# zjykzj/YOLOv4

Hardware: AMD Instinct MI355X
Metric: images/sec fwd+bwd @608x608 bs=64 per GPU (YOLOv4 training step: forward + YOLOLoss + backward) (higher is better)
Workload: dtype f32

## Files before the change

include/yolov4_amd.h:

```cpp
#ifndef YOLOV4_AMD_H
#define YOLOV4_AMD_H

#include <stddef.h>
#include <stdint.h>

#ifdef __cplusplus
extern "C" {
#endif

#define Y4_OK 0
#define Y4_ERR_SHAPE 1
#define Y4_ERR_NULL 2
#define Y4_ERR_LAUNCH 3
#define Y4_ERR_WORKSPACE 4
#define Y4_ERR_NODEVICE 5

#define Y4_ACT_LINEAR 0
#define Y4_ACT_LEAKY 1
#define Y4_ACT_MISH 2
#define Y4_ACT_RELU 3

const char* y4_strerror(int code);
int y4_version(void);
int y4_device_count(void);

int y4_set_conv_mode(int mode);
int y4_get_conv_mode(void);
int y4_set_planes_bf16(int on);
int y4_get_planes_bf16(void);
int y4_conv_planes_fit(int B, int H, int W, int Cin, int Cout, int k, int stride, int dgrad_planes);
size_t y4_conv2d_fwd_workspace(int Cin, int Cout, int k);
int y4_conv2d_fwd_f32(const float* x, int ldx, const float* w, float* y, int ldy,
                      int B, int H, int W, int Cin, int Cout, int k, int stride,
                      const float* scale, const float* shift, int act,
                      const float* residual, int ldr, const unsigned* x_amax ,
                      unsigned* y_amax ,
                      void* workspace, size_t workspace_bytes, void* stream);
size_t y4_conv2d_prepared_bytes(int Cout, int K);
int y4_conv2d_prepare_filter_f32(const float* w, int Cout, int K, void* prepared, size_t prepared_bytes, void* stream);
int y4_conv2d_fwd_prepared_f32(const float* x, int ldx, void* w_prepared, float* y, int ldy,
                               int B, int H, int W, int Cin, int Cout, int k, int stride,
                               const float* scale, const float* shift, int act,
                               const float* residual, int ldr, const unsigned* x_amax, unsigned* y_amax, void* stream);
int y4_amax_f32(const float* x, int ldx, long long M, int C, unsigned* amax_bits, void* stream);
int y4_amax_merge_u32(unsigned* dst, const unsigned* src, void* stream);

int y4_last_conv_kernel(char* buf, int cap);

size_t y4_conv2d_bnstats_workspace(int B, int H, int W, int Cin, int Cout, int k, int stride);
int y4_conv2d_fwd_bnstats_f32(const float* x, int ldx, const float* w, float* y, int ldy,
                              int B, int H, int W, int Cin, int Cout, int k, int stride,
                              float* partials, size_t partial_bytes, long long* nparts_host,
                              const unsigned* x_amax ,
                              void* workspace, size_t workspace_bytes ,
                              void* dgrad_filter ,
                              size_t dgrad_filter_bytes , void* stream);

int y4_planes_split_f32(const float* x, int ldx, long long M, int C, const unsigned* amax, void* planes, void* stream);
int y4_planes_split_into_f32(const float* x, int ldx, long long M, int C, const unsigned* amax, void* planes, int ld_planes, int c_valid,
                             void* stream);
int y4_conv2d_fwd_planes_f32(const void* x_planes, const float* w, float* y, int ldy,
                             int B, int H, int W, int Cin, int Cout, int k, int stride,
                             float* partials, size_t partial_bytes, long long* nparts_host, const unsigned* x_amax,
                             void* workspace, size_t workspace_bytes,
                             void* dgrad_filter ,
                             size_t dgrad_filter_bytes,
                             int y_bf16 ,
                             const float* bias ,
                             void* stream);

int y4_conv2d_dgrad_planes_f32(const void* dy_planes, const float* w , float* dx, int lddx,
                               int B, int H, int W, int Cin, int Cout, int k,
                               int stride ,
                               void* workspace, size_t workspace_bytes, const unsigned* dy_amax,
                               const float* residual, int ldr, void* stream);
size_t y4_conv2d_wgrad_planes_workspace(int B, int H, int W, int Cin, int Cout, int k, int stride);
int y4_conv2d_wgrad_planes_f32(const void* x_planes, const void* dy_planes, float* dw,
                               int B, int H, int W, int Cin, int Cout, int k, int stride,
                               void* workspace, size_t workspace_bytes, const unsigned* x_amax, const unsigned* dy_amax,
                               void* stream);

int y4_conv2d_generic_fwd_f32(const float* x, int ldx, const float* w, float* y, int ldy,
                              int B, int H, int W, int Cin, int Cout, int k, int stride,
                              const float* scale, const float* shift, int act, const float* residual, int ldr, void* stream);
int y4_conv2d_generic_dgrad_f32(const float* dy, int lddy, const float* w, float* dx, int lddx,
                                int B, int H, int W, int Cin, int Cout, int k, int stride,
                                const float* residual, int ldr, void* stream);
int y4_conv2d_generic_wgrad_f32(const float* x, int ldx, const float* dy, int lddy, float* dw,
                                int B, int H, int W, int Cin, int Cout, int k, int stride, void* stream);
int y4_conv2d_stem_dgrad_f32(const float* dy, int lddy, const float* w, float* dx, long long sxb, long long sxc, long long sxh,
                             long long sxw, int B, int H, int W, int Cout, void* stream);

int y4_conv2d_stem_fwd_f32(const float* x, long long sxb, long long sxc, long long sxh, long long sxw,
                           const float* w, float* y, int ldy, int B, int H, int W, int Cout,
                           const float* scale, const float* shift, int act,
                           float* bnstats_partials, void* stream);

size_t y4_conv2d_dgrad_workspace(int Cin, int Cout, int k);
int y4_conv2d_dgrad_f32(const float* dy, int lddy, const float* w , float* dx, int lddx,
                        int B, int H, int W, int Cin, int Cout, int k, int stride,
                        void* workspace, size_t workspace_bytes, const unsigned* dy_amax ,
                        const float* residual, int ldr, void* stream);

size_t y4_conv2d_wgrad_workspace(int B, int H, int W, int Cin, int Cout, int k, int stride);
int y4_conv2d_wgrad_f32(const float* x, int ldx, const float* dy, int lddy, float* dw,
                        int B, int H, int W, int Cin, int Cout, int k, int stride,
                        void* workspace, size_t workspace_bytes,
                        const unsigned* x_amax, const unsigned* dy_amax , void* stream);
size_t y4_conv2d_stem_wgrad_workspace(int B, int H, int W, int Cout);
int y4_conv2d_stem_wgrad_f32(const float* x, long long sxb, long long sxc, long long sxh, long long sxw,
                             const float* dy, int lddy, float* dw, int B, int H, int W, int Cout,
                             void* workspace, size_t workspace_bytes, void* stream);

size_t y4_bn_workspace(long long M, int C);
size_t y4_bn_finalize_workspace(int C);
int y4_bn_stats_f32(const float* y, int ldy, long long M, int C, float* mean, float* invstd,
                    float* running_mean, float* running_var, long long* num_batches_tracked,
                    float momentum, float eps, void* workspace, size_t workspace_bytes, void* stream);
int y4_bn_finalize_partials_f32(const float* partials, long long nparts, long long M, int C,
                                float* mean, float* invstd, float* running_mean, float* running_var,
                                long long* num_batches_tracked, float momentum, float eps,
                                void* workspace, size_t workspace_bytes, void* stream);
int y4_bn_planes_bound_f32(const float* gamma, const float* beta, int C, long long M, const unsigned* floor_word, unsigned* out,
                           void* stream);
int y4_bn_act_fwd_f32(const float* y, int ldy, const float* mean, const float* invstd,
                      const float* gamma, const float* beta, int act,
                      const float* residual, int ldr, float* z, int ldz,
                      long long M, int C, unsigned* out_amax, int z_planes, const unsigned* res_amax, float* planes_twin,
                      void* stream);
int y4_bn_act_bwd_f32(const float* dz, int lddz, const float* y, int ldy,
                      const float* mean, const float* invstd, const float* gamma, const float* beta,
                      int act, float* dy, int lddy, float* dgamma, float* dbeta,
                      long long M, int C, void* workspace, size_t workspace_bytes,
                      unsigned* out_amax ,
                      unsigned* f16_planes ,
                      float* planes_twin ,
                      int frozen_stats ,
                      void* stream);
size_t y4_bias_grad_workspace(long long M, int C);
int y4_bias_grad_f32(const float* dy, int lddy, long long M, int C, float* dbias,
                     void* workspace, size_t workspace_bytes, void* stream);
int y4_bn_fold_f32(const float* gamma, const float* beta, const float* running_mean,
                   const float* running_var, float eps, float* scale, float* shift, int C, void* stream);

int y4_copy_channels_f32(const float* src, int lds, float* dst, int ldd, long long M, int C, void* stream);
int y4_add_f32(const float* a, int lda, const float* b, int ldb, float* out, int ldo,
               long long M, int C, void* stream);
int y4_maxpool_s1_fwd_f32(const float* x, int ldx, float* y, int ldy, signed char* idx,
                          int B, int H, int W, int C, int ksize, void* stream);
int y4_maxpool_s1_bwd_f32(const float* dy, int lddy, const signed char* idx, float* dx, int lddx,
                          int accumulate, int B, int H, int W, int C, int ksize, void* stream);
int y4_upsample2x_fwd_f32(const float* x, int ldx, float* y, int ldy, int B, int H, int W, int C, void* stream);
int y4_upsample2x_bwd_f32(const float* dy, int lddy, float* dx, int lddx, int B, int H, int W, int C, void* stream);

int y4_yolo_decode_train_f32(const float* logits, int ldl, float* output, float* pred,
                             int B, int F, int A, int n_classes, const float* anchors_wh_host, void* stream);
int y4_yolo_decode_eval_f32(const float* logits, int ldl, float* out, long long n_total, long long box_off,
                            int B, int F, int A, int n_classes, const float* anchors_wh_host,
                            float stride, void* stream);
int y4_yolo_decode_bwd_f32(const float* logits, int ldl, const float* g_output, const float* g_pred,
                           float* g_logits, int B, int F, int A, int n_classes,
                           const float* anchors_wh_host, void* stream);

size_t y4_yolo_loss_workspace(int B, int F, int A, int K, int n_classes);
int y4_yolo_loss_fwd_f32(const float* output, const float* pred, const float* labels, int K,
                         int B, int F, int A, int n_classes, float stride, float ignore_thresh,
                         const float* all_anchors_host, int n_all_anchors, const int* anch_mask_host,
                         float* obj_mask, double* loss_parts,
                         void* workspace, size_t workspace_bytes, void* stream);
int y4_yolo_loss_bwd_f32(const float* output, int output_is_masked, const float* obj_mask,
                         const float* gscale, float* g_output,
                         int B, int F, int A, int K, int n_classes,
                         const void* workspace, size_t workspace_bytes, void* stream);
int y4_yolo_loss_mask_output_f32(float* output, const float* obj_mask, int B, int F, int A, int K,
                                 int n_classes, const void* workspace, size_t workspace_bytes, void* stream);
int y4_yolo_loss_dense_targets_f32(float* target, float* tgt_mask, float* tgt_scale,
                                   int B, int F, int A, int K, int n_classes,
                                   const void* workspace, size_t workspace_bytes, void* stream);

int y4_post_scan_i32(const int* counts, int n_segments, long long cap, int* seg_offsets, int* info, void* stream);
int y4_post_compact_f32(const float* det_rows, const int* seg_offsets, const int* kept, int B, int n_classes,
                        float* out_rows, int* out_offsets, int* img_offsets, void* stream);
int y4_post_count_f32(float* prediction, int B, long long N, int n_classes, float conf_thre,
                      int convert_xyxy, int* counts, void* stream);
size_t y4_post_nms_workspace(long long total_candidates, int n_segments);
int y4_post_nms_f32(const float* prediction, int B, long long N, int n_classes, float conf_thre,
                    float nms_thre, const int* seg_offsets , long long total_candidates,
                    float* det_rows , int* kept ,
                    void* workspace, size_t workspace_bytes, void* stream);
size_t y4_nms_workspace(long long R);
int y4_nms_f32(const float* boxes, const float* scores , long long R, float thresh,
               int limit, int* keep_idx , int* n_keep ,
               void* workspace, size_t workspace_bytes, void* stream);

int y4_bboxes_iou_f32(const float* boxes_a, long long Na, const float* boxes_b, long long Nb, int xyxy, float* iou,
                      void* stream);
int y4_act_fwd_f32(const float* x, float* y, long long n, int act, void* stream);
int y4_act_bwd_f32(const float* x, const float* dy, float* dx, long long n, int act, void* stream);
int y4_upsample_nearest_fwd_f32(const float* x, int ldx, float* y, int ldy, int B, int H, int W, int Ho, int Wo, int C,
                                int integer_factor, void* stream);
int y4_upsample_nearest_bwd_f32(const float* dy, int lddy, float* dx, int lddx, int B, int H, int W, int Ho, int Wo, int C,
                                int integer_factor, void* stream);

int y4_adam_step_f32(float* param, const float* grad, float* exp_avg, float* exp_avg_sq, long long n,
                     float lr, float beta1, float beta2, float eps, float weight_decay, int step,
                     float grad_scale, void* stream);
int y4_adam_hyper_f32(float lr, float beta1, float beta2, float weight_decay, int step, float* out4_host);
int y4_adam_multi_step_f32(const void* chunks_dev, int nchunks, const float* hyper_host, int nhyper,
                           float beta1, float beta2, float eps, float grad_scale, void* stream);
int y4_sgd_multi_step_f32(const void* chunks_dev, int nchunks, const float* hyper_host, int nhyper,
                          float grad_scale, void* stream);

int y4_preprocess_u8_f32(const void* src, int src_h, int src_w, long long src_pitch_bytes, int swap_rb,
                         float* dst, long long dst_sc, long long dst_sh, long long dst_sw, int S, void* stream);

#ifdef __cplusplus
}
#endif
#endif
```

yolov4_amd/_lib.py:

```python
import ctypes
import os
from ctypes import c_char_p, c_double, c_float, c_int, c_longlong, c_size_t, c_void_p

_HERE = os.path.dirname(os.path.abspath(__file__))
LIB_PATH = os.environ.get('Y4_LIB_PATH') or os.path.join(_HERE, 'lib', 'libyolov4_amd.so')

ACT_IDS = {'linear': 0, 'leaky_relu': 1, 'mish': 2, 'relu': 3}


class Y4Error(RuntimeError):
    pass


P = c_void_p
I, L, F, Z = c_int, c_longlong, c_float, c_size_t

PROTOTYPES = {
    'y4_strerror': (c_char_p, [I]),
    'y4_version': (I, []),
    'y4_device_count': (I, []),
    'y4_set_conv_mode': (I, [I]),
    'y4_get_conv_mode': (I, []),
    'y4_set_planes_bf16': (I, [I]),
    'y4_get_planes_bf16': (I, []),
    'y4_conv_planes_fit': (I, [I, I, I, I, I, I, I, I]),
    'y4_conv2d_fwd_workspace': (Z, [I, I, I]),
    'y4_conv2d_fwd_f32': (I, [P, I, P, P, I, I, I, I, I, I, I, I, P, P, I, P, I, P, P, P, Z, P]),
    'y4_amax_f32': (I, [P, I, L, I, P, P]),
    'y4_conv2d_prepared_bytes': (Z, [I, I]),
    'y4_conv2d_prepare_filter_f32': (I, [P, I, I, P, Z, P]),
    'y4_conv2d_fwd_prepared_f32': (I, [P, I, P, P, I, I, I, I, I, I, I, I, P, P, I, P, I, P, P, P]),
    'y4_amax_merge_u32': (I, [P, P, P]),
    'y4_last_conv_kernel': (I, [ctypes.c_char_p, I]),
    'y4_conv2d_bnstats_workspace': (Z, [I, I, I, I, I, I, I]),
    'y4_conv2d_fwd_bnstats_f32': (I, [P, I, P, P, I, I, I, I, I, I, I, I, P, Z, P, P, P, Z, P, Z, P]),
    'y4_planes_split_f32': (I, [P, I, L, I, P, P, P]),
    'y4_planes_split_into_f32': (I, [P, I, L, I, P, P, I, I, P]),
    'y4_conv2d_fwd_planes_f32': (I, [P, P, P, I, I, I, I, I, I, I, I, P, Z, P, P, P, Z, P, Z, I, P, P]),
    'y4_conv2d_dgrad_planes_f32': (I, [P, P, P, I, I, I, I, I, I, I, I, P, Z, P, P, I, P]),
    'y4_conv2d_wgrad_planes_workspace': (Z, [I, I, I, I, I, I, I]),
    'y4_conv2d_wgrad_planes_f32': (I, [P, P, P, I, I, I, I, I, I, I, P, Z, P, P, P]),
    'y4_conv2d_generic_fwd_f32': (I, [P, I, P, P, I, I, I, I, I, I, I, I, P, P, I, P, I, P]),
    'y4_conv2d_generic_dgrad_f32': (I, [P, I, P, P, I, I, I, I, I, I, I, I, P, I, P]),
    'y4_conv2d_generic_wgrad_f32': (I, [P, I, P, I, P, I, I, I, I, I, I, I, P]),
    'y4_conv2d_stem_dgrad_f32': (I, [P, I, P, P, L, L, L, L, I, I, I, I, P]),
    'y4_conv2d_stem_fwd_f32': (I, [P, L, L, L, L, P, P, I, I, I, I, I, P, P, I, P, P]),
    'y4_conv2d_dgrad_workspace': (Z, [I, I, I]),
    'y4_conv2d_dgrad_f32': (I, [P, I, P, P, I, I, I, I, I, I, I, I, P, Z, P, P, I, P]),
    'y4_conv2d_wgrad_workspace': (Z, [I, I, I, I, I, I, I]),
    'y4_conv2d_wgrad_f32': (I, [P, I, P, I, P, I, I, I, I, I, I, I, P, Z, P, P, P]),
    'y4_conv2d_stem_wgrad_workspace': (Z, [I, I, I, I]),
    'y4_conv2d_stem_wgrad_f32': (I, [P, L, L, L, L, P, I, P, I, I, I, I, P, Z, P]),
    'y4_bn_workspace': (Z, [L, I]),
    'y4_bn_finalize_workspace': (Z, [I]),
    'y4_bn_finalize_partials_f32': (I, [P, L, L, I, P, P, P, P, P, F, F, P, Z, P]),
    'y4_bn_stats_f32': (I, [P, I, L, I, P, P, P, P, P, F, F, P, Z, P]),
    'y4_bn_act_fwd_f32': (I, [P, I, P, P, P, P, I, P, I, P, I, L, I, P, I, P, P, P]),
    'y4_bn_planes_bound_f32': (I, [P, P, I, L, P, P, P]),
    'y4_bn_act_bwd_f32': (I, [P, I, P, I, P, P, P, P, I, P, I, P, P, L, I, P, Z, P, P, P, I, P]),
    'y4_bias_grad_workspace': (Z, [L, I]),
    'y4_bias_grad_f32': (I, [P, I, L, I, P, P, Z, P]),
    'y4_bn_fold_f32': (I, [P, P, P, P, F, P, P, I, P]),
    'y4_copy_channels_f32': (I, [P, I, P, I, L, I, P]),
    'y4_add_f32': (I, [P, I, P, I, P, I, L, I, P]),
    'y4_maxpool_s1_fwd_f32': (I, [P, I, P, I, P, I, I, I, I, I, P]),
    'y4_maxpool_s1_bwd_f32': (I, [P, I, P, P, I, I, I, I, I, I, I, P]),
    'y4_upsample2x_fwd_f32': (I, [P, I, P, I, I, I, I, I, P]),
    'y4_upsample2x_bwd_f32': (I, [P, I, P, I, I, I, I, I, P]),
    'y4_yolo_decode_train_f32': (I, [P, I, P, P, I, I, I, I, P, P]),
    'y4_yolo_decode_eval_f32': (I, [P, I, P, L, L, I, I, I, I, P, F, P]),
    'y4_yolo_decode_bwd_f32': (I, [P, I, P, P, P, I, I, I, I, P, P]),
    'y4_yolo_loss_workspace': (Z, [I, I, I, I, I]),
    'y4_yolo_loss_fwd_f32': (I, [P, P, P, I, I, I, I, I, F, F, P, I, P, P, P, P, Z, P]),
    'y4_yolo_loss_bwd_f32': (I, [P, I, P, P, P, I, I, I, I, I, P, Z, P]),
    'y4_yolo_loss_mask_output_f32': (I, [P, P, I, I, I, I, I, P, Z, P]),
    'y4_yolo_loss_dense_targets_f32': (I, [P, P, P, I, I, I, I, I, P, Z, P]),
    'y4_post_count_f32': (I, [P, I, L, I, F, I, P, P]),
    'y4_post_scan_i32': (I, [P, I, L, P, P, P]),
    'y4_post_compact_f32': (I, [P, P, P, I, I, P, P, P, P]),
    'y4_post_nms_workspace': (Z, [L, I]),
    'y4_post_nms_f32': (I, [P, I, L, I, F, F, P, L, P, P, P, Z, P]),
    'y4_nms_workspace': (Z, [L]),
    'y4_nms_f32': (I, [P, P, L, F, I, P, P, P, Z, P]),
    'y4_bboxes_iou_f32': (I, [P, L, P, L, I, P, P]),
    'y4_act_fwd_f32': (I, [P, P, L, I, P]),
    'y4_act_bwd_f32': (I, [P, P, P, L, I, P]),
    'y4_upsample_nearest_fwd_f32': (I, [P, I, P, I, I, I, I, I, I, I, I, P]),
    'y4_upsample_nearest_bwd_f32': (I, [P, I, P, I, I, I, I, I, I, I, I, P]),
    'y4_adam_step_f32': (I, [P, P, P, P, L, F, F, F, F, F, I, F, P]),
    'y4_adam_hyper_f32': (I, [F, F, F, F, I, P]),
    'y4_adam_multi_step_f32': (I, [P, I, P, I, F, F, F, F, P]),
    'y4_sgd_multi_step_f32': (I, [P, I, P, I, F, P]),
    'y4_preprocess_u8_f32': (I, [P, I, I, L, I, P, L, L, L, I, P]),
}

_lib = None


def lib():
    global _lib
    if _lib is None:
        if not os.path.isfile(LIB_PATH):
            raise Y4Error(f'{LIB_PATH} is missing: build it with `make -C yolov4_amd/csrc` '
                          '(hipcc --offload-arch=gfx950); there is no fallback path')
        handle = ctypes.CDLL(LIB_PATH)
        for name, (res, args) in PROTOTYPES.items():
            fn = getattr(handle, name)
            fn.restype = res
            fn.argtypes = args
        _lib = handle
        if os.environ.get('Y4_CONV_MODE'):
            handle.y4_set_conv_mode(int(os.environ['Y4_CONV_MODE']))
    return _lib


def check(code, what=''):
    if code != 0:
        msg = lib().y4_strerror(code).decode()
        raise Y4Error(f'{what}: {msg} (code {code})')


def float_array(values):
    arr = (c_float * len(values))(*[float(v) for v in values])
    return arr


def int_array(values):
    return (c_int * len(values))(*[int(v) for v in values])
```

yolov4_amd/csrc/common.h:

```cpp
#pragma once
#include <hip/hip_runtime.h>
#include <stdint.h>
#include "../../include/yolov4_amd.h"

typedef float f32x4 __attribute__((ext_vector_type(4)));
typedef float f32x16 __attribute__((ext_vector_type(16)));
typedef unsigned int u32x4 __attribute__((ext_vector_type(4)));

#define Y4_CHECK_LAUNCH()                                   \
    do {                                                    \
        if (hipGetLastError() != hipSuccess) return Y4_ERR_LAUNCH; \
    } while (0)

static inline hipStream_t y4_stream(void* s) { return reinterpret_cast<hipStream_t>(s); }

#include <atomic>
struct Y4DynLds {
    std::atomic<unsigned long long> done{0ull};
    bool ensure(const void* kernel, size_t bytes) {
        int d = 0;
        if (hipGetDevice(&d) != hipSuccess) return false;
        if (d >= 0 && d < 64 && ((done.load(std::memory_order_acquire) >> d) & 1ull)) return true;
        if (hipFuncSetAttribute(kernel, hipFuncAttributeMaxDynamicSharedMemorySize, (int)bytes) != hipSuccess) return false;
        if (d >= 0 && d < 64) done.fetch_or(1ull << d, std::memory_order_release);
        return true;
    }
};

__device__ __forceinline__ float y4_mish(float x) {
    const float n = __expf(fminf(x, 20.0f));
    const float w = n * (n + 2.0f);
    return x * (w * __frcp_rn(w + 2.0f));
}
__device__ __forceinline__ float y4_mish_grad(float x) {
    const float n = __expf(fminf(x, 20.0f));
    const float w = n * (n + 2.0f);
    const float rd = __frcp_rn(w + 2.0f);
    const float q = fmaf(n, n, n);
    return fmaf(4.0f * (x * q), rd, w) * rd;
}
__device__ __forceinline__ float y4_act(float x, int act) {
    switch (act) {
        case Y4_ACT_LEAKY: return x > 0.0f ? x : 0.1f * x;
        case Y4_ACT_MISH: return y4_mish(x);
        case Y4_ACT_RELU: return fmaxf(x, 0.0f);
        default: return x;
    }
}
__device__ __forceinline__ float y4_act_grad(float x, int act) {
    switch (act) {
        case Y4_ACT_LEAKY: return x > 0.0f ? 1.0f : 0.1f;
        case Y4_ACT_MISH: return y4_mish_grad(x);
        case Y4_ACT_RELU: return x > 0.0f ? 1.0f : 0.0f;
        default: return 1.0f;
    }
}

template <int ACT> __device__ __forceinline__ float y4_act_t(float x) {
    if constexpr (ACT == Y4_ACT_LEAKY) return x > 0.0f ? x : 0.1f * x;
    else if constexpr (ACT == Y4_ACT_MISH) return y4_mish(x);
    else if constexpr (ACT == Y4_ACT_RELU) return fmaxf(x, 0.0f);
    else return x;
}
template <int ACT> __device__ __forceinline__ float y4_act_grad_t(float x) {
    if constexpr (ACT == Y4_ACT_LEAKY) return x > 0.0f ? 1.0f : 0.1f;
    else if constexpr (ACT == Y4_ACT_MISH) return y4_mish_grad(x);
    else if constexpr (ACT == Y4_ACT_RELU) return x > 0.0f ? 1.0f : 0.0f;
    else return 1.0f;
}

__device__ __forceinline__ int y4_xcd_remap(int bid, int nwg) {
    const int q = nwg >> 3, r = nwg & 7, xcd = bid & 7;
    const int base = (xcd < r) ? xcd * (q + 1) : r * (q + 1) + (xcd - r) * q;
    return base + (bid >> 3);
}

__device__ __forceinline__ __amdgpu_buffer_rsrc_t y4_make_rsrc(const void* base, unsigned num_bytes) {
    return __builtin_amdgcn_make_buffer_rsrc(const_cast<void*>(base), (short)0, (int)num_bytes, 0x00020000);
}
__device__ __forceinline__ f32x4 y4_buf_load4(__amdgpu_buffer_rsrc_t r, unsigned voff_bytes, unsigned soff_bytes) {
    const u32x4 v = __builtin_amdgcn_raw_buffer_load_b128(r, (int)voff_bytes, (int)soff_bytes, 0);
    return __builtin_bit_cast(f32x4, v);
}
```

yolov4_amd/csrc/conv_geom.h:

```cpp
#pragma once
#include "common.h"

namespace y4 {

struct ConvGeom {
    const float* src; const float* wt; float* dst;
    const float* scale; const float* shift; const float* res;
    float* stats;
    long long lds_, ldd, ldr;
    int B, Hs, Ws, Cs;
    int Cs_valid;
    int Hd, Wd, N;
    int k, stride, pad;
    int M;
    int K;
    int act;
    int mtiles, ntiles;
    int cls_tile0[5];
    int cls_h[2], cls_w[2];
    int cls_slot0[5];
    unsigned long long src_total_bytes;
    unsigned wt_bytes;
    const unsigned short* wt_planes;
    const unsigned* src_amax; const unsigned* wt_amax;
    unsigned* dst_amax;
};

struct WgradGeom {
    const float* x; const float* dy; float* out;
    long long ldx, lddy;
    int B, H, W, Cin, Ho, Wo, Cout;
    int k, stride, pad;
    int M;
    int J;
    int ntn, ntj, splits, chunks_per_split;
    int tn, tj;
    const unsigned* x_amax; const unsigned* dy_amax;
    unsigned long long x_total_bytes, dy_total_bytes;
};

int f16x2_gather(const ConvGeom& g, bool transposed, hipStream_t st, int* nparts);
int f16x2_wgrad(const WgradGeom& g, hipStream_t st);
int f16x2_refresh_prepared(const float* w, void* prepared, int Cout, int K, hipStream_t st);
int f16x2_filter_planes(const float* w, unsigned short* planes, int Cout, int K, unsigned* amax_out, unsigned* part, hipStream_t st);
int f16x2_filter_planes_dual(const float* w, unsigned short* planes, unsigned* amax_out, unsigned* part, unsigned short* planes_t,
                             unsigned* amax_out_t, int Cout, int Cin, int kk, int Cout_pad, bool mirror, hipStream_t st);
int f16x2_filter_planes_transposed(const float* w, unsigned short* planes, int Cout, int Cin, int kk, int Cout_pad,
                                   unsigned* amax_out, unsigned* part, hipStream_t st, bool mirror = false);
int slab_reduce(const float* slabs, float* dw, long long n, int splits, hipStream_t st);
int amax_launch(const float* x, long long ld, long long M, int C, unsigned* amax_bits, hipStream_t st,
                bool prezeroed = false);
int amax_merge(unsigned* dst, const unsigned* src, hipStream_t st);


bool tile_conv_ok(int Cs, int Cs_valid, int N, int k, int stride, int H, int W);
int f16x2_tile(const ConvGeom& g, hipStream_t st, int* nparts);
bool tile_dgrad_s2_ok(int Cs, int Cs_valid, int N, int k, int stride, int Hs, int Ws);
int f16x2_tile_dgrad_s2(const ConvGeom& g, hipStream_t st);

bool tile_wgrad_ok(int Cin, int Cout, int k, int stride, int H, int W, long long ldx, long long lddy);
int tile_wgrad_slabs(int Cin, int Cout);
int f16x2_wgrad_tile(const WgradGeom& g, hipStream_t st);

bool planes_conv_ok(int Cin, int Cout, int k, int stride);
int planes_conv(const void* src, const unsigned* src_amax, const void* wt_planes, const unsigned* wt_amax, float* dst, long long ldd,
                const float* res, long long ldr, float* stats, int* nparts, int B, int Hs, int Ws, int Cs, int N, int k, int stride,
                hipStream_t st, bool bf = false, bool dst_bf16 = false);
int planes_dgrad_s2(const void* dy, const unsigned* dy_amax, const void* wt_planes, const unsigned* wt_amax, float* dx, long long lddx,
                    int B, int H, int W, int Cin, int Cout, hipStream_t st, bool bf = false);
int planes_split(const float* x, long long ld, long long M, int C, const unsigned* amax, void* planes, hipStream_t st, bool bf = false,
                 long long pitch_ch = 0, int c_valid = 0);
void planes_wgrad_plan(int B, int H, int W, int Cin, int Cout, int k, int* ntn, int* ntj, int* splits, int* sps, int tn = 128, bool bf = false);
int planes_wgrad_tn(int Cout, bool bf);
int planes_wgrad(const void* x, const unsigned* x_amax, const void* dy, const unsigned* dy_amax, float* dw, void* workspace,
                 size_t workspace_bytes, int B, int H, int W, int Cin, int Cout, int k, hipStream_t st, bool bf = false,
                 int stride = 1);

void note_kernel(const char* fmt, ...);
}
```

yolov4_amd/csrc/conv_igemm.hip:

```cpp
#include <stdlib.h>
#include "common.h"
#include <cstdarg>
#include <cstdio>
#include "conv_geom.h"

namespace {

constexpr int BK = 32;


using y4::ConvGeom;
using y4::WgradGeom;

template <int BM, int BN, int WM, int WN, bool TRANSPOSED, int BKT = 32>
__global__ __launch_bounds__(256, (BKT == 16 ? 3 : 2)) void conv_gather_mfma_f32(const ConvGeom g) {
    constexpr int LPR = BKT / 4;
    constexpr int RPP = 256 / LPR;
    constexpr int PA = BM / RPP, PB = BN / RPP;
    constexpr int LDS_PITCH = BKT + 4;
    constexpr int BK = BKT;
    constexpr int WTM = BM / WM, WTN = BN / WN;
    constexpr int TM = WTM / 32, TN = WTN / 32;
    static_assert(WM * WN == 4, "4 waves");
    extern __shared__ __attribute__((aligned(16))) float smem[];
// ... 1073 lines not shown
    f32x4 ra[4], rb[4];
    int ld_chunk = 0;
    auto load_chunk = [&]() {
        const int pbase = (chunk0 + ld_chunk) * 32 + pg * 4;
#pragma unroll
        for (int i = 0; i < 4; ++i) {
            const bool ok = an_ok && pbase + i < g.M;
            ra[i] = y4_buf_load4(dy_rsrc, ok ? a_off0 + (unsigned)i * dy_pix_bytes : OOB, (unsigned)ld_chunk * chunk_bytes);
        }
#pragma unroll
        for (int i = 0; i < 4; ++i) {
            const int hi = pb_h[i] * g.stride - g.pad + jr, wi = pb_w[i] * g.stride - g.pad + jq;
            const bool ok = bj_ok && pbase + i < g.M && (unsigned)hi < (unsigned)g.H && (unsigned)wi < (unsigned)g.W;
            const unsigned off = (unsigned)((pb_b[i] * g.H + hi) * g.W + wi) * x_pix_bytes + (unsigned)jc * 4u;
            rb[i] = y4_buf_load4(x_rsrc, ok ? off : OOB, 0u);
            pb_w[i] += 32;
            while (pb_w[i] >= g.Wo) { pb_w[i] -= g.Wo; if (++pb_h[i] == g.Ho) { pb_h[i] = 0; ++pb_b[i]; } }
        }
        ++ld_chunk;
    };
    auto split_store = [&](const f32x4 (&v)[4], unsigned char* base, int rows) {
        if constexpr (NP == 1) {
#pragma unroll
            for (int e = 0; e < 4; ++e) {
                u32x2 p;
                p[0] = pack_hi16(rn_bf16_bits(v[1][e]), rn_bf16_bits(v[0][e]));
                p[1] = pack_hi16(rn_bf16_bits(v[3][e]), rn_bf16_bits(v[2][e]));
                *reinterpret_cast<u32x2*>(base + (cg * 4 + e) * PITCH_B + pg * 8) = p;
            }
            return;
        }
        unsigned h1[4][4], h2[4][4], h3[4][4];
#pragma unroll
        for (int i = 0; i < 4; ++i)
#pragma unroll
            for (int e = 0; e < 4; ++e) {
                h1[i][e] = __float_as_uint(v[i][e]);
                const float r1 = v[i][e] - __uint_as_float(h1[i][e] & 0xffff0000u);
                h2[i][e] = __float_as_uint(r1);
                const float r2 = r1 - __uint_as_float(h2[i][e] & 0xffff0000u);
                h3[i][e] = __float_as_uint(r2);
            }
#pragma unroll
        for (int e = 0; e < 4; ++e) {
            unsigned char* d = base + (cg * 4 + e) * PITCH_B + pg * 8;
            u32x2 p;
            p[0] = pack_hi16(h1[1][e], h1[0][e]); p[1] = pack_hi16(h1[3][e], h1[2][e]);
            *reinterpret_cast<u32x2*>(d) = p;
            p[0] = pack_hi16(h2[1][e], h2[0][e]); p[1] = pack_hi16(h2[3][e], h2[2][e]);
            *reinterpret_cast<u32x2*>(d + rows * PITCH_B) = p;
            p[0] = pack_hi16(h3[1][e], h3[0][e]); p[1] = pack_hi16(h3[3][e], h3[2][e]);
            *reinterpret_cast<u32x2*>(d + 2 * rows * PITCH_B) = p;
        }
    };
    auto store_chunk = [&]() {
        if (a_act) split_store(ra, As, TN_);
        if (b_act) split_store(rb, Bs, TJ_);
    };

    f32x16 acc[MI][MJ];
#pragma unroll
    for (int i = 0; i < MI; ++i)
#pragma unroll
        for (int jj = 0; jj < MJ; ++jj)
#pragma unroll
            for (int e = 0; e < 16; ++e) acc[i][jj][e] = 0.f;

    const int fr = lane & 31, fh = lane >> 5;
    const unsigned char* a_frag = As + (wm * (TN_ / 2) + fr) * PITCH_B + fh * 16;
    const unsigned char* b_frag = Bs + (wn * (TJ_ / 2) + fr) * PITCH_B + fh * 16;
    if (nchunks > 0) {
        load_chunk();
        store_chunk();
        __syncthreads();
        for (int ch = 0; ch < nchunks; ++ch) {
            if (ch + 1 < nchunks) load_chunk();
#pragma unroll
            for (int ks = 0; ks < 2; ++ks) {
                bf16x8 fa[MI][NP], fb[MJ][NP];
#pragma unroll
                for (int i = 0; i < MI; ++i)
#pragma unroll
                    for (int pl = 0; pl < NP; ++pl)
                        fa[i][pl] = *reinterpret_cast<const bf16x8*>(a_frag + pl * TN_ * PITCH_B + i * 32 * PITCH_B + ks * 32);
#pragma unroll
                for (int jj = 0; jj < MJ; ++jj)
#pragma unroll
                    for (int pl = 0; pl < NP; ++pl)
                        fb[jj][pl] = *reinterpret_cast<const bf16x8*>(b_frag + pl * TJ_ * PITCH_B + jj * 32 * PITCH_B + ks * 32);
#pragma unroll
                for (int i = 0; i < MI; ++i)
#pragma unroll
                    for (int jj = 0; jj < MJ; ++jj) {
                        f32x16 c = acc[i][jj];
                        if constexpr (NP == 3) {
                            c = __builtin_amdgcn_mfma_f32_32x32x16_bf16(fa[i][2], fb[jj][0], c, 0, 0, 0);
                            c = __builtin_amdgcn_mfma_f32_32x32x16_bf16(fa[i][1], fb[jj][1], c, 0, 0, 0);
                            c = __builtin_amdgcn_mfma_f32_32x32x16_bf16(fa[i][0], fb[jj][2], c, 0, 0, 0);
                            c = __builtin_amdgcn_mfma_f32_32x32x16_bf16(fa[i][1], fb[jj][0], c, 0, 0, 0);
                            c = __builtin_amdgcn_mfma_f32_32x32x16_bf16(fa[i][0], fb[jj][1], c, 0, 0, 0);
                        }
                        c = __builtin_amdgcn_mfma_f32_32x32x16_bf16(fa[i][0], fb[jj][0], c, 0, 0, 0);
                        acc[i][jj] = c;
                    }
            }
            __syncthreads();
            if (ch + 1 < nchunks) store_chunk();
            __syncthreads();
        }
    }
    float* out = g.out + (long long)split * g.Cout * g.J;
#pragma unroll
    for (int jj = 0; jj < MJ; ++jj) {
        const int jcol = j0 + wn * (TJ_ / 2) + jj * 32 + fr;
#pragma unroll
        for (int i = 0; i < MI; ++i) {
            const int nb = n0 + wm * (TN_ / 2) + i * 32 + 4 * fh;
#pragma unroll
            for (int e = 0; e < 16; ++e) {
                const int n = nb + (e & 3) + 8 * (e >> 2);
                if (n < g.Cout && jcol < g.J) out[(long long)n * g.J + jcol] = acc[i][jj][e];
            }
        }
    }
}

template <int VEC>
__global__ __launch_bounds__(256) void slab_reduce_vec_kernel(const f32x4* __restrict__ slabs, f32x4* __restrict__ out,
                                                              long long nvec, int splits) {
    constexpr int SG = 256 / VEC;
    __shared__ f32x4 red[SG][VEC];
    const int v = threadIdx.x % VEC, sg = threadIdx.x / VEC;
    const long long i = (long long)blockIdx.x * VEC + v;
    f32x4 s0 = {0.f, 0.f, 0.f, 0.f}, s1 = s0, s2 = s0, s3 = s0;
    if (i < nvec) {
        int k = sg;
        for (; k + 3 * SG < splits; k += 4 * SG) {
            const f32x4 a = slabs[(long long)k * nvec + i], b = slabs[(long long)(k + SG) * nvec + i];
            const f32x4 c = slabs[(long long)(k + 2 * SG) * nvec + i], d = slabs[(long long)(k + 3 * SG) * nvec + i];
            s0 += a; s1 += b; s2 += c; s3 += d;
        }
        for (; k < splits; k += SG) s0 += slabs[(long long)k * nvec + i];
    }
    red[sg][v] = (s0 + s1) + (s2 + s3);
    __syncthreads();
    if (sg == 0 && i < nvec) {
        f32x4 t = red[0][v];
#pragma unroll
        for (int g = 1; g < SG; ++g) t += red[g][v];
        out[i] = t;
    }
}

__global__ void slab_reduce_kernel(const float* __restrict__ slabs, float* __restrict__ out,
                                   long long n, int splits) {
    for (long long i = blockIdx.x * (long long)blockDim.x + threadIdx.x; i < n;
         i += (long long)gridDim.x * blockDim.x) {
        float s = 0.f;
        for (int k = 0; k < splits; ++k) s += slabs[(long long)k * n + i];
        out[i] = s;
    }
}

void wgrad_plan(int B, int H, int W, int Cin, int Cout, int k, int stride, WgradGeom& g) {
    const int pad = (k - 1) / 2;
    g.B = B; g.H = H; g.W = W; g.Cin = Cin; g.Cout = Cout; g.k = k; g.stride = stride; g.pad = pad;
    g.Ho = (H + 2 * pad - k) / stride + 1;
    g.Wo = (W + 2 * pad - k) / stride + 1;
    g.M = B * g.Ho * g.Wo;
    g.J = k * k * Cin;
    g.tn = Cout <= 64 ? 64 : 128;
    g.tj = g.J <= 64 ? 64 : 128;
    g.ntn = (Cout + g.tn - 1) / g.tn;
    g.ntj = (g.J + g.tj - 1) / g.tj;
    const int tiles = g.ntn * g.ntj;
    const int chunks = (g.M + 31) / 32;
    int per_cu = (160 * 1024) / (2 * 32 * (g.tn + g.tj) * 4);
    if (per_cu > 4) per_cu = 4;
    if (g.tn + g.tj == 256 && per_cu > 2) per_cu = 2;
    const int slots = 256 * per_cu;
    int max_s = chunks / 16;
    if (max_s < 1) max_s = 1;
    if (max_s > 4096) max_s = 4096;
    int best_s = 1;
    double best_eff = -1.0;
    for (int sp = 1; sp <= max_s; ++sp) {
        const long long blocks = (long long)tiles * sp;
        const long long rounds = (blocks + slots - 1) / slots;
        double eff = (double)blocks / (double)(rounds * slots);
        if (rounds > 6) eff = 1.0;
        if (eff > best_eff + 0.02) { best_eff = eff; best_s = sp; }
        if (blocks >= 2ll * slots && eff >= 0.93) break;
        if (blocks >= 6ll * slots) break;
    }
    { static const char* fs = getenv("Y4_WGRAD_SPLITS"); if (fs) { best_s = atoi(fs); if (best_s > max_s) best_s = max_s; if (best_s < 1) best_s = 1; } }
    g.chunks_per_split = (chunks + best_s - 1) / best_s;
    const unsigned long long per_px = 8ull * (unsigned long long)((Cout + 3) / 4 * 4 > Cin * stride * stride ? (Cout + 3) / 4 * 4 : Cin * stride * stride);
    const unsigned long long slack = 2ull * g.Ho * g.Wo;
    const unsigned long long max_px = 0xf0000000ull / per_px;
    if (max_px > slack + 32 && (unsigned long long)g.chunks_per_split * 32ull + slack > max_px)
        g.chunks_per_split = (int)((max_px - slack) / 32ull);
    g.splits = (chunks + g.chunks_per_split - 1) / g.chunks_per_split;
}

template <int TN_, int TJ_, int NP = 0>
int launch_wgrad(const WgradGeom& g, hipStream_t st) {
    constexpr bool SPLIT = NP > 0;
    const size_t smem = SPLIT ? (size_t)NP * (TN_ + TJ_) * 80 : 2ull * 32 * (TN_ + TJ_) * sizeof(float);
    void (*kern)(const WgradGeom);
    if constexpr (SPLIT) kern = conv_wgrad_bf16x3<TN_, TJ_, (NP > 0 ? NP : 3)>;
    else kern = conv_wgrad_mfma_f32<TN_, TJ_>;
    static Y4DynLds lds_attr;
    if (!lds_attr.ensure(reinterpret_cast<const void*>(kern), smem)) return Y4_ERR_LAUNCH;
    hipLaunchKernelGGL(kern, dim3(g.ntn * g.ntj * g.splits), dim3(256), smem, st, g);
    Y4_CHECK_LAUNCH();
    return Y4_OK;
}

struct StemGeom {
    const float* x; const float* w; float* y; const float* scale; const float* shift;
    float* stats;
    long long sxb, sxc, sxh, sxw, ldy;
    int B, H, W, Cout, act;
    long long M;
};

__global__ __launch_bounds__(256) void conv_stem_fwd_kernel(const StemGeom g) {
    __shared__ float tile[4][64][33];
    __shared__ __attribute__((aligned(16))) float wl[27 * 32];
    const int tid = threadIdx.x, lane = tid & 63, wave = tid >> 6;
    for (int i = tid; i < 27 * 32; i += 256) {
        const int n = i & 31, kk = i >> 5;
        wl[i] = n < g.Cout ? g.w[n * 27 + kk] : 0.f;
    }
    __syncthreads();
    const long long pix0 = (long long)blockIdx.x * 256 + wave * 64;
    const long long pix = pix0 + lane;
    float acc[32];
#pragma unroll
    for (int n = 0; n < 32; ++n) acc[n] = 0.f;
    if (pix < g.M) {
        const int b = (int)(pix / ((long long)g.H * g.W));
        const int rem = (int)(pix - (long long)b * g.H * g.W);
        const int h = rem / g.W, w = rem - h * g.W;
        const float* xb = g.x + b * g.sxb;
        float xv[27];
#pragma unroll
        for (int r = 0; r < 3; ++r)
#pragma unroll
            for (int q = 0; q < 3; ++q) {
                const int hi = h + r - 1, wi = w + q - 1;
                const bool ok = (unsigned)hi < (unsigned)g.H && (unsigned)wi < (unsigned)g.W;
#pragma unroll
                for (int c = 0; c < 3; ++c) xv[(r * 3 + q) * 3 + c] = ok ? xb[c * g.sxc + hi * g.sxh + wi * g.sxw] : 0.f;
            }
#pragma unroll
        for (int kk = 0; kk < 27; ++kk) {
            const f32x4* wp = reinterpret_cast<const f32x4*>(wl + kk * 32);
            const float v = xv[kk];
#pragma unroll
            for (int n4 = 0; n4 < 8; ++n4) {
                const f32x4 wv = wp[n4];
#pragma unroll
                for (int e = 0; e < 4; ++e) acc[n4 * 4 + e] = fmaf(v, wv[e], acc[n4 * 4 + e]);
            }
            __builtin_amdgcn_sched_barrier(0);
        }
    }
#pragma unroll
    for (int n = 0; n < 32; ++n) {
        float v = acc[n];
        if (n < g.Cout) {
            v = v * (g.scale ? g.scale[n] : 1.f) + (g.shift ? g.shift[n] : 0.f);
            v = y4_act(v, g.act);
        }
        tile[wave][lane][n] = v;
    }
    __syncthreads();
    const int ch = lane & 31;
    if (ch < g.Cout) {
#pragma unroll 4
        for (int it = 0; it < 32; ++it) {
            const int pl = it * 2 + (lane >> 5);
            const long long p = pix0 + pl;
            if (p < g.M) g.y[p * g.ldy + ch] = tile[wave][pl][ch];
        }
    }
    if (g.stats) {
        __shared__ float sred[8][32][2];
        const int grp = tid >> 5;
        float cs = 0.f, css = 0.f;
        for (int i = 0; i < 32; ++i) { const float v = tile[grp >> 1][(grp & 1) * 32 + i][ch]; cs += v; css += v * v; }
        sred[grp][ch][0] = cs; sred[grp][ch][1] = css;
        __syncthreads();
        if (tid < 64) {
            const int c = tid & 31, which = tid >> 5;
            float t = 0.f;
            for (int k = 0; k < 8; ++k) t += sred[k][c][which];
            if (c < g.Cout) g.stats[((long long)blockIdx.x * 2 + which) * g.Cout + c] = t;
        }
    }
}

__global__ __launch_bounds__(256) void conv_stem_fwd_bf16x3_kernel(const StemGeom g, const int ngroups, const float inv_hw,
                                                                   const float inv_w) {
    __shared__ float sred[4][32][2];
    const int tid = threadIdx.x, lane = tid & 63, wave = tid >> 6;
    const int fr = lane & 31, fh = lane >> 5;
    const int HW = g.H * g.W;
    bf16x8 fb[2][3];
    int koff[16];
    int ktap[16];
#pragma unroll
    for (int i = 0; i < 16; ++i) {
        const int k = (i >> 3) * 16 + fh * 8 + (i & 7);
        const int r = k / 9, c = (k - r * 9) / 3, q = k - r * 9 - c * 3;
        const bool kv = k < 27;
        koff[i] = kv ? (int)(c * g.sxc + (r - 1) * g.sxh + (q - 1) * g.sxw) * 4 : 0;
        ktap[i] = kv ? r * 3 + q : 9;
    }
#pragma unroll
    for (int ks = 0; ks < 2; ++ks) {
        f32x4 w0, w1;
#pragma unroll
        for (int i = 0; i < 8; ++i) {
            const int k = ks * 16 + fh * 8 + i;
            const int r = k / 9, c = (k - r * 9) / 3, q = k - r * 9 - c * 3;
            const float v = (k < 27 && fr < g.Cout) ? g.w[fr * 27 + (r * 3 + q) * 3 + c] : 0.f;
            if (i < 4) w0[i] = v; else w1[i - 4] = v;
        }
        u32x2 a1, a2, a3, b1, b2, b3;
        split3x4(w0, a1, a2, a3);
        split3x4(w1, b1, b2, b3);
        const u32x4 q1 = {a1[0], a1[1], b1[0], b1[1]}, q2 = {a2[0], a2[1], b2[0], b2[1]}, q3 = {a3[0], a3[1], b3[0], b3[1]};
        fb[ks][0] = __builtin_bit_cast(bf16x8, q1); fb[ks][1] = __builtin_bit_cast(bf16x8, q2); fb[ks][2] = __builtin_bit_cast(bf16x8, q3);
    }
    const float sc = (g.scale && fr < g.Cout) ? g.scale[fr] : 1.f;
    const float sh = (g.shift && fr < g.Cout) ? g.shift[fr] : 0.f;
    const __amdgpu_buffer_rsrc_t rsrc = y4_make_rsrc(g.x, 0xfffffff0u);
    float xv0[16], xv1[16];
    auto load = [&](float (&xv)[16], long long tile) {
        const long long p = tile * 32 + fr;
        unsigned base = 0xffffffffu;
        unsigned m9 = 0;
        if (p < g.M) {
            int b = (int)((float)p * inv_hw);
            int rem = (int)(p - (long long)b * HW);
            if (rem < 0) { --b; rem += HW; } else if (rem >= HW) { ++b; rem -= HW; }
            int h = (int)((float)rem * inv_w);
            int w = rem - h * g.W;
            if (w < 0) { --h; w += g.W; } else if (w >= g.W) { ++h; w -= g.W; }
            base = (unsigned)(b * g.sxb + h * g.sxh + w * g.sxw) * 4u;
            const unsigned hm = (h > 0 ? 1u : 0u) | 2u | (h + 1 < g.H ? 4u : 0u);
            const unsigned wm = (w > 0 ? 1u : 0u) | 2u | (w + 1 < g.W ? 4u : 0u);
            m9 = ((hm & 1u) ? wm : 0u) | ((hm & 2u) ? wm << 3 : 0u) | ((hm & 4u) ? wm << 6 : 0u);
        }
#pragma unroll
        for (int i = 0; i < 16; ++i) {
            const bool ok = (m9 >> ktap[i]) & 1u;
            xv[i] = __builtin_bit_cast(float, __builtin_amdgcn_raw_buffer_load_b32(rsrc, ok ? (int)(base + (unsigned)koff[i]) : -1, 0, 0));
        }
    };
    float cs = 0.f, css = 0.f;
    auto compute = [&](float (&xv)[16], long long tile) {
        f32x16 acc;
#pragma unroll
        for (int e = 0; e < 16; ++e) acc[e] = 0.f;
#pragma unroll
        for (int ks = 0; ks < 2; ++ks) {
            const f32x4 v0 = {xv[ks * 8 + 0], xv[ks * 8 + 1], xv[ks * 8 + 2], xv[ks * 8 + 3]};
            const f32x4 v1 = {xv[ks * 8 + 4], xv[ks * 8 + 5], xv[ks * 8 + 6], xv[ks * 8 + 7]};
            u32x2 a1, a2, a3, b1, b2, b3;
            split3x4(v0, a1, a2, a3);
            split3x4(v1, b1, b2, b3);
            const u32x4 q1 = {a1[0], a1[1], b1[0], b1[1]}, q2 = {a2[0], a2[1], b2[0], b2[1]}, q3 = {a3[0], a3[1], b3[0], b3[1]};
            const bf16x8 f1 = __builtin_bit_cast(bf16x8, q1), f2 = __builtin_bit_cast(bf16x8, q2), f3 = __builtin_bit_cast(bf16x8, q3);
            acc = __builtin_amdgcn_mfma_f32_32x32x16_bf16(f3, fb[ks][0], acc, 0, 0, 0);
            acc = __builtin_amdgcn_mfma_f32_32x32x16_bf16(f2, fb[ks][1], acc, 0, 0, 0);
            acc = __builtin_amdgcn_mfma_f32_32x32x16_bf16(f1, fb[ks][2], acc, 0, 0, 0);
            acc = __builtin_amdgcn_mfma_f32_32x32x16_bf16(f2, fb[ks][0], acc, 0, 0, 0);
            acc = __builtin_amdgcn_mfma_f32_32x32x16_bf16(f1, fb[ks][1], acc, 0, 0, 0);
            acc = __builtin_amdgcn_mfma_f32_32x32x16_bf16(f1, fb[ks][0], acc, 0, 0, 0);
        }
        const long long mbase = tile * 32 + 4 * fh;
#pragma unroll
        for (int e = 0; e < 16; ++e) {
            const float raw = acc[e];
            cs += raw; css += raw * raw;
            const long long m = mbase + (e & 3) + 8 * (e >> 2);
            if (fr < g.Cout && m < g.M) g.y[m * g.ldy + fr] = y4_act(raw * sc + sh, g.act);
        }
    };
    for (int grp = blockIdx.x; grp < ngroups; grp += gridDim.x) {
        const long long t0 = (long long)grp * 8 + wave * 2;
        load(xv0, t0);
        load(xv1, t0 + 1);
        cs = 0.f; css = 0.f;
        compute(xv0, t0);
        compute(xv1, t0 + 1);
        if (g.stats) {
            cs += __shfl_xor(cs, 32, 64);
            css += __shfl_xor(css, 32, 64);
            if (fh == 0) { sred[wave][fr][0] = cs; sred[wave][fr][1] = css; }
            __syncthreads();
            if (tid < 64) {
                const int c = tid & 31, which = tid >> 5;
                const float t = (sred[0][c][which] + sred[1][c][which]) + (sred[2][c][which] + sred[3][c][which]);
                if (c < g.Cout) g.stats[((long long)grp * 2 + which) * g.Cout + c] = t;
            }
            __syncthreads();
        }
    }
}

struct StemWgradGeom {
    const float* x; const float* dy; float* slabs;
    long long sxb, sxc, sxh, sxw, lddy;
    int B, H, W, Cout;
    long long M, pix_per_wave;
};

__global__ __launch_bounds__(256) void conv_stem_wgrad_kernel(const StemWgradGeom g) {
    const int tid = threadIdx.x, lane = tid & 63;
    const long long wave_id = (long long)blockIdx.x * 4 + (tid >> 6);
    const long long p_begin = wave_id * g.pix_per_wave;
    long long p_end = p_begin + g.pix_per_wave;
    if (p_end > g.M) p_end = g.M;
    const int fr = lane & 31, fh = lane >> 5;
    const bool jok = fr < 27;
    const int tap = jok ? fr / 3 : 0, c = jok ? fr - tap * 3 : 0;
    const int r = tap / 3 - 1, q = tap - (tap / 3) * 3 - 1;
    const bool nok = fr < g.Cout;
    f32x16 acc;
#pragma unroll
    for (int e = 0; e < 16; ++e) acc[e] = 0.f;
    long long p = p_begin + fh;
    int b = 0, h = 0, w = 0;
    if (p < g.M) {
        b = (int)(p / ((long long)g.H * g.W));
        const int rem = (int)(p - (long long)b * g.H * g.W);
        h = rem / g.W; w = rem - h * g.W;
    }
    const long long dy_first = p_begin < g.M ? p_begin : 0;
    const __amdgpu_buffer_rsrc_t dy_rsrc = y4_make_rsrc(g.dy + dy_first * g.lddy, (unsigned)(g.pix_per_wave * g.lddy * 4));
    const __amdgpu_buffer_rsrc_t x_rsrc = y4_make_rsrc(g.x, 0xfffffff0u);
    const unsigned dy_step = (unsigned)g.lddy * 8u;
    unsigned dy_off = ((unsigned)fh * (unsigned)g.lddy + (unsigned)fr) * 4u;
    const long long coff = c * g.sxc;
    for (long long pc = p_begin; pc < p_end; pc += 16) {
        float a[8], bv[8];
#pragma unroll
        for (int u = 0; u < 8; ++u) {
            const bool pok = p < p_end;
            const int hi = h + r, wi = w + q;
            const bool xok = pok && jok && (unsigned)hi < (unsigned)g.H && (unsigned)wi < (unsigned)g.W;
            const unsigned xo = (unsigned)(b * g.sxb + coff + hi * g.sxh + wi * g.sxw) * 4u;
            a[u] = __builtin_bit_cast(float, __builtin_amdgcn_raw_buffer_load_b32(dy_rsrc, (pok && nok) ? (int)dy_off : -1, 0, 0));
            bv[u] = __builtin_bit_cast(float, __builtin_amdgcn_raw_buffer_load_b32(x_rsrc, xok ? (int)xo : -1, 0, 0));
            dy_off += dy_step;
            p += 2;
            w += 2;
            if (w >= g.W) { w -= g.W; if (++h == g.H) { h = 0; ++b; } }
        }
#pragma unroll
        for (int u = 0; u < 8; ++u) acc = __builtin_amdgcn_mfma_f32_32x32x2f32(a[u], bv[u], acc, 0, 0, 0);
    }
    float* out = g.slabs + wave_id * 1024;
#pragma unroll
    for (int e = 0; e < 16; ++e) {
        const int n = (e & 3) + 8 * (e >> 2) + 4 * fh;
        out[n * 32 + fr] = acc[e];
    }
}

__global__ __launch_bounds__(256) void stem_wgrad_reduce1_kernel(const float* __restrict__ slabs, double* __restrict__ part,
                                                                 int nslabs) {
    const int per = (nslabs + gridDim.x - 1) / gridDim.x;
    const int k0 = blockIdx.x * per;
    const int k1 = min(nslabs, k0 + per);
    double s[4] = {0, 0, 0, 0};
    for (int k = k0; k < k1; ++k) {
        const f32x4 v = *reinterpret_cast<const f32x4*>(slabs + (long long)k * 1024 + threadIdx.x * 4);
#pragma unroll
        for (int e = 0; e < 4; ++e) s[e] += (double)v[e];
    }
#pragma unroll
    for (int e = 0; e < 4; ++e) part[(long long)blockIdx.x * 1024 + threadIdx.x * 4 + e] = s[e];
}
__global__ __launch_bounds__(256) void stem_wgrad_reduce2_kernel(const double* __restrict__ part, float* __restrict__ dw,
                                                                 int nparts, int Cout) {
    for (int i = threadIdx.x; i < Cout * 27; i += 256) {
        const int n = i / 27, j = i - n * 27;
        double s = 0.0;
        for (int k = 0; k < nparts; ++k) s += part[(long long)k * 1024 + n * 32 + j];
        dw[i] = (float)s;
    }
}

constexpr int STEM_WAVES = 4096;

}

namespace y4 {
int slab_reduce(const float* slabs, float* dw, long long n, int splits, hipStream_t st) {
    if ((n & 3) == 0 && !(reinterpret_cast<uintptr_t>(dw) & 15) && !(reinterpret_cast<uintptr_t>(slabs) & 15)) {
        const long long nvec = n / 4;
        if (nvec >= 64 * 1024)
            hipLaunchKernelGGL(slab_reduce_vec_kernel<64>, dim3((unsigned)((nvec + 63) / 64)), dim3(256), 0, st,
                               reinterpret_cast<const f32x4*>(slabs), reinterpret_cast<f32x4*>(dw), nvec, splits);
        else
            hipLaunchKernelGGL(slab_reduce_vec_kernel<16>, dim3((unsigned)((nvec + 15) / 16)), dim3(256), 0, st,
                               reinterpret_cast<const f32x4*>(slabs), reinterpret_cast<f32x4*>(dw), nvec, splits);
    } else {
        const int blocks = (int)((n + 255) / 256 > 2048 ? 2048 : (n + 255) / 256);
        hipLaunchKernelGGL(slab_reduce_kernel, dim3(blocks), dim3(256), 0, st, slabs, dw, n, splits);
    }
    Y4_CHECK_LAUNCH();
    return Y4_OK;
}
}

extern "C" {

int y4_set_conv_mode(int mode) {
    if (mode < 0 || mode > 3) return Y4_ERR_SHAPE;
    g_conv_mode = mode;
    return Y4_OK;
}
int y4_get_conv_mode(void) { return g_conv_mode; }

constexpr size_t FWD_WS_HDR = 64 + 4096;

size_t y4_conv2d_fwd_workspace(int Cin, int Cout, int k) {
    if (Cin <= 0 || Cout <= 0 || k <= 0) return 0;
    return FWD_WS_HDR + (size_t)Cout * k * k * Cin * 6;
}

static int conv_fwd_impl(const float* x, int ldx, const float* w, float* y, int ldy,
                         int B, int H, int W, int Cin, int Cout, int k, int stride,
                         const float* scale, const float* shift, int act,
                         const float* residual, int ldr, float* stats, int* nparts, const unsigned* x_amax,
                         unsigned* y_amax, void* workspace, size_t workspace_bytes, void* stream,
                         void* w_prepared = nullptr, void* dgrad_filter = nullptr, size_t dgrad_filter_bytes = 0) {
    if (!x || (!w && !w_prepared) || !y) return Y4_ERR_NULL;
    if (B <= 0 || H <= 0 || W <= 0 || Cout <= 0 || (k != 1 && k != 3) || (stride != 1 && stride != 2))
        return Y4_ERR_SHAPE;
    if (Cin <= 0 || Cin % BK != 0 || ldx < Cin || ldy < Cout || (ldx & 3) || (residual && ldr < Cout))
        return Y4_ERR_SHAPE;
    if ((reinterpret_cast<uintptr_t>(x) & 15) || (reinterpret_cast<uintptr_t>(w) & 15)) return Y4_ERR_SHAPE;
    const int pad = (k - 1) / 2;
    ConvGeom g{};
    g.src = x; g.wt = w; g.dst = y; g.scale = scale; g.shift = shift; g.res = residual; g.stats = stats;
    g.lds_ = ldx; g.ldd = ldy; g.ldr = ldr;
    g.B = B; g.Hs = H; g.Ws = W; g.Cs = Cin; g.Cs_valid = Cin;
    g.Hd = (H + 2 * pad - k) / stride + 1;
    g.Wd = (W + 2 * pad - k) / stride + 1;
    g.N = Cout; g.k = k; g.stride = stride; g.pad = pad;
    const long long M = (long long)B * g.Hd * g.Wd;
    if (M >= (1ll << 31)) return Y4_ERR_SHAPE;
    g.M = (int)M; g.K = k * k * Cin; g.act = act;
    if (w_prepared) {
        if (g_conv_mode != 3) return Y4_ERR_SHAPE;
        if (reinterpret_cast<uintptr_t>(w_prepared) & 15) return Y4_ERR_SHAPE;
        unsigned* hdr = static_cast<unsigned*>(w_prepared);
        g.wt_planes = reinterpret_cast<unsigned short*>(static_cast<char*>(w_prepared) + 64 + 4096);
        if (!x_amax) {
            const int rc = y4::amax_launch(x, ldx, (long long)B * H * W, Cin, hdr + 1, y4_stream(stream));
            if (rc != Y4_OK) return rc;
            x_amax = hdr + 1;
        }
        g.src_amax = x_amax; g.wt_amax = hdr; g.dst_amax = y_amax;
        return y4::f16x2_gather(g, false, y4_stream(stream), nparts);
    }
    if (g_conv_mode != 0) {
        const long long nw = (long long)Cout * g.K;
        if (!workspace) return Y4_ERR_NULL;
        if (workspace_bytes < y4_conv2d_fwd_workspace(Cin, Cout, k)) return Y4_ERR_WORKSPACE;
        if (reinterpret_cast<uintptr_t>(workspace) & 15) return Y4_ERR_SHAPE;
        unsigned* hdr = static_cast<unsigned*>(workspace);
        unsigned short* planes = reinterpret_cast<unsigned short*>(static_cast<char*>(workspace) + FWD_WS_HDR);
        g.wt_planes = planes;
        if (g_conv_mode == 3) {
            int rc;
            if (dgrad_filter) {
                if (dgrad_filter_bytes < y4_conv2d_dgrad_workspace(Cin, Cout, k)) return Y4_ERR_WORKSPACE;
                if (reinterpret_cast<uintptr_t>(dgrad_filter) & 15) return Y4_ERR_SHAPE;
                const int cp = (Cout + 31) / 32 * 32;
                unsigned* hdr_t = reinterpret_cast<unsigned*>(static_cast<char*>(dgrad_filter) + (size_t)Cin * k * k * cp * 6);
                rc = y4::f16x2_filter_planes_dual(w, planes, hdr, hdr + 16, static_cast<unsigned short*>(dgrad_filter), hdr_t, Cout, Cin,
                                                  k * k, cp, y4::tile_conv_ok(cp, Cout, Cin, k, stride, H, W), y4_stream(stream));
            } else {
                rc = y4::f16x2_filter_planes(w, planes, Cout, g.K, hdr, hdr + 16, y4_stream(stream));
            }
            if (rc != Y4_OK) return rc;
            if (!x_amax) {
                rc = y4::amax_launch(x, ldx, (long long)B * H * W, Cin, hdr + 1, y4_stream(stream));
                if (rc != Y4_OK) return rc;
                x_amax = hdr + 1;
            }
            g.src_amax = x_amax; g.wt_amax = hdr; g.dst_amax = y_amax;
            return y4::f16x2_gather(g, false, y4_stream(stream), nparts);
        }
        const int blocks = (int)((nw + 255) / 256 > 4096 ? 4096 : (nw + 255) / 256);
        hipLaunchKernelGGL(split_filter_kernel, dim3(blocks), dim3(256), 0, y4_stream(stream), w, planes, nw,
                           g_conv_mode == 2 ? 1 : 3);
        Y4_CHECK_LAUNCH();
    }
    return dispatch_gather<false>(g, y4_stream(stream), nparts);
}

int y4_conv2d_fwd_f32(const float* x, int ldx, const float* w, float* y, int ldy,
                      int B, int H, int W, int Cin, int Cout, int k, int stride,
                      const float* scale, const float* shift, int act,
                      const float* residual, int ldr, const unsigned* x_amax, unsigned* y_amax,
                      void* workspace, size_t workspace_bytes, void* stream) {
    return conv_fwd_impl(x, ldx, w, y, ldy, B, H, W, Cin, Cout, k, stride, scale, shift, act, residual, ldr, nullptr,
                         nullptr, x_amax, y_amax, workspace, workspace_bytes, stream);
}

int y4_amax_f32(const float* x, int ldx, long long M, int C, unsigned* amax_bits, void* stream) {
    if (!x || !amax_bits) return Y4_ERR_NULL;
    if (M < 0 || C <= 0 || ldx < C) return Y4_ERR_SHAPE;
    return y4::amax_launch(x, ldx, M, C, amax_bits, y4_stream(stream));
}

int y4_amax_merge_u32(unsigned* dst, const unsigned* src, void* stream) {
    if (!dst || !src) return Y4_ERR_NULL;
    return y4::amax_merge(dst, src, y4_stream(stream));
}

size_t y4_conv2d_bnstats_workspace(int B, int H, int W, int Cin, int Cout, int k, int stride) {
    if (B <= 0 || H <= 0 || W <= 0 || Cout <= 0 || (k != 1 && k != 3) || (stride != 1 && stride != 2)) return 0;
    const int pad = (k - 1) / 2;
    const long long M = (long long)B * ((H + 2 * pad - k) / stride + 1) * ((W + 2 * pad - k) / stride + 1);
    long long rows = Cin == 3 ? (M + 255) / 256 : (M + 63) / 64;
    const long long per_img = (long long)B * ((M / B + 127) / 128);
    if (per_img > rows) rows = per_img;
    return (size_t)rows * 2 * Cout * sizeof(float);
}

int y4_conv2d_fwd_bnstats_f32(const float* x, int ldx, const float* w, float* y, int ldy,
                              int B, int H, int W, int Cin, int Cout, int k, int stride,
                              float* partials, size_t partial_bytes, long long* nparts_host, const unsigned* x_amax,
                              void* workspace, size_t workspace_bytes, void* dgrad_filter, size_t dgrad_filter_bytes,
                              void* stream) {
    if (!partials || !nparts_host) return Y4_ERR_NULL;
    if (dgrad_filter && g_conv_mode != 3) return Y4_ERR_SHAPE;
    if (partial_bytes < y4_conv2d_bnstats_workspace(B, H, W, Cin, Cout, k, stride)) return Y4_ERR_WORKSPACE;
    int np = 0;
    const int rc = conv_fwd_impl(x, ldx, w, y, ldy, B, H, W, Cin, Cout, k, stride, nullptr, nullptr, Y4_ACT_LINEAR,
                                 nullptr, 0, partials, &np, x_amax, nullptr, workspace, workspace_bytes, stream, nullptr,
                                 dgrad_filter, dgrad_filter_bytes);
    if (rc != Y4_OK) return rc;
    *nparts_host = np;
    return Y4_OK;
}

size_t y4_conv2d_dgrad_workspace(int Cin, int Cout, int k) {
    const size_t cp = (size_t)((Cout + 31) / 32) * 32;
    return (size_t)Cin * k * k * cp * 6 + 64 + 4096;
}

static int conv_dgrad_impl(const float* dy, int lddy, const float* w, float* dx, int lddx,
                           int B, int H, int W, int Cin, int Cout, int k, int stride,
                           void* workspace, size_t workspace_bytes, const unsigned* dy_amax,
                           const float* residual, int ldr, void* stream) {
    if (!dy || !dx || !workspace) return Y4_ERR_NULL;
    if (!w && g_conv_mode != 3) return Y4_ERR_NULL;
    if (B <= 0 || H <= 0 || W <= 0 || Cin <= 0 || Cout <= 0 || (k != 1 && k != 3) || (stride != 1 && stride != 2))
        return Y4_ERR_SHAPE;
    const int Cout_pad = (Cout + 31) / 32 * 32;
    if (lddy < Cout_pad || (lddy & 3) || lddx < Cin) return Y4_ERR_SHAPE;
    if (workspace_bytes < y4_conv2d_dgrad_workspace(Cin, Cout, k)) return Y4_ERR_WORKSPACE;
    if ((reinterpret_cast<uintptr_t>(dy) & 15) || (reinterpret_cast<uintptr_t>(workspace) & 15)) return Y4_ERR_SHAPE;
    hipStream_t st = y4_stream(stream);
    float* wt = static_cast<float*>(workspace);
    const long long total = (long long)Cin * k * k * Cout_pad;
    const int blocks = (int)((total + 255) / 256 > 4096 ? 4096 : (total + 255) / 256);
    unsigned* hdr = reinterpret_cast<unsigned*>(static_cast<char*>(workspace) + (size_t)total * 6);
    unsigned* wamax = hdr;
    if (g_conv_mode == 3) {
        if (w) {
            const int rc = y4::f16x2_filter_planes_transposed(w, static_cast<unsigned short*>(workspace), Cout, Cin, k * k, Cout_pad,
                                                              wamax, hdr + 16, st, y4::tile_conv_ok(Cout_pad, Cout, Cin, k, stride, H, W));
            if (rc != Y4_OK) return rc;
        }
    } else if (g_conv_mode != 0)
        hipLaunchKernelGGL(transpose_split_filter_kernel, dim3(blocks), dim3(256), 0, st, w,
                           static_cast<unsigned short*>(workspace), Cout, Cin, k * k, Cout_pad, g_conv_mode == 2 ? 1 : 3);
    else
        hipLaunchKernelGGL(transpose_filter_kernel, dim3(blocks), dim3(256), 0, st, w, wt, Cout, Cin, k * k, Cout_pad);
    Y4_CHECK_LAUNCH();
    const int pad = (k - 1) / 2;
    ConvGeom g{};
    if (residual && ldr < Cin) return Y4_ERR_SHAPE;
    g.src = dy; g.wt = wt; g.dst = dx; g.scale = nullptr; g.shift = nullptr; g.res = residual;
    g.wt_planes = static_cast<const unsigned short*>(workspace);
    g.lds_ = lddy; g.ldd = lddx; g.ldr = ldr;
    g.B = B;
    g.Hs = (H + 2 * pad - k) / stride + 1;
    g.Ws = (W + 2 * pad - k) / stride + 1;
    g.Cs = Cout_pad; g.Cs_valid = Cout;
    g.Hd = H; g.Wd = W; g.N = Cin; g.k = k; g.stride = stride; g.pad = pad;
    const long long M = (long long)B * H * W;
    if (M >= (1ll << 31)) return Y4_ERR_SHAPE;
    g.M = (int)M; g.K = k * k * Cout_pad; g.act = Y4_ACT_LINEAR;
    if (g_conv_mode == 3) {
        if (!dy_amax) {
            const int rc = y4::amax_launch(dy, lddy, (long long)B * g.Hs * g.Ws, Cout, hdr + 1, st);
            if (rc != Y4_OK) return rc;
            dy_amax = hdr + 1;
        }
        g.src_amax = dy_amax; g.wt_amax = wamax;
        if (y4::tile_conv_ok(Cout_pad, Cout, Cin, k, stride, H, W)) return y4::f16x2_tile(g, st, nullptr);
        if (y4::tile_dgrad_s2_ok(Cout_pad, Cout, Cin, k, stride, g.Hs, g.Ws)) return y4::f16x2_tile_dgrad_s2(g, st);
        return y4::f16x2_gather(g, true, st, nullptr);
    }
    return dispatch_gather<true>(g, st);
}

int y4_conv2d_dgrad_f32(const float* dy, int lddy, const float* w, float* dx, int lddx,
                        int B, int H, int W, int Cin, int Cout, int k, int stride,
                        void* workspace, size_t workspace_bytes, const unsigned* dy_amax,
                        const float* residual, int ldr, void* stream) {
    return conv_dgrad_impl(dy, lddy, w, dx, lddx, B, H, W, Cin, Cout, k, stride, workspace, workspace_bytes, dy_amax,
                           residual, ldr, stream);
}

int y4_last_conv_kernel(char* buf, int cap) {
    if (!buf || cap <= 0) return Y4_ERR_NULL;
    snprintf(buf, (size_t)cap, "%s", g_last_kernel);
    g_last_kernel[0] = 0;
    return Y4_OK;
}

size_t y4_conv2d_prepared_bytes(int Cout, int K) {
    if (Cout <= 0 || K <= 0) return 0;
    return 64 + 4096 + (size_t)Cout * (size_t)K * 4;
}

int y4_conv2d_prepare_filter_f32(const float* w, int Cout, int K, void* prepared, size_t prepared_bytes, void* stream) {
    if (!w || !prepared) return Y4_ERR_NULL;
    if (Cout <= 0 || K <= 0 || (K & 31)) return Y4_ERR_SHAPE;
    if (prepared_bytes < y4_conv2d_prepared_bytes(Cout, K)) return Y4_ERR_WORKSPACE;
    if ((reinterpret_cast<uintptr_t>(prepared) & 15) || (reinterpret_cast<uintptr_t>(w) & 15)) return Y4_ERR_SHAPE;
    return y4::f16x2_refresh_prepared(w, prepared, Cout, K, y4_stream(stream));
}

int y4_conv2d_fwd_prepared_f32(const float* x, int ldx, void* w_prepared, float* y, int ldy,
                               int B, int H, int W, int Cin, int Cout, int k, int stride,
                               const float* scale, const float* shift, int act,
                               const float* residual, int ldr, const unsigned* x_amax, unsigned* y_amax, void* stream) {
    if (!w_prepared) return Y4_ERR_NULL;
    return conv_fwd_impl(x, ldx, nullptr, y, ldy, B, H, W, Cin, Cout, k, stride, scale, shift, act, residual, ldr, nullptr,
                         nullptr, x_amax, y_amax, nullptr, 0, stream, w_prepared);
}

size_t y4_conv2d_wgrad_workspace(int B, int H, int W, int Cin, int Cout, int k, int stride) {
    WgradGeom g{};
    wgrad_plan(B, H, W, Cin, Cout, k, stride, g);
    int splits = g.splits;
    if (y4::tile_wgrad_ok(Cin, Cout, k, stride, H, W, 0, 0) && y4::tile_wgrad_slabs(Cin, Cout) > splits) splits = y4::tile_wgrad_slabs(Cin, Cout);
    return (splits > 1 ? (size_t)splits * Cout * g.J * sizeof(float) : 0) + 64;
}

int y4_conv2d_wgrad_f32(const float* x, int ldx, const float* dy, int lddy, float* dw,
                        int B, int H, int W, int Cin, int Cout, int k, int stride,
                        void* workspace, size_t workspace_bytes, const unsigned* x_amax, const unsigned* dy_amax,
                        void* stream) {
    if (!x || !dy || !dw) return Y4_ERR_NULL;
    if (B <= 0 || H <= 0 || W <= 0 || Cout <= 0 || (k != 1 && k != 3) || (stride != 1 && stride != 2))
        return Y4_ERR_SHAPE;
    if (Cin <= 0 || (Cin & 3) || ldx < Cin || (ldx & 3) || (lddy & 3) || lddy < ((Cout + 3) & ~3)) return Y4_ERR_SHAPE;
    if ((reinterpret_cast<uintptr_t>(x) & 15) || (reinterpret_cast<uintptr_t>(dy) & 15)) return Y4_ERR_SHAPE;
    WgradGeom g{};
    wgrad_plan(B, H, W, Cin, Cout, k, stride, g);
    if ((long long)B * g.Ho * g.Wo >= (1ll << 31)) return Y4_ERR_SHAPE;
    g.x = x; g.dy = dy; g.ldx = ldx; g.lddy = lddy;
    {
        g.x_total_bytes = (unsigned long long)B * H * W * (unsigned long long)ldx * 4ull;
        g.dy_total_bytes = (unsigned long long)B * g.Ho * g.Wo * (unsigned long long)lddy * 4ull;
        const unsigned long long range_px = (unsigned long long)g.chunks_per_split * 32ull + 2ull * g.Ho * g.Wo;
        const unsigned long long per_px = 4ull * (unsigned long long)(lddy > ldx * stride * stride ? lddy : ldx * stride * stride);
        if (range_px * per_px >= 0xfffffff0ull) return Y4_ERR_SHAPE;
    }
    hipStream_t st = y4_stream(stream);
    const bool tile = g_conv_mode == 3 && y4::tile_wgrad_ok(Cin, Cout, k, stride, H, W, ldx, lddy);
    if (tile) g.splits = y4::tile_wgrad_slabs(Cin, Cout);
    const size_t slab_bytes = g.splits > 1 ? (size_t)g.splits * Cout * g.J * sizeof(float) : 0;
    if (g.splits > 1) {
        if (!workspace) return Y4_ERR_NULL;
        if (workspace_bytes < slab_bytes) return Y4_ERR_WORKSPACE;
        g.out = static_cast<float*>(workspace);
    } else {
        g.out = dw;
    }
    int rc;
    if (g_conv_mode == 3) {
        if (!x_amax || !dy_amax) {
            if (!workspace || workspace_bytes < slab_bytes + 64) return Y4_ERR_WORKSPACE;
            unsigned* hdr = reinterpret_cast<unsigned*>(static_cast<char*>(workspace) + slab_bytes);
            if (!x_amax) {
                rc = y4::amax_launch(x, ldx, (long long)B * H * W, Cin, hdr, st);
                if (rc != Y4_OK) return rc;
                x_amax = hdr;
            }
            if (!dy_amax) {
                rc = y4::amax_launch(dy, lddy, (long long)B * g.Ho * g.Wo, Cout, hdr + 1, st);
                if (rc != Y4_OK) return rc;
                dy_amax = hdr + 1;
            }
        }
        g.x_amax = x_amax; g.dy_amax = dy_amax;
        rc = tile ? y4::f16x2_wgrad_tile(g, st) : y4::f16x2_wgrad(g, st);
    } else if (g_conv_mode == 1) {
        if (g.tn == 128 && g.tj == 128) rc = launch_wgrad<128, 128, 3>(g, st);
        else if (g.tn == 128) rc = launch_wgrad<128, 64, 3>(g, st);
        else if (g.tj == 128) rc = launch_wgrad<64, 128, 3>(g, st);
        else rc = launch_wgrad<64, 64, 3>(g, st);
    } else if (g_conv_mode == 2) {
        if (g.tn == 128 && g.tj == 128) rc = launch_wgrad<128, 128, 1>(g, st);
        else if (g.tn == 128) rc = launch_wgrad<128, 64, 1>(g, st);
        else if (g.tj == 128) rc = launch_wgrad<64, 128, 1>(g, st);
        else rc = launch_wgrad<64, 64, 1>(g, st);
    } else if (g.tn == 128 && g.tj == 128) rc = launch_wgrad<128, 128>(g, st);
    else if (g.tn == 128) rc = launch_wgrad<128, 64>(g, st);
    else if (g.tj == 128) rc = launch_wgrad<64, 128>(g, st);
    else rc = launch_wgrad<64, 64>(g, st);
    if (rc != Y4_OK) return rc;
    if (g.splits > 1) {
        const int rc2 = y4::slab_reduce(static_cast<const float*>(workspace), dw, (long long)Cout * g.J, g.splits, st);
        if (rc2 != Y4_OK) return rc2;
    }
    return Y4_OK;
}

int y4_conv2d_stem_fwd_f32(const float* x, long long sxb, long long sxc, long long sxh, long long sxw,
                           const float* w, float* y, int ldy, int B, int H, int W, int Cout,
                           const float* scale, const float* shift, int act,
                           float* bnstats_partials, void* stream) {
    if (!x || !w || !y) return Y4_ERR_NULL;
    if (B <= 0 || H <= 0 || W <= 0 || Cout <= 0 || Cout > 32 || ldy < Cout) return Y4_ERR_SHAPE;
    StemGeom g{};
    g.x = x; g.w = w; g.y = y; g.scale = scale; g.shift = shift; g.stats = bnstats_partials;
    g.sxb = sxb; g.sxc = sxc; g.sxh = sxh; g.sxw = sxw; g.ldy = ldy;
    g.B = B; g.H = H; g.W = W; g.Cout = Cout; g.act = act;
    g.M = (long long)B * H * W;
    const long long blocks = (g.M + 255) / 256;
    if (blocks >= (1ll << 31)) return Y4_ERR_SHAPE;
    const bool mfma_ok = (g_conv_mode >= 1 && g_conv_mode <= 3) && sxb >= 0 && sxc >= 0 && sxh >= 0 && sxw >= 0 &&
                         ((long long)(B - 1) * sxb + 2 * sxc + (long long)(H - 1) * sxh + (long long)(W - 1) * sxw + 1) * 4 < 0xfffffff0ll &&
                         (long long)H * W < (1 << 24);
    if (mfma_ok) {
        const int grid = (int)(blocks < 2048 ? blocks : 2048);
        hipLaunchKernelGGL(conv_stem_fwd_bf16x3_kernel, dim3(grid), dim3(256), 0, y4_stream(stream), g, (int)blocks,
                           1.0f / (float)((long long)H * W), 1.0f / (float)W);
        Y4_CHECK_LAUNCH();
        return Y4_OK;
    }
    hipLaunchKernelGGL(conv_stem_fwd_kernel, dim3((unsigned)blocks), dim3(256), 0, y4_stream(stream), g);
    Y4_CHECK_LAUNCH();
    return Y4_OK;
}

size_t y4_conv2d_stem_wgrad_workspace(int, int, int, int) {
    return (size_t)STEM_WAVES * 1024 * sizeof(float) + 64 * 1024 * sizeof(double);
}

int y4_conv2d_stem_wgrad_f32(const float* x, long long sxb, long long sxc, long long sxh, long long sxw,
                             const float* dy, int lddy, float* dw, int B, int H, int W, int Cout,
                             void* workspace, size_t workspace_bytes, void* stream) {
    if (!x || !dy || !dw || !workspace) return Y4_ERR_NULL;
    if (B <= 0 || H <= 0 || W < 2 || Cout <= 0 || Cout > 32 || lddy < Cout) return Y4_ERR_SHAPE;
    if (workspace_bytes < y4_conv2d_stem_wgrad_workspace(B, H, W, Cout)) return Y4_ERR_WORKSPACE;
    StemWgradGeom g{};
    g.x = x; g.dy = dy; g.slabs = static_cast<float*>(workspace);
    g.sxb = sxb; g.sxc = sxc; g.sxh = sxh; g.sxw = sxw; g.lddy = lddy;
    g.B = B; g.H = H; g.W = W; g.Cout = Cout;
    g.M = (long long)B * H * W;
    long long ppw = (g.M + STEM_WAVES - 1) / STEM_WAVES;
    ppw = (ppw + 15) & ~15ll;
    if ((long long)ppw * lddy * 4 >= 0xfffffff0ll || sxb < 0 || sxc < 0 || sxh < 0 || sxw < 0 ||
        ((long long)(B - 1) * sxb + 2 * sxc + (long long)(H - 1) * sxh + (long long)(W - 1) * sxw + 1) * 4 >= 0xfffffff0ll)
        return Y4_ERR_SHAPE;
    g.pix_per_wave = ppw;
    hipStream_t st = y4_stream(stream);
    hipLaunchKernelGGL(conv_stem_wgrad_kernel, dim3(STEM_WAVES / 4), dim3(256), 0, st, g);
    Y4_CHECK_LAUNCH();
    double* part = reinterpret_cast<double*>(static_cast<char*>(workspace) + (size_t)STEM_WAVES * 1024 * sizeof(float));
    hipLaunchKernelGGL(stem_wgrad_reduce1_kernel, dim3(64), dim3(256), 0, st, static_cast<const float*>(workspace), part,
                       STEM_WAVES);
    Y4_CHECK_LAUNCH();
    hipLaunchKernelGGL(stem_wgrad_reduce2_kernel, dim3(1), dim3(256), 0, st, part, dw, 64, Cout);
    Y4_CHECK_LAUNCH();
    return Y4_OK;
}

}
```

yolov4_amd/csrc/pointwise.hip:

```cpp
#include "common.h"

namespace {

constexpr int PW_THREADS = 256;
constexpr int PW_UNROLL = 4;
#define Y4_ACT_SWITCH(ACTV, CALL)                                              \
    switch (ACTV) {                                                            \
        case Y4_ACT_MISH: { constexpr int A_ = Y4_ACT_MISH; CALL; } break;     \
        case Y4_ACT_LEAKY: { constexpr int A_ = Y4_ACT_LEAKY; CALL; } break;   \
        case Y4_ACT_RELU: { constexpr int A_ = Y4_ACT_RELU; CALL; } break;     \
        default: { constexpr int A_ = Y4_ACT_LINEAR; CALL; } break;            \
    }

struct RowMap {
    int tpr;
    int rpb;
};
static inline RowMap row_map(int C) {
    RowMap r;
    int c4 = C / 4;
    r.tpr = c4 < PW_THREADS ? c4 : PW_THREADS;
    int p = 1;
    while (p * 2 <= r.tpr) p *= 2;
    r.tpr = p;
    r.rpb = PW_THREADS / r.tpr;
    return r;
}

__device__ __forceinline__ f32x4 ld4(const float* p) { return *reinterpret_cast<const f32x4*>(p); }
__device__ __forceinline__ void st4(float* p, f32x4 v) { *reinterpret_cast<f32x4*>(p) = v; }
__device__ __forceinline__ f32x4 ld4y(const float* row, int c0, int ybf) {
    if (!ybf) return ld4(row + c0);
    typedef unsigned u2 __attribute__((ext_vector_type(2)));
    const u2 b = *reinterpret_cast<const u2*>(reinterpret_cast<const unsigned char*>(row) + c0 * 2);
    f32x4 v;
    v[0] = __uint_as_float(b[0] << 16); v[1] = __uint_as_float(b[0] & 0xffff0000u);
    v[2] = __uint_as_float(b[1] << 16); v[3] = __uint_as_float(b[1] & 0xffff0000u);
    return v;
}

constexpr int STAT_ROWS_PER_THREAD = 128;
static inline int stat_rows(long long M, int rpb) {
    long long r = M / ((long long)rpb * 4096);
    if (r < 4) r = 4;
    if (r > STAT_ROWS_PER_THREAD) r = STAT_ROWS_PER_THREAD;
    return (int)r;
}

__global__ __launch_bounds__(PW_THREADS) void bn_stats_kernel(const float* __restrict__ y, long long ldy,
                                                              long long M, int C, int tpr, int rpb, int nrows,
                                                              float* __restrict__ part ) {
    __shared__ float red[2][PW_THREADS][4];
    const int tid = threadIdx.x;
    const int cv = tid % tpr, rg = tid / tpr;
    const long long row0 = (long long)blockIdx.x * rpb * nrows;
    for (int cb = 0; cb < C; cb += tpr * 4) {
        const int c0 = cb + cv * 4;
        const bool cok = c0 < C;
        f32x4 s = {0, 0, 0, 0}, ss = {0, 0, 0, 0};
#pragma unroll 8
        for (int i = 0; i < nrows; ++i) {
            const long long m = row0 + (long long)i * rpb + rg;
            if (m < M && cok) {
                const f32x4 v = ld4(y + m * ldy + c0);
                s += v;
                ss += v * v;
            }
        }
#pragma unroll
        for (int e = 0; e < 4; ++e) { red[0][tid][e] = s[e]; red[1][tid][e] = ss[e]; }
        __syncthreads();
        if (rg == 0 && cok) {
            f32x4 ds = {0, 0, 0, 0}, dss = {0, 0, 0, 0};
            for (int g = 0; g < rpb; ++g)
#pragma unroll
                for (int e = 0; e < 4; ++e) {
                    ds[e] += red[0][g * tpr + cv][e];
                    dss[e] += red[1][g * tpr + cv][e];
                }
            float* pp = part + (long long)blockIdx.x * 2 * C;
            st4(pp + c0, ds);
            st4(pp + C + c0, dss);
        }
        __syncthreads();
    }
}

constexpr int FOLD_BLOCKS = 256;
__global__ __launch_bounds__(PW_THREADS) void fold_partials_kernel(const float* __restrict__ part, long long nparts,
                                                                   int C2, int cw, double* __restrict__ bacc) {
    __shared__ double red[PW_THREADS];
    const long long per = (nparts + gridDim.x - 1) / gridDim.x;
    const long long p0 = (long long)blockIdx.x * per;
    long long p1 = p0 + per;
    if (p1 > nparts) p1 = nparts;
    const int rg_n = PW_THREADS / cw;
    const int col = threadIdx.x % cw, rg = threadIdx.x / cw;
    for (int c0 = 0; c0 < C2; c0 += cw) {
        const int c = c0 + col;
        double s[8] = {0, 0, 0, 0, 0, 0, 0, 0};
        if (c < C2) {
            long long p = p0 + rg;
            for (; p + 7ll * rg_n < p1; p += 8ll * rg_n) {
                float v[8];
#pragma unroll
                for (int u = 0; u < 8; ++u) v[u] = part[(p + (long long)u * rg_n) * C2 + c];
#pragma unroll
                for (int u = 0; u < 8; ++u) s[u] += (double)v[u];
            }
            for (; p < p1; p += rg_n) s[0] += (double)part[p * C2 + c];
        }
        red[threadIdx.x] = ((s[0] + s[1]) + (s[2] + s[3])) + ((s[4] + s[5]) + (s[6] + s[7]));
        __syncthreads();
        if (rg == 0 && c < C2) {
            double t = red[col];
            for (int g = 1; g < rg_n; ++g) t += red[g * cw + col];
            bacc[(long long)blockIdx.x * C2 + c] = t;
        }
        __syncthreads();
    }
}

__device__ __forceinline__ void fold_rows32(const double* __restrict__ bacc, int nb, int C, int c0, double (&red)[2][8][32],
                                            double& s, double& ss) {
    const int cl = threadIdx.x & 31, g = threadIdx.x >> 5;
    const int c = c0 + cl;
    double a = 0, b2 = 0;
    if (c < C) {
        int r = g;
        for (; r + 56 < nb; r += 64) {
            double va[8], vb[8];
#pragma unroll
            for (int u = 0; u < 8; ++u) {
                va[u] = bacc[(long long)(r + 8 * u) * 2 * C + c];
                vb[u] = bacc[(long long)(r + 8 * u) * 2 * C + C + c];
            }
#pragma unroll
            for (int u = 0; u < 8; ++u) { a += va[u]; b2 += vb[u]; }
        }
        for (; r < nb; r += 8) { a += bacc[(long long)r * 2 * C + c]; b2 += bacc[(long long)r * 2 * C + C + c]; }
    }
    red[0][g][cl] = a; red[1][g][cl] = b2;
    __syncthreads();
    s = 0; ss = 0;
    if (g == 0) {
#pragma unroll
        for (int k = 0; k < 8; ++k) { s += red[0][k][cl]; ss += red[1][k][cl]; }
    }
}

__global__ __launch_bounds__(256) void bn_finalize_kernel(const double* __restrict__ bacc, int nb, long long M, int C, float eps,
                                                          float momentum, float* __restrict__ mean, float* __restrict__ invstd,
                                                          float* __restrict__ rmean, float* __restrict__ rvar, long long* nbt) {
    __shared__ double red[2][8][32];
    double s, ss;
    fold_rows32(bacc, nb, C, blockIdx.x * 32, red, s, ss);
    if (blockIdx.x == 0 && threadIdx.x == 0 && nbt) *nbt += 1;
    const int c = blockIdx.x * 32 + (threadIdx.x & 31);
    if ((threadIdx.x >> 5) != 0 || c >= C) return;
    const double mu = s / (double)M;
    double var = ss / (double)M - mu * mu;
    if (var < 0) var = 0;
    mean[c] = (float)mu;
    invstd[c] = (float)(1.0 / sqrt(var + (double)eps));
    if (rmean) rmean[c] = (1.0f - momentum) * rmean[c] + momentum * (float)mu;
    if (rvar) {
        const double unb = M > 1 ? var * (double)M / (double)(M - 1) : var;
        rvar[c] = (1.0f - momentum) * rvar[c] + momentum * (float)unb;
    }
}

__device__ __forceinline__ void amax_track(unsigned& m, const f32x4 o) {
#pragma unroll
    for (int e = 0; e < 4; ++e) {
        const unsigned b = __float_as_uint(o[e]) & 0x7fffffffu;
        if (b < 0x7f800000u && b > m) m = b;
    }
}
__device__ __forceinline__ void amax_commit(unsigned m, unsigned* out) {
    __shared__ unsigned wmax[PW_THREADS / 64];
#pragma unroll
    for (int off = 32; off > 0; off >>= 1) {
        const unsigned o = (unsigned)__shfl_xor((int)m, off, 64);
        m = o > m ? o : m;
    }
    if ((threadIdx.x & 63) == 0) wmax[threadIdx.x >> 6] = m;
    __syncthreads();
    if (threadIdx.x == 0) {
        unsigned v = wmax[0];
#pragma unroll
        for (int w = 1; w < PW_THREADS / 64; ++w) v = wmax[w] > v ? wmax[w] : v;
        if (v > __hip_atomic_load(out, __ATOMIC_RELAXED, __HIP_MEMORY_SCOPE_AGENT)) atomicMax(out, v);
    }
}

__global__ __launch_bounds__(256) void bn_planes_bound_kernel(const float* __restrict__ gamma, const float* __restrict__ beta, int C,
                                                              float sqrt_m1, const unsigned* __restrict__ res_amax,
                                                              unsigned* __restrict__ out, const unsigned* __restrict__ floor_word = nullptr) {
    __shared__ float red[256];
    float m = 0.f;
    for (int c = threadIdx.x; c < C; c += 256) m = fmaxf(m, fabsf(gamma[c]) * sqrt_m1 + fabsf(beta[c]));
    red[threadIdx.x] = m;
    __syncthreads();
    for (int s = 128; s > 0; s >>= 1) {
        if (threadIdx.x < s) red[threadIdx.x] = fmaxf(red[threadIdx.x], red[threadIdx.x + s]);
        __syncthreads();
    }
    if (threadIdx.x == 0) {
        float b = red[0] * 1.0001f;
        if (res_amax) b += __uint_as_float(*res_amax) * 1.0001f;
        unsigned w = __float_as_uint(b);
        if (floor_word && *floor_word > w) w = *floor_word;
        *out = w;
    }
}


__device__ __forceinline__ unsigned st_off(unsigned voff, unsigned soff) { return voff + soff; }
constexpr int POL_NT = 2;
typedef unsigned u2v __attribute__((ext_vector_type(2)));
__device__ __forceinline__ unsigned pair_swap(unsigned v) {
    return (unsigned)__builtin_amdgcn_update_dpp(0, (int)v, 0xB1, 0xf, 0xf, true);
}
__device__ __forceinline__ unsigned planes_col_off(int c0, bool paired) {
    const unsigned tile = (unsigned)(c0 >> 5) * 128u;
    return paired ? tile + ((c0 & 4) ? 64u : 0u) + (unsigned)((c0 & 24) >> 3) * 16u : tile + (unsigned)(c0 & 31) * 2u;
}
__device__ __forceinline__ void store_planes4(__amdgpu_buffer_rsrc_t rs, unsigned voff, unsigned soff, int c0, const f32x4 o, float ps,
                                              bool paired) {
    typedef _Float16 h2 __attribute__((ext_vector_type(2)));
    h2 h01, h23, l01, l23;
    const float t0 = o[0] * ps, t1 = o[1] * ps, t2 = o[2] * ps, t3 = o[3] * ps;
    h01[0] = (_Float16)t0; h01[1] = (_Float16)t1; h23[0] = (_Float16)t2; h23[1] = (_Float16)t3;
    l01[0] = (_Float16)((t0 - (float)h01[0]) * 2048.f); l01[1] = (_Float16)((t1 - (float)h01[1]) * 2048.f);
    l23[0] = (_Float16)((t2 - (float)h23[0]) * 2048.f); l23[1] = (_Float16)((t3 - (float)h23[1]) * 2048.f);
    const unsigned hv0 = __builtin_bit_cast(unsigned, h01), hv1 = __builtin_bit_cast(unsigned, h23);
    const unsigned lv0 = __builtin_bit_cast(unsigned, l01), lv1 = __builtin_bit_cast(unsigned, l23);
    if (paired) {
        const bool odd = (c0 & 4) != 0;
        const unsigned r0 = pair_swap(odd ? hv0 : lv0), r1 = pair_swap(odd ? hv1 : lv1);
        u32x4 v;
        if (odd) { v[0] = r0; v[1] = r1; v[2] = lv0; v[3] = lv1; }
        else { v[0] = hv0; v[1] = hv1; v[2] = r0; v[3] = r1; }
        __builtin_amdgcn_raw_buffer_store_b128(v, rs, (int)st_off(voff, soff), 0, 0);
    } else {
        u2v hv, lv;
        hv[0] = hv0; hv[1] = hv1; lv[0] = lv0; lv[1] = lv1;
        __builtin_amdgcn_raw_buffer_store_b64(hv, rs, (int)st_off(voff, soff), 0, 0);
        __builtin_amdgcn_raw_buffer_store_b64(lv, rs, (int)(st_off(voff, soff) + 64u), 0, 0);
    }
}

__device__ __forceinline__ void store_bf16x4(__amdgpu_buffer_rsrc_t rs, unsigned voff, unsigned soff, const f32x4 o) {
    u2v v;
    v[0] = (unsigned)__builtin_bit_cast(unsigned short, (__bf16)o[0]) | ((unsigned)__builtin_bit_cast(unsigned short, (__bf16)o[1]) << 16);
    v[1] = (unsigned)__builtin_bit_cast(unsigned short, (__bf16)o[2]) | ((unsigned)__builtin_bit_cast(unsigned short, (__bf16)o[3]) << 16);
    __builtin_amdgcn_raw_buffer_store_b64(v, rs, (int)st_off(voff, soff), 0, 0);
}

template <bool YBF> struct YRaw { u32x4 r; };
template <> struct YRaw<true> { u2v r; };
template <bool YBF, int POL>
__device__ __forceinline__ void y_load(YRaw<YBF>& d, __amdgpu_buffer_rsrc_t rs, unsigned voff, unsigned soff) {
    if constexpr (YBF) d.r = __builtin_amdgcn_raw_buffer_load_b64(rs, (int)voff, (int)soff, POL);
    else d.r = __builtin_amdgcn_raw_buffer_load_b128(rs, (int)voff, (int)soff, POL);
}
template <bool YBF> __device__ __forceinline__ f32x4 y_get(const YRaw<YBF>& d) {
    if constexpr (YBF) {
        f32x4 v;
        v[0] = __uint_as_float(d.r[0] << 16); v[1] = __uint_as_float(d.r[0] & 0xffff0000u);
        v[2] = __uint_as_float(d.r[1] << 16); v[3] = __uint_as_float(d.r[1] & 0xffff0000u);
        return v;
    } else {
        return __builtin_bit_cast(f32x4, d.r);
    }
}
template <int POL>
__device__ __forceinline__ f32x4 bn_load4(__amdgpu_buffer_rsrc_t rs, unsigned voff, unsigned soff) {
    return __builtin_bit_cast(f32x4, __builtin_amdgcn_raw_buffer_load_b128(rs, (int)voff, (int)soff, POL));
}
__device__ __forceinline__ void buf_store4(__amdgpu_buffer_rsrc_t rs, unsigned voff, unsigned soff, f32x4 v) {
    __builtin_amdgcn_raw_buffer_store_b128(__builtin_bit_cast(u32x4, v), rs, (int)st_off(voff, soff), 0, 0);
}
__device__ __forceinline__ __amdgpu_buffer_rsrc_t trip_rsrc(const float* t, long long ld, long long tb, long long M) {
    const unsigned long long left = (unsigned long long)(M - tb) * (unsigned long long)ld * 4ull;
    return y4_make_rsrc(t ? t + tb * ld : t, t ? (unsigned)(left < 0xfffffff0ull ? left : 0xfffffff0ull) : 0u);
}

template <int ACT, bool RES, bool YBF, bool NT>
__global__ __launch_bounds__(PW_THREADS) void bn_act_fwd_kernel(
    const float* __restrict__ y, long long ldy, const float* __restrict__ mean, const float* __restrict__ invstd,
    const float* __restrict__ gamma, const float* __restrict__ beta,
    const float* __restrict__ res, long long ldr, float* __restrict__ z, long long ldz,
    long long M, int C, int tpr, int rpb, unsigned* __restrict__ out_amax, int planes, float* __restrict__ twin) {
    const int tid = threadIdx.x;
    const int cv = tid % tpr, rg = tid / tpr;
    unsigned amax = 0u;
    float ps = 1.f;
    const bool paired = (C & 7) == 0 && tpr >= 2;
    if (planes == 1) {
        const unsigned e8 = (*out_amax >> 23) & 0xffu;
        int se = 268 - (int)e8;
        if (e8 == 0u || e8 == 255u) se = 127;
        se = se < 2 ? 2 : (se > 252 ? 252 : se);
        ps = __uint_as_float((unsigned)se << 23);
    }
    const long long trip_rows = (long long)PW_UNROLL * rpb;
    const long long step = (long long)gridDim.x * trip_rows;
    float* const pdst = twin ? twin : z;
    const long long ldp = twin ? (long long)C : ldz;
    const unsigned sy = (unsigned)(rpb * ldy * 4), sr = (unsigned)(rpb * ldr * 4), sz = (unsigned)(rpb * ldz * 4),
                   sp = (unsigned)(rpb * ldp * 4);
    for (int c0 = cv * 4; c0 < C; c0 += tpr * 4) {
        f32x4 a, b;
#pragma unroll
// ... 550 lines not shown
}

int y4_bn_stats_f32(const float* y, int ldy, long long M, int C, float* mean, float* invstd,
                    float* running_mean, float* running_var, long long* num_batches_tracked,
                    float momentum, float eps, void* workspace, size_t workspace_bytes, void* stream) {
    if (!y || !mean || !invstd || !workspace) return Y4_ERR_NULL;
    if (!vec_ok(y, ldy, C) || M <= 0) return Y4_ERR_SHAPE;
    if (workspace_bytes < y4_bn_workspace(M, C)) return Y4_ERR_WORKSPACE;
    hipStream_t st = y4_stream(stream);
    double* acc = static_cast<double*>(workspace);
    double* bacc = acc + 2 * C;
    float* part = reinterpret_cast<float*>(acc + (size_t)(1 + FOLD_BLOCKS) * 2 * C);
    const RowMap rm = row_map(C);
    const int nrows = stat_rows(M, rm.rpb);
    const long long blocks = bn_blocks(M, C);
    hipLaunchKernelGGL(bn_stats_kernel, dim3((unsigned)blocks), dim3(PW_THREADS), 0, st, y, (long long)ldy, M, C,
                       rm.tpr, rm.rpb, nrows, part);
    Y4_CHECK_LAUNCH();
    int nb = 0;
    { const int rc = fold_partials(part, blocks, C, bacc, &nb, st); if (rc != Y4_OK) return rc; }
    hipLaunchKernelGGL(bn_finalize_kernel, dim3((C + 31) / 32), dim3(256), 0, st, bacc, nb, M, C, eps, momentum, mean,
                       invstd, running_mean, running_var, num_batches_tracked);
    Y4_CHECK_LAUNCH();
    return Y4_OK;
}

int y4_bn_finalize_partials_f32(const float* partials, long long nparts, long long M, int C,
                                float* mean, float* invstd, float* running_mean, float* running_var,
                                long long* num_batches_tracked, float momentum, float eps,
                                void* workspace, size_t workspace_bytes, void* stream) {
    if (!partials || !mean || !invstd || !workspace) return Y4_ERR_NULL;
    if (nparts <= 0 || M <= 0 || C <= 0) return Y4_ERR_SHAPE;
    if (workspace_bytes < y4_bn_finalize_workspace(C)) return Y4_ERR_WORKSPACE;
    hipStream_t st = y4_stream(stream);
    double* bacc = static_cast<double*>(workspace) + 2 * C;
    int nb = 0;
    { const int rc = fold_partials(partials, nparts, C, bacc, &nb, st); if (rc != Y4_OK) return rc; }
    hipLaunchKernelGGL(bn_finalize_kernel, dim3((C + 31) / 32), dim3(256), 0, st, bacc, nb, M, C, eps, momentum, mean,
                       invstd, running_mean, running_var, num_batches_tracked);
    Y4_CHECK_LAUNCH();
    return Y4_OK;
}

int y4_bn_planes_bound_f32(const float* gamma, const float* beta, int C, long long M, const unsigned* floor_word, unsigned* out,
                           void* stream) {
    if (!gamma || !beta || !out) return Y4_ERR_NULL;
    if (C <= 0 || M <= 0) return Y4_ERR_SHAPE;
    hipLaunchKernelGGL(bn_planes_bound_kernel, dim3(1), dim3(256), 0, y4_stream(stream), gamma, beta, C,
                       sqrtf((float)(M > 1 ? M - 1 : 1)), nullptr, out, floor_word);
    Y4_CHECK_LAUNCH();
    return Y4_OK;
}

int y4_bn_act_fwd_f32(const float* y, int ldy, const float* mean, const float* invstd,
                      const float* gamma, const float* beta, int act,
                      const float* residual, int ldr, float* z, int ldz,
                      long long M, int C, unsigned* out_amax, int z_planes, const unsigned* res_amax, float* planes_twin,
                      void* stream) {
    if (!y || !mean || !invstd || !gamma || !beta) return Y4_ERR_NULL;
    const int ybf = (z_planes >> 4) & 1;
    z_planes &= 15;
    if (!z && (!out_amax || z_planes)) return Y4_ERR_NULL;
    if (z_planes < 0 || z_planes > 3) return Y4_ERR_SHAPE;
    if (planes_twin && (!z_planes || (reinterpret_cast<uintptr_t>(planes_twin) & 15))) return Y4_ERR_SHAPE;
    if (z_planes && ((!out_amax && z_planes != 3) || (C & 31))) return Y4_ERR_SHAPE;
    if (z_planes && !planes_twin && ldz != C && (ldz < C || (ldz & 31) || (reinterpret_cast<uintptr_t>(z) & 127))) return Y4_ERR_SHAPE;
    if (z_planes == 2) {
        if (residual && !res_amax) return Y4_ERR_NULL;
        hipLaunchKernelGGL(bn_planes_bound_kernel, dim3(1), dim3(256), 0, y4_stream(stream), gamma, beta, C,
                           sqrtf((float)(M > 1 ? M - 1 : 1)), residual ? res_amax : nullptr, out_amax);
        Y4_CHECK_LAUNCH();
    }
    if (!vec_ok(y, ldy, C) || (z && !vec_ok(z, ldz, C)) || (residual && !vec_ok(residual, ldr, C)) || M <= 0)
        return Y4_ERR_SHAPE;
    const RowMap rm = row_map(C);
    long long blocks = (M + rm.rpb * PW_UNROLL - 1) / (rm.rpb * PW_UNROLL);
    if (blocks > 256 * 16) blocks = 256 * 16;
    const bool nt = bn_loads_nt(M, C);
#define Y4_BN_FWD(RES_, YBF_)                                                                                                    \
    if (nt) Y4_BN_FWD_(RES_, YBF_, true); else Y4_BN_FWD_(RES_, YBF_, false)
#define Y4_BN_FWD_(RES_, YBF_, NT_)                                                                                              \
    hipLaunchKernelGGL((bn_act_fwd_kernel<A_, RES_, YBF_, NT_>), dim3((unsigned)blocks), dim3(PW_THREADS), 0, y4_stream(stream), y, \
                       (long long)ldy, mean, invstd, gamma, beta, residual, (long long)ldr, z, (long long)ldz, M, C, rm.tpr,      \
                       rm.rpb, z_planes == 3 ? nullptr : out_amax, z_planes == 3 ? 2 : (z_planes ? 1 : 0), planes_twin)
    if (residual) {
        if (ybf) { Y4_ACT_SWITCH(act, Y4_BN_FWD(true, true)); }
        else { Y4_ACT_SWITCH(act, Y4_BN_FWD(true, false)); }
    } else {
        if (ybf) { Y4_ACT_SWITCH(act, Y4_BN_FWD(false, true)); }
        else { Y4_ACT_SWITCH(act, Y4_BN_FWD(false, false)); }
    }
#undef Y4_BN_FWD
#undef Y4_BN_FWD_
    Y4_CHECK_LAUNCH();
    return Y4_OK;
}

static int bn_act_bwd_impl(const float* dz, int lddz, const float* y, int ldy,
                           const float* mean, const float* invstd, const float* gamma, const float* beta,
                           int act, float* dy, int lddy, float* dgamma, float* dbeta,
                           long long M, int C, void* workspace, size_t workspace_bytes, unsigned* out_amax,
                           unsigned* f16_planes, float* planes_twin, int flags, void* stream) {
    if (!dz || !y || !mean || !invstd || !gamma || !beta || !dy || !dgamma || !dbeta || !workspace) return Y4_ERR_NULL;
    const int frozen = flags & 1, bf = (flags >> 1) & 1, ybf = (flags >> 2) & 1;
    if (frozen && f16_planes) return Y4_ERR_SHAPE;
    if (bf && (f16_planes || (!planes_twin && lddy != C) || (C & 31))) return Y4_ERR_SHAPE;
    if (planes_twin && ((!f16_planes && !bf) || (reinterpret_cast<uintptr_t>(planes_twin) & 15))) return Y4_ERR_SHAPE;
    if (!vec_ok(dz, lddz, C) || !vec_ok(y, ldy, C) || !vec_ok(dy, lddy, C) || M <= 0) return Y4_ERR_SHAPE;
    if (workspace_bytes < y4_bn_workspace(M, C)) return Y4_ERR_WORKSPACE;
    hipStream_t st = y4_stream(stream);
    double* acc = static_cast<double*>(workspace);
    double* bacc = acc + 2 * C;
    float* part = reinterpret_cast<float*>(acc + (size_t)(1 + FOLD_BLOCKS) * 2 * C);
    const RowMap rm = row_map(C);
    const int nrows = stat_rows(M, rm.rpb);
    const long long rblocks = bn_blocks(M, C);
    int nb = 0;
    const bool nt = bn_loads_nt(M, C);
    {
#define Y4_BN_RED(BND_, YBF_)                                                                                                    \
        if (nt) Y4_BN_RED_(BND_, YBF_, true); else Y4_BN_RED_(BND_, YBF_, false)
#define Y4_BN_RED_(BND_, YBF_, NT_)                                                                                              \
        hipLaunchKernelGGL((bn_act_bwd_reduce_kernel<A_, BND_, YBF_, NT_>), dim3((unsigned)rblocks), dim3(PW_THREADS), 0, st, dz,  \
                           (long long)lddz, y, (long long)ldy, mean, invstd, gamma, beta, M, C, rm.tpr, rm.rpb, nrows, part,       \
                           f16_planes)
        if (f16_planes && ybf) return Y4_ERR_SHAPE;
        if (f16_planes) { Y4_ACT_SWITCH(act, Y4_BN_RED(true, false)); }
        else if (ybf) { Y4_ACT_SWITCH(act, Y4_BN_RED(false, true)); }
        else { Y4_ACT_SWITCH(act, Y4_BN_RED(false, false)); }
#undef Y4_BN_RED
#undef Y4_BN_RED_
        Y4_CHECK_LAUNCH();
        const int rc = fold_partials(part, rblocks, C, bacc, &nb, st);
        if (rc != Y4_OK) return rc;
    }
    if (f16_planes && ((!planes_twin && lddy != C) || (C & 31))) return Y4_ERR_SHAPE;
    hipLaunchKernelGGL(bn_bwd_finalize_kernel, dim3((C + 31) / 32), dim3(256), 0, st, bacc, nb, C, acc, dgamma, dbeta, gamma,
                       invstd, 1.0 / (double)M, f16_planes);
    Y4_CHECK_LAUNCH();
    long long blocks = (M + rm.rpb * PW_UNROLL - 1) / (rm.rpb * PW_UNROLL);
    if (blocks > 256 * 16) blocks = 256 * 16;
#define Y4_BN_APP(YBF_)                                                                                                          \
    if (nt) Y4_BN_APP_(YBF_, true); else Y4_BN_APP_(YBF_, false)
#define Y4_BN_APP_(YBF_, NT_)                                                                                                    \
    hipLaunchKernelGGL((bn_act_bwd_apply_kernel<A_, YBF_, NT_>), dim3((unsigned)blocks), dim3(PW_THREADS), 0, st, dz,              \
                       (long long)lddz,                                                                                          \
                       y, (long long)ldy, mean, invstd, gamma, beta, acc, dy, (long long)lddy, M, C, rm.tpr, rm.rpb, out_amax,    \
                       f16_planes, frozen ? 1 : 0, bf, planes_twin)
    if (ybf) { Y4_ACT_SWITCH(act, Y4_BN_APP(true)); }
    else { Y4_ACT_SWITCH(act, Y4_BN_APP(false)); }
#undef Y4_BN_APP
#undef Y4_BN_APP_
    Y4_CHECK_LAUNCH();
    return Y4_OK;
}

int y4_bn_act_bwd_f32(const float* dz, int lddz, const float* y, int ldy,
                      const float* mean, const float* invstd, const float* gamma, const float* beta,
                      int act, float* dy, int lddy, float* dgamma, float* dbeta,
                      long long M, int C, void* workspace, size_t workspace_bytes, unsigned* out_amax,
                      unsigned* f16_planes, float* planes_twin, int frozen_stats, void* stream) {
    return bn_act_bwd_impl(dz, lddz, y, ldy, mean, invstd, gamma, beta, act, dy, lddy, dgamma, dbeta, M, C, workspace,
                           workspace_bytes, out_amax, f16_planes, planes_twin, frozen_stats, stream);
}

static int colsum_rows(long long M) { return (int)(M < 1024 ? M : 1024); }

size_t y4_bias_grad_workspace(long long M, int C) {
    if (M <= 0 || C <= 0) return 0;
    return (size_t)colsum_rows(M) * (size_t)C * sizeof(float);
}

int y4_bias_grad_f32(const float* dy, int lddy, long long M, int C, float* dbias,
                     void* workspace, size_t workspace_bytes, void* stream) {
    if (!dy || !dbias || !workspace) return Y4_ERR_NULL;
    if (M <= 0 || C <= 0 || lddy < C) return Y4_ERR_SHAPE;
    if (workspace_bytes < y4_bias_grad_workspace(M, C)) return Y4_ERR_WORKSPACE;
    hipStream_t st = y4_stream(stream);
    float* part = static_cast<float*>(workspace);
    const int R = colsum_rows(M);
    hipLaunchKernelGGL(colsum_kernel, dim3((unsigned)R, (C + 255) / 256), dim3(256), 0, st, dy, (long long)lddy, M, C, part);
    Y4_CHECK_LAUNCH();
    hipLaunchKernelGGL(colsum_finalize_kernel, dim3((C + 7) / 8), dim3(256), 0, st, part, R, C, dbias);
    Y4_CHECK_LAUNCH();
    return Y4_OK;
}

int y4_bn_fold_f32(const float* gamma, const float* beta, const float* running_mean,
                   const float* running_var, float eps, float* scale, float* shift, int C, void* stream) {
    if (!gamma || !beta || !running_mean || !running_var || !scale || !shift) return Y4_ERR_NULL;
    if (C <= 0) return Y4_ERR_SHAPE;
    hipLaunchKernelGGL(bn_fold_kernel, dim3((C + 255) / 256), dim3(256), 0, y4_stream(stream), gamma, beta,
                       running_mean, running_var, eps, scale, shift, C);
    Y4_CHECK_LAUNCH();
    return Y4_OK;
}

int y4_copy_channels_f32(const float* src, int lds, float* dst, int ldd, long long M, int C, void* stream) {
    if (!vec_ok(src, lds, C) || !vec_ok(dst, ldd, C) || M <= 0) return Y4_ERR_SHAPE;
    hipLaunchKernelGGL(copy_rows_kernel, dim3(grid_for(M * (C / 4))), dim3(PW_THREADS), 0, y4_stream(stream),
                       src, (long long)lds, dst, (long long)ldd, M, C / 4);
    Y4_CHECK_LAUNCH();
    return Y4_OK;
}

int y4_add_f32(const float* a, int lda, const float* b, int ldb, float* out, int ldo,
               long long M, int C, void* stream) {
    if (!vec_ok(a, lda, C) || !vec_ok(b, ldb, C) || !vec_ok(out, ldo, C) || M <= 0) return Y4_ERR_SHAPE;
    hipLaunchKernelGGL(add_rows_kernel, dim3(grid_for(M * (C / 4))), dim3(PW_THREADS), 0, y4_stream(stream),
                       a, (long long)lda, b, (long long)ldb, out, (long long)ldo, M, C / 4);
    Y4_CHECK_LAUNCH();
    return Y4_OK;
}

int y4_maxpool_s1_fwd_f32(const float* x, int ldx, float* y, int ldy, signed char* idx,
                          int B, int H, int W, int C, int ksize, void* stream) {
    if (!vec_ok(x, ldx, C) || !vec_ok(y, ldy, C) || B <= 0 || H <= 0 || W <= 0) return Y4_ERR_SHAPE;
    if (ksize < 1 || (ksize & 1) == 0 || ksize > 11) return Y4_ERR_SHAPE;
    hipLaunchKernelGGL(maxpool_fwd_kernel, dim3(grid_for((long long)B * H * W * (C / 4))), dim3(PW_THREADS), 0,
                       y4_stream(stream), x, (long long)ldx, y, (long long)ldy, idx, B, H, W, C / 4, ksize);
    Y4_CHECK_LAUNCH();
    return Y4_OK;
}

int y4_maxpool_s1_bwd_f32(const float* dy, int lddy, const signed char* idx, float* dx, int lddx,
                          int accumulate, int B, int H, int W, int C, int ksize, void* stream) {
    if (!idx) return Y4_ERR_NULL;
    if (!vec_ok(dy, lddy, C) || !vec_ok(dx, lddx, C) || B <= 0 || H <= 0 || W <= 0) return Y4_ERR_SHAPE;
    if (ksize < 1 || (ksize & 1) == 0 || ksize > 11) return Y4_ERR_SHAPE;
    const int grid = grid_for((long long)B * H * W * (C / 4));
    if (accumulate)
        hipLaunchKernelGGL(maxpool_bwd_kernel<true>, dim3(grid), dim3(PW_THREADS), 0, y4_stream(stream), dy,
                           (long long)lddy, idx, dx, (long long)lddx, B, H, W, C / 4, ksize);
    else
        hipLaunchKernelGGL(maxpool_bwd_kernel<false>, dim3(grid), dim3(PW_THREADS), 0, y4_stream(stream), dy,
                           (long long)lddy, idx, dx, (long long)lddx, B, H, W, C / 4, ksize);
    Y4_CHECK_LAUNCH();
    return Y4_OK;
}

int y4_upsample2x_fwd_f32(const float* x, int ldx, float* y, int ldy, int B, int H, int W, int C, void* stream) {
    if (!vec_ok(x, ldx, C) || !vec_ok(y, ldy, C) || B <= 0 || H <= 0 || W <= 0) return Y4_ERR_SHAPE;
    hipLaunchKernelGGL(upsample2x_fwd_kernel, dim3(grid_for((long long)B * 4 * H * W * (C / 4))), dim3(PW_THREADS), 0,
                       y4_stream(stream), x, (long long)ldx, y, (long long)ldy, B, H, W, C / 4);
    Y4_CHECK_LAUNCH();
    return Y4_OK;
}

int y4_upsample2x_bwd_f32(const float* dy, int lddy, float* dx, int lddx, int B, int H, int W, int C, void* stream) {
    if (!vec_ok(dy, lddy, C) || !vec_ok(dx, lddx, C) || B <= 0 || H <= 0 || W <= 0) return Y4_ERR_SHAPE;
    hipLaunchKernelGGL(upsample2x_bwd_kernel, dim3(grid_for((long long)B * H * W * (C / 4))), dim3(PW_THREADS), 0,
                       y4_stream(stream), dy, (long long)lddy, dx, (long long)lddx, B, H, W, C / 4);
    Y4_CHECK_LAUNCH();
    return Y4_OK;
}

int y4_upsample_nearest_fwd_f32(const float* x, int ldx, float* y, int ldy, int B, int H, int W, int Ho, int Wo, int C,
                                int integer_factor, void* stream) {
    if (!vec_ok(x, ldx, C) || !vec_ok(y, ldy, C) || B <= 0 || H <= 0 || W <= 0 || Ho <= 0 || Wo <= 0) return Y4_ERR_SHAPE;
    int fh = 0, fw = 0;
    if (integer_factor) {
        if (Ho % H || Wo % W) return Y4_ERR_SHAPE;
        fh = Ho / H; fw = Wo / W;
    }
    hipLaunchKernelGGL(upsample_nearest_fwd_kernel, dim3(grid_for((long long)B * Ho * Wo * (C / 4))), dim3(PW_THREADS), 0,
                       y4_stream(stream), x, (long long)ldx, y, (long long)ldy, B, H, W, Ho, Wo, C / 4, fh, fw,
                       (float)H / (float)Ho, (float)W / (float)Wo);
    Y4_CHECK_LAUNCH();
    return Y4_OK;
}

int y4_upsample_nearest_bwd_f32(const float* dy, int lddy, float* dx, int lddx, int B, int H, int W, int Ho, int Wo, int C,
                                int integer_factor, void* stream) {
    if (!vec_ok(dy, lddy, C) || !vec_ok(dx, lddx, C) || B <= 0 || H <= 0 || W <= 0 || Ho <= 0 || Wo <= 0) return Y4_ERR_SHAPE;
    int fh = 0, fw = 0;
    if (integer_factor) {
        if (Ho % H || Wo % W) return Y4_ERR_SHAPE;
        fh = Ho / H; fw = Wo / W;
    }
    hipLaunchKernelGGL(upsample_nearest_bwd_kernel, dim3(grid_for((long long)B * H * W * (C / 4))), dim3(PW_THREADS), 0,
                       y4_stream(stream), dy, (long long)lddy, dx, (long long)lddx, B, H, W, Ho, Wo, C / 4, fh, fw,
                       (float)H / (float)Ho, (float)W / (float)Wo);
    Y4_CHECK_LAUNCH();
    return Y4_OK;
}

int y4_act_fwd_f32(const float* x, float* y, long long n, int act, void* stream) {
    if (!x || !y) return Y4_ERR_NULL;
    if (n <= 0 || act < 0 || act > 3) return Y4_ERR_SHAPE;
    hipLaunchKernelGGL(act_fwd_flat_kernel, dim3(grid_for((n + 3) / 4)), dim3(PW_THREADS), 0, y4_stream(stream), x, y, n, act);
    Y4_CHECK_LAUNCH();
    return Y4_OK;
}

int y4_act_bwd_f32(const float* x, const float* dy, float* dx, long long n, int act, void* stream) {
    if (!x || !dy || !dx) return Y4_ERR_NULL;
    if (n <= 0 || act < 0 || act > 3) return Y4_ERR_SHAPE;
    hipLaunchKernelGGL(act_bwd_flat_kernel, dim3(grid_for((n + 3) / 4)), dim3(PW_THREADS), 0, y4_stream(stream), x, dy, dx, n, act);
    Y4_CHECK_LAUNCH();
    return Y4_OK;
}

}
```

yolov4_amd/ops.py:

```python
import ctypes
import functools
import os

import torch

from ._lib import ACT_IDS, Y4Error, check, float_array, int_array, lib

CL = torch.channels_last


def _stream():
    return ctypes.c_void_p(torch.cuda.current_stream().cuda_stream)


def _ptr(t):
    return ctypes.c_void_p(t.data_ptr()) if t is not None else None


def _require_gpu(t, what):
    if not t.is_cuda:
        raise Y4Error(f'{what}: tensor is on {t.device}; the yolov4_amd hot path runs on an MI355X only '
                      '(no CPU fallback)')
    if t.dtype != torch.float32:
        raise Y4Error(f'{what}: expected float32, got {t.dtype}')
# ... 306 lines not shown
    __str__ = __repr__

    def __format__(self, spec):
        return self.__repr__()

    def detach(self):
        return as_planes(torch.Tensor.detach(self), getattr(self, 'y4_amax', None))


def as_planes(t, cell=None):
    if type(t) is not PlanesTensor:
        t = t.as_subclass(PlanesTensor)
    t.y4_planes = True
    if cell is not None:
        t.y4_amax = cell
    return t


def planes_split_raw(x, amax=None):
    L = lib()
    B, C, H, W = x.shape
    x, ldx = as_nhwc(x)
    if planes_mode() == 'bf16':
        amax = None
    else:
        if amax is None:
            amax = amax_of(x)
        if amax is None:
            amax = amax_raw(x)
    buf = torch.empty((B, H, W, C * 4), dtype=torch.uint8, device=x.device)
    check(L.y4_planes_split_f32(_ptr(x), ldx, B * H * W, C, _ptr(amax), _ptr(buf), _stream()), 'planes_split')
    return Planes(buf, (B, C, H, W), amax)


def conv_fwd_planes_raw(xp, w, k, s, stats=True, dgrad_filter=None, y_bf16=False, bias=None, out=None):
    L = lib()
    B, Cin, H, W = xp.shape
    Cout = w.shape[0]
    Ho, Wo = conv_out_hw(H, W, k, s)
    y = out if _slot_ok(out, (B, Cout, Ho, Wo)) else empty_nhwc(B, Cout, Ho, Wo, xp.buf.device)
    w = krsc(w)
    nbytes = L.y4_conv2d_fwd_workspace(Cin, Cout, k)
    ws = _ws(nbytes, xp.buf.device)
    pbytes = ((B * Ho * Wo + 127) // 128) * 2 * Cout * 4 if stats else 0
    part = _ws(pbytes, xp.buf.device) if stats else None
    n = ctypes.c_longlong(0)
    check(L.y4_conv2d_fwd_planes_f32(_ptr(xp.buf), _ptr(w), _ptr(y), nhwc_pitch(y), B, H, W, Cin, Cout, k, s,
                                     _ptr(part), pbytes, ctypes.byref(n), _ptr(xp.amax), _ptr(ws), nbytes,
                                     _ptr(dgrad_filter), dgrad_filter.numel() if dgrad_filter is not None else 0,
                                     1 if y_bf16 else 0, _ptr(bias), _stream()),
          'conv2d_fwd_planes')
    return (y, part, n.value) if stats else y


def conv_fwd_planes_bnstats_raw(xp, w, k, s, running_mean, running_var, nbt, momentum, eps, dgrad_filter=None, y_bf16=False):
    L = lib()
    y, part, nparts = conv_fwd_planes_raw(xp, w, k, s, dgrad_filter=dgrad_filter, y_bf16=y_bf16)
    Cout = w.shape[0]
    M = y.shape[0] * y.shape[2] * y.shape[3]
    mean = torch.empty(Cout, device=y.device, dtype=torch.float32)
    invstd = torch.empty(Cout, device=y.device, dtype=torch.float32)
    wsb = L.y4_bn_finalize_workspace(Cout)
    ws = _ws(wsb, y.device)
    check(L.y4_bn_finalize_partials_f32(_ptr(part), nparts, M, Cout, _ptr(mean), _ptr(invstd),
                                        _ptr(running_mean), _ptr(running_var), _ptr(nbt), float(momentum), float(eps),
                                        _ptr(ws), wsb, _stream()), 'bn_finalize_partials')
    return y, mean, invstd


def planes_of(t):
    if t is None or not getattr(t, 'y4_planes', False):
        return None
    return Planes(t, t.shape, getattr(t, 'y4_amax', None))


def conv_dgrad_planes_raw(dyp, w, x_shape, k, residual=None, prepared=None, s=1):
    L = lib()
    B, Cin, H, W = x_shape
    Cout = w.shape[0]
    dx = empty_nhwc(B, Cin, H, W, dyp.buf.device)
    nbytes = L.y4_conv2d_dgrad_workspace(Cin, Cout, k)
    ws = prepared if prepared is not None else _ws(nbytes, dyp.buf.device)
    ldr = 0
    if residual is not None:
        residual, ldr = as_nhwc(residual)
    check(L.y4_conv2d_dgrad_planes_f32(_ptr(dyp.buf), None if prepared is not None else _ptr(krsc(w)), _ptr(dx), nhwc_pitch(dx), B, H, W, Cin, Cout, k,
                                       s, _ptr(ws), nbytes, _ptr(dyp.amax), _ptr(residual), ldr, _stream()), 'conv2d_dgrad_planes')
    return dx


def conv_wgrad_planes_raw(xp, dyp, w_shape, k, out=None, s=1):
    L = lib()
    B, Cin, H, W = xp.shape
    Cout = w_shape[0]
    if out is not None and tuple(out.shape) == tuple(w_shape) and _is_krsc_dense(out) and out.data_ptr() % 16 == 0:
        dw = out
        WGRAD_STATS['in_place'] += 1
    else:
        WGRAD_STATS['temporary'] += 1
        dw = krsc(torch.empty(w_shape, device=xp.buf.device, dtype=torch.float32).contiguous(memory_format=CL))
    nbytes = L.y4_conv2d_wgrad_planes_workspace(B, H, W, Cin, Cout, k, s)
    ws = _ws(nbytes, xp.buf.device)
    check(L.y4_conv2d_wgrad_planes_f32(_ptr(xp.buf), _ptr(dyp.buf), _ptr(dw), B, H, W, Cin, Cout, k, s, _ptr(ws), nbytes,
                                       _ptr(xp.amax), _ptr(dyp.amax), _stream()), 'conv2d_wgrad_planes')
    return dw


def conv_stem_dgrad_raw(dy, w, x):
    L = lib()
    B, _, H, W = x.shape
    dy, lddy = as_nhwc(dy, need_vec4=False)
    dx = torch.empty_like(x, memory_format=torch.preserve_format)
    sb, sc, sh, sw = dx.stride()
    check(L.y4_conv2d_stem_dgrad_f32(_ptr(dy), lddy, _ptr(krsc(w)), _ptr(dx), sb, sc, sh, sw, B, H, W, w.shape[0], _stream()),
          'conv2d_stem_dgrad')
    return dx


def last_conv_kernel():
    import ctypes
    buf = ctypes.create_string_buffer(160)
    check(lib().y4_last_conv_kernel(buf, 160), 'last_conv_kernel')
    return buf.value.decode()


def conv_dgrad_raw(dy, w, x_shape, k, s, dy_amax=None, residual=None, prepared=None):
    L = lib()
    B, Cin, H, W = x_shape
    Cout = w.shape[0]
    if k not in (1, 3) or s not in (1, 2):
        dy, lddy = as_nhwc(dy, need_vec4=False)
        dx = empty_nhwc(B, Cin, H, W, dy.device)
        ldr = 0
        if residual is not None:
            residual, ldr = as_nhwc(residual, need_vec4=False)
        check(L.y4_conv2d_generic_dgrad_f32(_ptr(dy), lddy, _ptr(krsc(w)), _ptr(dx), nhwc_pitch(dx), B, H, W, Cin, Cout, k, s,
                                            _ptr(residual), ldr, _stream()), 'conv2d_generic_dgrad')
        return dx
    cpad = (Cout + 31) // 32 * 32
    dy, lddy = as_nhwc(dy, min_pitch=cpad)
    dx = empty_nhwc(B, Cin, H, W, dy.device)
    nbytes = L.y4_conv2d_dgrad_workspace(Cin, Cout, k)
    ws = prepared if prepared is not None else _ws(nbytes, dy.device)
    ldr = 0
    if residual is not None:
        residual, ldr = as_nhwc(residual, need_vec4=False)
    check(L.y4_conv2d_dgrad_f32(_ptr(dy), lddy, None if prepared is not None else _ptr(krsc(w)), _ptr(dx), nhwc_pitch(dx), B, H, W, Cin, Cout, k, s,
                                _ptr(ws), nbytes, _ptr(dy_amax), _ptr(residual), ldr, _stream()),
          'conv2d_dgrad')
    return dx


def _is_krsc_dense(t):
    Co, Ci, kh, kw = t.shape
    exp = (kh * kw * Ci, 1, kw * Ci, Ci)
    st = t.stride()
    return t.dtype == torch.float32 and all(t.shape[i] == 1 or st[i] == exp[i] for i in range(4))


WGRAD_STATS = {'in_place': 0, 'temporary': 0}



def conv_wgrad_raw(x, dy, w_shape, k, s, out=None, x_amax=None, dy_amax=None):
    L = lib()
    B, Cin, H, W = x.shape
    Cout = w_shape[0]
    if out is not None and tuple(out.shape) == tuple(w_shape) and _is_krsc_dense(out) and out.data_ptr() % 16 == 0:
        dw = out
        WGRAD_STATS['in_place'] += 1
    else:
        WGRAD_STATS['temporary'] += 1
        dw = torch.empty(w_shape, device=dy.device, dtype=torch.float32).contiguous(memory_format=CL)
        dw = krsc(dw)
    if k not in (1, 3) or s not in (1, 2) or (Cin % 4 and Cin != 3) or (Cin == 3 and (k != 3 or s != 1 or Cout > 32)):
        xs, ldx = as_nhwc(x, need_vec4=False)
        dys, lddy = as_nhwc(dy, need_vec4=False)
        check(L.y4_conv2d_generic_wgrad_f32(_ptr(xs), ldx, _ptr(dys), lddy, _ptr(dw), B, H, W, Cin, Cout, k, s, _stream()),
              'conv2d_generic_wgrad')
        return dw
    if Cin == 3:
        dy, lddy = as_nhwc(dy, need_vec4=False)
        nbytes = L.y4_conv2d_stem_wgrad_workspace(B, H, W, Cout)
        ws = _ws(nbytes, dy.device)
        sb, sc, sh, sw = x.stride()
        check(L.y4_conv2d_stem_wgrad_f32(_ptr(x), sb, sc, sh, sw, _ptr(dy), lddy, _ptr(dw), B, H, W, Cout,
                                         _ptr(ws), nbytes, _stream()), 'conv2d_stem_wgrad')
        return dw
    x, ldx = as_nhwc(x)
    dy, lddy = as_nhwc(dy, min_pitch=(Cout + 3) // 4 * 4)
    nbytes = L.y4_conv2d_wgrad_workspace(B, H, W, Cin, Cout, k, s)
    ws = _ws(nbytes, dy.device)
    check(L.y4_conv2d_wgrad_f32(_ptr(x), ldx, _ptr(dy), lddy, _ptr(dw), B, H, W, Cin, Cout, k, s,
                                _ptr(ws), nbytes, _ptr(x_amax), _ptr(dy_amax), _stream()), 'conv2d_wgrad')
    return dw


def bn_stats_raw(y, running_mean, running_var, nbt, momentum, eps):
    L = lib()
    B, C, H, W = y.shape
    y, ld = as_nhwc(y)
    mean = torch.empty(C, device=y.device, dtype=torch.float32)
    invstd = torch.empty(C, device=y.device, dtype=torch.float32)
    nbytes = L.y4_bn_workspace(B * H * W, C)
    ws = _ws(nbytes, y.device)
    check(L.y4_bn_stats_f32(_ptr(y), ld, B * H * W, C, _ptr(mean), _ptr(invstd), _ptr(running_mean),
                            _ptr(running_var), _ptr(nbt), float(momentum), float(eps), _ptr(ws), nbytes, _stream()),
          'bn_stats')
    return mean, invstd


def _slot_ok(out, shape):
    if out is None:
        return False
    ld = nhwc_pitch(out)
    return (tuple(out.shape) == tuple(shape) and out.dtype == torch.float32 and ld is not None and ld % 4 == 0
            and out.data_ptr() % 16 == 0)


def bn_act_fwd_raw(y, mean, invstd, gamma, beta, act, residual=None, out=None, out_amax=None, planes=False, y_bf16=False, cell=None):
    L = lib()
    B, C, H, W = y.shape
    y, ldy = as_nhwc(y)
    ldr = 0
    if residual is not None:
        residual, ldr = as_nhwc(residual)
    yb = 16 if y_bf16 else 0
    if planes == 'slot':
        cb = out.y4_cat
        if residual is not None or not _slot_ok(out, (B, C, H, W)):
            raise Y4Error('a pre-split concat slot takes a BatchNorm result of its own shape, without a skip operand')
        bf = planes_mode() == 'bf16'
        zp = out.data_ptr()
        if bf:
            zp = cb.buf.data_ptr() + (zp - cb.buf.data_ptr()) // 2
        check(L.y4_bn_act_fwd_f32(_ptr(y), ldy, _ptr(mean), _ptr(invstd), _ptr(gamma), _ptr(beta), ACT_IDS[act], None, 0,
                                  ctypes.c_void_p(zp), nhwc_pitch(out), B * H * W, C, None if bf else _ptr(cb.cell[0:1]),
                                  (3 if bf else 1) + yb, None, None, _stream()), 'bn_act_fwd(planes slot)')
        return out
    if planes:
        both = planes == 'both'
        zp = empty_nhwc(B, C, H, W, y.device)
        z = (out if _slot_ok(out, (B, C, H, W)) else empty_nhwc(B, C, H, W, y.device)) if both else zp
        args = (_ptr(y), ldy, _ptr(mean), _ptr(invstd), _ptr(gamma), _ptr(beta), ACT_IDS[act], _ptr(residual), ldr)
        if planes_mode() == 'bf16':
            check(L.y4_bn_act_fwd_f32(*args, _ptr(z), nhwc_pitch(z), B * H * W, C, None, 3 + yb, None,
                                      _ptr(zp) if both else None, _stream()), 'bn_act_fwd(bf16)')
            zp = as_planes(zp)
            if both:
                z.y4_twin = zp
                return z
            return zp
        given = cell is not None
        if given and (residual is not None or both):
            raise Y4Error('a given plane scale goes with a plain planes-only result')
        cell = cell if given else planes_cell(y.device)
        res_cell = amax_of(residual) if residual is not None else None
        if given:
            mode = 1
        elif residual is not None and res_cell is None:
            check(L.y4_bn_act_fwd_f32(*args, None, C, B * H * W, C, _ptr(cell), yb, None, None, _stream()), 'bn_act_fwd(measure)')
            mode = 1
        else:
            mode = 2
        check(L.y4_bn_act_fwd_f32(*args, _ptr(z), nhwc_pitch(z), B * H * W, C, _ptr(cell), mode + yb, _ptr(res_cell),
                                  _ptr(zp) if both else None, _stream()), 'bn_act_fwd(planes)')
        zp = as_planes(zp, cell)
        if both:
            z.y4_twin = zp
            return tag_amax(z, cell[0:1])
        return as_planes(zp, cell[0:1])
    z = out if _slot_ok(out, (B, C, H, W)) else empty_nhwc(B, C, H, W, y.device)
    check(L.y4_bn_act_fwd_f32(_ptr(y), ldy, _ptr(mean), _ptr(invstd), _ptr(gamma), _ptr(beta), ACT_IDS[act],
                              _ptr(residual), ldr, _ptr(z), nhwc_pitch(z), B * H * W, C, _ptr(out_amax), yb, None, None, _stream()),
          'bn_act_fwd')
    return z


def bn_act_bwd_raw(dz, y, mean, invstd, gamma, beta, act, dgamma_out=None, dbeta_out=None, out_amax=None, planes=None,
                   frozen=False, bf16=False, twin=False, y_bf16=False):
    L = lib()
    B, C, H, W = y.shape
    dz, lddz = as_nhwc(dz)
    y, ldy = as_nhwc(y)
    dy = empty_nhwc(B, C, H, W, y.device)

    def slot(t):
        ok = t is not None and t.dtype == torch.float32 and tuple(t.shape) == (C,) and t.is_contiguous() and t.is_cuda
        return t if ok else torch.empty(C, device=y.device, dtype=torch.float32)
    dgamma, dbeta = slot(dgamma_out), slot(dbeta_out)
    dyp = empty_nhwc(B, C, H, W, y.device) if twin else None
    nbytes = L.y4_bn_workspace(B * H * W, C)
    ws = _ws(nbytes, y.device)
    check(L.y4_bn_act_bwd_f32(_ptr(dz), lddz, _ptr(y), ldy, _ptr(mean), _ptr(invstd), _ptr(gamma), _ptr(beta),
                              ACT_IDS[act], _ptr(dy), nhwc_pitch(dy), _ptr(dgamma), _ptr(dbeta), B * H * W, C,
                              _ptr(ws), nbytes, _ptr(out_amax), _ptr(planes), _ptr(dyp) if twin else None,
                              (1 if frozen else 0) | (2 if bf16 else 0) | (4 if y_bf16 else 0), _stream()),
          'bn_act_bwd')
    if twin:
        return dy, dgamma, dbeta, dyp
    return dy, dgamma, dbeta


def bias_grad_raw(dy):
    L = lib()
    B, C, H, W = dy.shape
    dy, ld = as_nhwc(dy, need_vec4=False)
    db = torch.empty(C, device=dy.device, dtype=torch.float32)
    nbytes = L.y4_bias_grad_workspace(B * H * W, C)
    ws = _ws(nbytes, dy.device)
    check(L.y4_bias_grad_f32(_ptr(dy), ld, B * H * W, C, _ptr(db), _ptr(ws), nbytes, _stream()), 'bias_grad')
    return db


def bn_fold_raw(gamma, beta, rm, rv, eps):
    L = lib()
    C = gamma.numel()
    scale = torch.empty(C, device=gamma.device, dtype=torch.float32)
    shift = torch.empty(C, device=gamma.device, dtype=torch.float32)
    check(L.y4_bn_fold_f32(_ptr(gamma), _ptr(beta), _ptr(rm), _ptr(rv), float(eps), _ptr(scale), _ptr(shift), C,
                           _stream()), 'bn_fold')
    return scale, shift


def add_raw(a, b):
    L = lib()
    B, C, H, W = a.shape
    a, lda = as_nhwc(a)
    b, ldb = as_nhwc(b)
    out = empty_nhwc(B, C, H, W, a.device)
    check(L.y4_add_f32(_ptr(a), lda, _ptr(b), ldb, _ptr(out), nhwc_pitch(out), B * H * W, C, _stream()), 'add')
    return out


def copy_into_raw(src, dst):
    L = lib()
    B, C, H, W = src.shape
    src, lds = as_nhwc(src)
    ldd = nhwc_pitch(dst)
    if ldd is None:
        raise Y4Error('copy_into: destination is not NHWC')
    check(L.y4_copy_channels_f32(_ptr(src), lds, _ptr(dst), ldd, B * H * W, C, _stream()), 'copy_channels')


_ASYNC = {'on': os.environ.get('Y4_ASYNC_WGRAD', '0') == '1', 'streams': {}, 'join_queued': False}


def set_async_wgrad(on):
    _ASYNC['on'] = bool(on)


def side_stream(device):
    key = device.index if device.index is not None else torch.cuda.current_device()
    st = _ASYNC['streams'].get(key)
    if st is None:
        st = torch.cuda.Stream(device=device)
        _ASYNC['streams'][key] = st
    return st


def join_side_stream(device=None):
    for st in _ASYNC['streams'].values():
        torch.cuda.current_stream(st.device).wait_stream(st)
    _ASYNC['join_queued'] = False


def _wgrad_to_param(x, dy, param, k, s, x_amax=None, dy_amax=None, fn=None):
    main = torch.cuda.current_stream(x.device)
    side = side_stream(x.device)
    ev = main.record_event()
    with torch.cuda.stream(side):
        side.wait_event(ev)
        dw = fn() if fn is not None else conv_wgrad_raw(x, dy, tuple(param.shape), k, s, x_amax=x_amax, dy_amax=dy_amax)
        if param.grad is None:
            dw.record_stream(main)
            param.grad = dw
        else:
            param.grad.record_stream(side)
            param.grad.add_(dw)
        ready = getattr(param, '_y4_grad_ready', None)
        if ready is not None:
            ready()
    x.record_stream(side)
    dy.record_stream(side)
    for cell in (x_amax, dy_amax):
        if cell is not None:
            cell.record_stream(side)
    if not _ASYNC['join_queued']:
        _ASYNC['join_queued'] = True
        torch.autograd.Variable._execution_engine.queue_callback(join_side_stream)


def _pad_out_channels(weight, bias, cop):
    co = weight.shape[0]
    if cop == co:
        return weight, bias
    wp = torch.zeros((cop,) + tuple(weight.shape[1:]), dtype=weight.dtype, device=weight.device).contiguous(memory_format=torch.channels_last)
    wp[:co].copy_(weight)
    bp = None
    if bias is not None:
        bp = torch.zeros(cop, dtype=bias.dtype, device=bias.device)
        bp[:co].copy_(bias)
    return wp, bp


def _split_padded(t, cop, amax=None):
    B, C, H, W = t.shape
    t, ld = as_nhwc(t)
    if ld < cop:
        v = empty_nhwc(B, cop, H, W, t.device)
        v[:, :C].copy_(t)
        t, ld = v, nhwc_pitch(v)
    buf = torch.empty((B, H, W, cop * 4), dtype=torch.uint8, device=t.device)
    check(lib().y4_planes_split_into_f32(_ptr(t), ld, B * H * W, cop, _ptr(amax), _ptr(buf), cop, C, _stream()), 'planes_split(padded)')
    return Planes(buf, (B, cop, H, W), amax)


class ConvBNActFn(torch.autograd.Function):

    @staticmethod
    def forward(ctx, x, weight, bias, gamma, beta, residual, cfg):
        k, s, act, training, bn = cfg['k'], cfg['s'], cfg['act'], cfg['training'], cfg['bn']
        _require_gpu(x, 'ConvBNAct input')
        _require_gpu(weight, 'ConvBNAct weight')
        dest = cfg.pop('out', None)
        ctx.cfg = {key: cfg.get(key) for key in ('k', 's', 'act', 'gamma_param', 'beta_param', 'weight_param',
                                                 'dres_put', 'dres_take', 'dx_put')}
        ctx.x_shape = tuple(x.shape)
        ctx.has_res = residual is not None
        f16 = f16x2_mode() and x.shape[1] != 3
        bfm = planes_mode() == 'bf16'
        xp = planes_of(x)
        if xp is None and cfg.get('x_twin') is not None:
            xp = planes_of(cfg['x_twin'])
        ctx.x_planes = xp is not None
        nobn_planes = xp is not None and not bn and act == 'linear' and residual is None and s == 1 and cfg.get('grad', True)
        if xp is not None and not ((f16 or bfm) and x.shape[1] % 32 == 0 and (nobn_planes or (
                bn and training and weight.shape[0] % 32 == 0 and (s == 1 or planes_stride2_ok(k, s, x.shape[2], x.shape[3]))))):
            raise Y4Error('a pre-split (planes) tensor reached a conv that cannot consume it')
        x_amax = live(cfg.get('x_amax')) if f16 else None
        z_amax = None
        io = cfg.get('io')
        if xp is not None:
            x_amax = xp.amax
        elif f16 and x_amax is None and (ctx.needs_input_grad[0] or ctx.needs_input_grad[1]):
            x_amax = amax_raw(x)
        ctx.x_amax = x_amax
        if bn and training:
            if x.shape[0] * conv_out_hw(x.shape[2], x.shape[3], k, s)[0] * conv_out_hw(x.shape[2], x.shape[3], k, s)[1] <= 1:
                raise ValueError('Expected more than 1 value per channel when training')
            ctx.dgrad_filter = None
            if ((f16 or (bfm and xp is not None)) and ctx.needs_input_grad[0] and x.shape[1] % 32 == 0 and fast_conv_shape(x.shape[1], k, s)
                    and weight.shape[0] % 4 == 0 and (xp is None or weight.shape[0] % 32 == 0)
                    and not (bfm and xp is not None and s == 2
                             and not s2_plane_dgrad(x.shape[0], x.shape[2], x.shape[3], x.shape[1], weight.shape[0]))):
                ctx.dgrad_filter = dgrad_filter_buffer(x.shape[1], weight.shape[0], k, x.device)
            ybf = ctx.y_bf16 = bool(bfm and xp is not None and weight.shape[0] % 32 == 0 and _BF16_Y)
            if xp is not None:
                y, mean, invstd = conv_fwd_planes_bnstats_raw(xp, weight, k, s, cfg['running_mean'], cfg['running_var'],
                                                              cfg['nbt'], cfg['momentum'], cfg['eps'], dgrad_filter=ctx.dgrad_filter,
                                                              y_bf16=ybf)
            else:
                y, mean, invstd = conv_fwd_bnstats_raw(x, weight, k, s, cfg['running_mean'], cfg['running_var'],
                                                       cfg['nbt'], cfg['momentum'], cfg['eps'], x_amax=x_amax,
                                                       dgrad_filter=ctx.dgrad_filter)
            want = cfg.get('out_planes')
            cb = cfg.get('out_cat')
            if cb is not None and cb.planes:
                z = bn_act_fwd_raw(y, mean, invstd, gamma, beta, act, residual, out=dest, planes='slot', y_bf16=ybf)
                if io is not None:
                    io['z_planes'] = True
                z_amax = cb.cell[0:1] if cb.cell is not None else None
            elif want and (f16 or bfm) and y.shape[1] % 32 == 0 and (want == 'both' or dest is None):
                sf = cfg.get('scale_from')
                z = bn_act_fwd_raw(y, mean, invstd, gamma, beta, act, residual, out=dest if want == 'both' else None,
                                   planes='both' if want == 'both' else True, y_bf16=ybf,
                                   cell=sf.cell if (sf is not None and sf.planes and sf.cell is not None and want is True) else None)
                z_amax = getattr(z, 'y4_amax', None)
                if io is not None:
                    io['z_planes'] = want != 'both'
                    io['z_twin'] = getattr(z, 'y4_twin', None)
            else:
                if f16x2_mode():
                    z_amax = live(cfg.get('out_amax')) if (dest is not None and _slot_ok(dest, tuple(y.shape))) else None
                    if z_amax is None:
                        z_amax = new_amax(x.device)
                z = bn_act_fwd_raw(y, mean, invstd, gamma, beta, act, residual, out=dest, out_amax=z_amax, y_bf16=ybf)
            ctx.save_for_backward(xp.buf if xp is not None else x, weight, y, mean, invstd, gamma, beta)
            ctx.mode = 'bn_train'
        elif bn and cfg.get('grad', True) and any(ctx.needs_input_grad[i] for i in (0, 1, 3, 4)):
            y = conv_fwd_raw(x, weight, k, s, x_amax=x_amax, out=empty_nhwc(x.shape[0], weight.shape[0],
                                                                              *conv_out_hw(x.shape[2], x.shape[3], k, s), x.device, pad_to=4))
            invstd, _ = bn_fold_raw(torch.ones_like(gamma), beta, cfg['running_mean'], cfg['running_var'], cfg['eps'])
            mean = cfg['running_mean']
            if f16x2_mode():
                z_amax = live(cfg.get('out_amax')) if (dest is not None and _slot_ok(dest, tuple(y.shape))) else None
                if z_amax is None:
                    z_amax = new_amax(x.device)
            z = bn_act_fwd_raw(y, mean, invstd, gamma, beta, act, residual, out=dest, out_amax=z_amax)
            ctx.save_for_backward(x, weight, y, mean.detach().clone(), invstd, gamma, beta)
            ctx.mode = 'bn_eval_grad'
        elif bn:
            frozen = not cfg.get('grad', True) and os.environ.get('Y4_NO_INFER_CACHE') != '1'
            fast = f16 and fast_conv_shape(x.shape[1], k, s)
            wprep = prepared_filter(cfg['weight_param']) if (frozen and fast and cfg.get('weight_param') is not None) else None
            scale, shift = bn_fold_raw(gamma, beta, cfg['running_mean'], cfg['running_var'], cfg['eps'])
            o = dest
            Ho, Wo = conv_out_hw(x.shape[2], x.shape[3], k, s)
            o = o if _slot_ok(o, (x.shape[0], weight.shape[0], Ho, Wo)) else None
            if fast:
                z_amax = live(cfg.get('out_amax')) if o is not None else None
                if z_amax is None:
                    z_amax = new_amax(x.device)
            z = conv_fwd_raw(x, weight, k, s, scale, shift, act, residual, out=o, x_amax=x_amax, out_amax=z_amax,
                             w_prepared=wprep)
            ctx.mode = 'bn_eval'
        elif nobn_planes:
            co = weight.shape[0]
            q = 64 if bfm else 32
            cop = (co + q - 1) // q * q
            wpad, bpad = _pad_out_channels(weight, bias, cop)
            Ho, Wo = conv_out_hw(x.shape[2], x.shape[3], k, s)
            zf = empty_nhwc(x.shape[0], cop, Ho, Wo, x.device)
            ctx.dgrad_filter = dgrad_filter_buffer(x.shape[1], cop, k, x.device) if ctx.needs_input_grad[0] else None
            conv_fwd_planes_raw(xp, wpad, k, s, stats=False, dgrad_filter=ctx.dgrad_filter, bias=bpad, out=zf)
            z = zf[:, :co]
            ctx.save_for_backward(xp.buf, weight)
            ctx.mode = 'nobn_linear'
        else:
            wprep = prepared_filter(cfg['weight_param']) if (not cfg.get('grad', True) and f16 and fast_conv_shape(x.shape[1], k, s)
                                                              and os.environ.get('Y4_NO_INFER_CACHE') != '1'
                                                              and cfg.get('weight_param') is not None) else None
            z = conv_fwd_raw(x, weight, k, s, None, bias, act, residual, out_pad=32, x_amax=x_amax, w_prepared=wprep)
            if act != 'linear':
                ctx.mode = 'nobn_act'
            else:
                ctx.save_for_backward(x, weight)
                ctx.mode = 'nobn_linear'
        if io is not None:
            io['z_amax'] = z_amax
        return z

    @staticmethod
    def backward(ctx, dz):
        cfg = ctx.cfg
        k, s, act = cfg['k'], cfg['s'], cfg['act']
        f16 = f16x2_mode() and ctx.x_shape[1] != 3
        dy_amax = dy_pl = dyP = wq = None
        x_amax = live(ctx.x_amax)
        x_planes = getattr(ctx, 'x_planes', False)
        if ctx.mode in ('bn_train', 'bn_eval_grad'):
            x, weight, y, mean, invstd, gamma, beta = ctx.saved_tensors
            gp, bp = cfg.get('gamma_param'), cfg.get('beta_param')
            sink = (gp is not None and bp is not None and getattr(gp, '_y4_grad_fresh', False)
                    and getattr(bp, '_y4_grad_fresh', False) and gp.grad is not None and bp.grad is not None
                    and ctx.needs_input_grad[3] and ctx.needs_input_grad[4])
            bfp = x_planes and planes_mode() == 'bf16'
            planes = planes_cell(dz.device, 8) if (x_planes and not bfp) else None
            dy_amax = planes[5:6] if planes is not None else (new_amax(dz.device) if f16 else None)
            twin_dy = x_planes and s == 2 and ctx.needs_input_grad[0] and not s2_plane_dgrad(
                ctx.x_shape[0], ctx.x_shape[2], ctx.x_shape[3], ctx.x_shape[1], dz.shape[1])
            res = bn_act_bwd_raw(dz, y, mean, invstd, gamma, beta, act,
                                 gp.grad if sink else None, bp.grad if sink else None,
                                 out_amax=None if planes is not None else dy_amax, planes=planes,
                                 frozen=ctx.mode == 'bn_eval_grad', bf16=bfp, twin=twin_dy, y_bf16=getattr(ctx, 'y_bf16', False))
            dy, dgamma, dbeta = res[:3]
            dy_pl = res[3] if twin_dy else dy
            if sink and dgamma is gp.grad and dbeta is bp.grad:
                gp._y4_grad_fresh = bp._y4_grad_fresh = False
                gp._y4_grad_ready()
                bp._y4_grad_ready()
                dgamma = dbeta = None
            dbias = None
        elif ctx.mode == 'nobn_linear':
            x, weight = ctx.saved_tensors
            dy = dz
            dgamma = dbeta = None
            dbias = bias_grad_raw(dz) if ctx.needs_input_grad[2] else None
            if x_planes:
                bfp = planes_mode() == 'bf16'
                q = 64 if bfp else 32
                cop = (weight.shape[0] + q - 1) // q * q
                dyP = _split_padded(dz, cop, None if bfp else amax_raw(dz))
                wq = _pad_out_channels(weight, None, cop)[0]
            elif f16:
                dy_amax = amax_raw(dy)
        else:
            raise Y4Error(f'backward through ConvBNAct in mode {ctx.mode} is not implemented')
        dx = None
        take = cfg.get('dres_take')
        skip_grad = take.pop('dres', None) if take is not None else None
        if take is not None and skip_grad is None:
            take['taker_done'] = True
        if ctx.needs_input_grad[0]:
            if ctx.x_shape[1] == 3 and k == 3 and s == 1 and weight.shape[0] <= 32 and skip_grad is None:
                dx = conv_stem_dgrad_raw(dy, weight, x)
            elif x_planes and dyP is not None:
                dx = conv_dgrad_planes_raw(dyP, wq, ctx.x_shape, k, residual=skip_grad, prepared=getattr(ctx, 'dgrad_filter', None))
            elif x_planes and (s == 1 or not twin_dy):
                dx = conv_dgrad_planes_raw(Planes(dy, dy.shape, dy_amax), weight, ctx.x_shape, k, residual=skip_grad,
                                           prepared=getattr(ctx, 'dgrad_filter', None), s=s)
            else:
                dx = conv_dgrad_raw(dy, weight, ctx.x_shape, k, s, dy_amax=dy_amax, residual=skip_grad,
                                    prepared=getattr(ctx, 'dgrad_filter', None) if f16x2_mode() else None)
            ctx.dgrad_filter = None
        elif skip_grad is not None:
            raise Y4Error('a parked skip gradient has no consumer (input of the 1x1 conv does not require grad)')
        fbox = cfg.get('dx_put')
        if fbox is not None and dx is not None and not fbox.get('taker_done'):
            fbox['dres'] = dx
            dx = None
        dw = None
        if ctx.needs_input_grad[1]:
            param = cfg.get('weight_param')

            def wgrad(out=None):
                if x_planes and dyP is not None:
                    return conv_wgrad_planes_raw(Planes(x, ctx.x_shape, ctx.x_amax), dyP, tuple(weight.shape), k, out=out)
                if x_planes:
                    return conv_wgrad_planes_raw(Planes(x, ctx.x_shape, ctx.x_amax), Planes(dy_pl, dy.shape, dy_amax),
                                                 tuple(weight.shape), k, out=out, s=s)
                return conv_wgrad_raw(x, dy, tuple(weight.shape), k, s, out=out, x_amax=x_amax, dy_amax=dy_amax)
            if _ASYNC['on'] and param is not None and param.requires_grad:
                _wgrad_to_param(x, (dyP.buf if dyP is not None else dy_pl) if x_planes else dy, param, k, s,
                                ctx.x_amax if x_planes else x_amax, dyP.amax if dyP is not None else dy_amax,
                                fn=wgrad if x_planes else None)
            elif param is not None and getattr(param, '_y4_grad_fresh', False) and param.grad is not None:
                param._y4_grad_fresh = False
                got = wgrad(out=param.grad)
                if got is not param.grad:
                    param.grad.add_(got)
                param._y4_grad_ready()
            else:
                dw = wgrad()
        dres = dz if ctx.has_res else None
        put = cfg.get('dres_put')
        if dres is not None and put is not None:
            put['dres'] = dres
            dres = None
        return dx, dw, dbias, dgamma, dbeta, dres, None


class Fork2Fn(torch.autograd.Function):

    @staticmethod
    def forward(ctx, x):
        ctx.set_materialize_grads(False)
        return x.view_as(x), x.view_as(x)

    @staticmethod
    def backward(ctx, g1, g2):
        if g1 is None:
            return g2
        if g2 is None:
            return g1
        return add_raw(g1, g2)


def fork(x):
    if not (torch.is_grad_enabled() and x.requires_grad):
        return x, x
    a, b = Fork2Fn.apply(x)
    cell = amax_of(x)
    twin = getattr(x, 'y4_twin', None)
    if twin is not None:
        a.y4_twin = b.y4_twin = twin
    if getattr(x, 'y4_planes', False):
        cell = getattr(x, 'y4_amax', None)
        return as_planes(a, cell), as_planes(b, cell)
    return tag_amax(a, cell), tag_amax(b, cell)


class AddFn(torch.autograd.Function):

    @staticmethod
    def forward(ctx, a, b):
        _require_gpu(a, 'add input')
        _require_gpu(b, 'add input')
        return add_raw(a, b)

    @staticmethod
    def backward(ctx, g):
        return g, g


class CatBuffer:

    def __init__(self, B, sizes, H, W, device, planes_norms=None):
        self.sizes = list(sizes)
        self.buf = empty_nhwc(B, sum(self.sizes), H, W, device)
        self.offsets = [sum(self.sizes[:i]) for i in range(len(self.sizes))]
        self.amax = new_amax(device) if (device.type == 'cuda' and f16x2_mode()) else None
        self.planes = False
        pm = planes_mode()
        q = 64 if pm == 'bf16' else 32
        if planes_norms is not None and pm is not None and device.type == 'cuda' and all(c % q == 0 for c in self.sizes):
            self.planes = True
            self.cell = None
            if pm == 'f16x2':
                self.cell = planes_cell(device)
                for i, n in enumerate(planes_norms):
                    if isinstance(n, torch.Tensor) and not isinstance(n, torch.nn.Module):
                        c = live(amax_of(n))
                        amax_merge(self.cell[0:1], c if c is not None else amax_raw(n))
                        continue
                    n, M = n if isinstance(n, tuple) else (n, B * H * W)
                    check(lib().y4_bn_planes_bound_f32(_ptr(n.weight), _ptr(n.bias), self.sizes[i], M,
                                                       _ptr(self.cell[0:1]) if i else None, _ptr(self.cell[0:1]), _stream()),
                          'bn_planes_bound')
                self.amax = self.cell[0:1]

    def slot(self, i):
        t = tag_amax(self.buf[:, self.offsets[i]:self.offsets[i] + self.sizes[i]], self.amax)
        if self.planes:
            t.y4_cat = self
        return t


def _split_into_slot(t, dst, cb):
    B, C, H, W = t.shape
    t, ldt = as_nhwc(t)
    zp = dst.data_ptr()
    if planes_mode() == 'bf16':
        zp = cb.buf.data_ptr() + (zp - cb.buf.data_ptr()) // 2
    check(lib().y4_planes_split_into_f32(_ptr(t), ldt, B * H * W, C, _ptr(cb.cell[0:1]) if cb.cell is not None else None,
                                         ctypes.c_void_p(zp), nhwc_pitch(dst), 0, _stream()), 'planes_split_into')


class CatFn(torch.autograd.Function):

    @staticmethod
    def forward(ctx, into, *xs):
        B, _, H, W = xs[0].shape
        ctx.sizes = [t.shape[1] for t in xs]
        if into is not None and (into.sizes != ctx.sizes or tuple(into.buf.shape) != (B, sum(ctx.sizes), H, W)):
            into = None
        out = into.buf if into is not None else empty_nhwc(B, sum(ctx.sizes), H, W, xs[0].device)
        o = 0
        for t in xs:
            _require_gpu(t, 'cat input')
            dst = out[:, o:o + t.shape[1]]
            if not (t.data_ptr() == dst.data_ptr() and t.stride() == dst.stride()):
                if into is not None and into.planes:
                    if getattr(t, 'y4_planes', False):
                        raise Y4Error('a pre-split concat buffer takes pre-split inputs only where their producers wrote them in place')
                    _split_into_slot(t, dst, into)
                else:
                    copy_into_raw(t, dst)
            elif into is not None and into.planes != bool(getattr(t, 'y4_planes', False)):
                raise Y4Error('concat buffer and input disagree on the pre-split form')
            o += t.shape[1]
        return out

    @staticmethod
    def backward(ctx, g):
        outs, o = [None], 0
        for c in ctx.sizes:
            outs.append(g[:, o:o + c])
            o += c
        return tuple(outs)


def cat(xs, into=None):
    out = CatFn.apply(into, *xs)
    if into is not None and into.planes and out.data_ptr() == into.buf.data_ptr():
        return as_planes(out, into.cell[0:1] if into.cell is not None else None)
    if into is not None and into.amax is not None and out.data_ptr() == into.buf.data_ptr():
        for t in xs:
            cell = amax_of(t)
            if cell is None:
                cell = amax_raw(t)
            if cell.data_ptr() != into.amax.data_ptr():
                amax_merge(into.amax, cell)
        tag_amax(out, into.amax)
    return out


def cat_buffer(like, sizes, hw=None, planes_norms=None):
    H, W = hw if hw is not None else (like.shape[2], like.shape[3])
    return CatBuffer(like.shape[0], sizes, H, W, like.device, planes_norms=planes_norms)


class SppPoolCatFn(torch.autograd.Function):

    @staticmethod
    def forward(ctx, x, cell=None):
        L = lib()
        _require_gpu(x, 'SPP input')
        B, C, H, W = x.shape
        x, ldx = as_nhwc(x)
        out = empty_nhwc(B, 4 * C, H, W, x.device)
        ldo = nhwc_pitch(out)
        need_idx = ctx.needs_input_grad[0]
        idx5 = torch.empty((B, H, W, C), dtype=torch.int8, device=x.device) if need_idx else None
        idx9 = torch.empty((B, H, W, C), dtype=torch.int8, device=x.device) if need_idx else None
        st = _stream()
        check(L.y4_maxpool_s1_fwd_f32(_ptr(x), ldx, _ptr(out[:, 0:C]), ldo, _ptr(idx5), B, H, W, C, 5, st), 'maxpool5')
        check(L.y4_maxpool_s1_fwd_f32(_ptr(x), ldx, _ptr(out[:, C:2 * C]), ldo, _ptr(idx9), B, H, W, C, 9, st), 'maxpool9')
        copy_into_raw(out[:, 0:C], out[:, 2 * C:3 * C])
        copy_into_raw(x, out[:, 3 * C:4 * C])
        ctx.idx = (idx5, idx9)
        ctx.shape = (B, C, H, W)
        if cell is not None:
            pl = empty_nhwc(B, 4 * C, H, W, x.device)
            check(L.y4_planes_split_f32(_ptr(out), ldo, B * H * W, 4 * C, _ptr(cell.t), _ptr(pl), st), 'planes_split(spp)')
            return pl
        return out

    @staticmethod
    def backward(ctx, g):
        L = lib()
        B, C, H, W = ctx.shape
        idx5, idx9 = ctx.idx
        g, ldg = as_nhwc(g)
        dx = empty_nhwc(B, C, H, W, g.device)
        ldx = nhwc_pitch(dx)
        st = _stream()
        copy_into_raw(g[:, 3 * C:4 * C], dx)
        for sl, idx, ks in ((g[:, 0:C], idx5, 5), (g[:, C:2 * C], idx9, 9), (g[:, 2 * C:3 * C], idx5, 5)):
            check(L.y4_maxpool_s1_bwd_f32(_ptr(sl), ldg, _ptr(idx), _ptr(dx), ldx, 1, B, H, W, C, ks, st), 'maxpool_bwd')
        return dx, None


def spp_pool_cat(x, planes=False):
    pm = planes_mode()
    if planes and pm is not None and x.is_cuda and (4 * x.shape[1]) % (64 if pm == 'bf16' else 32) == 0:
        cell = None
        if pm == 'f16x2':
            cell = planes_cell(x.device)
            src = live(amax_of(x))
            amax_merge(cell[0:1], src if src is not None else amax_raw(x))
        out = SppPoolCatFn.apply(x, Slot(cell[0:1]) if cell is not None else Slot(None))
        return as_planes(out, cell[0:1] if cell is not None else None)
    return tag_amax(SppPoolCatFn.apply(x), amax_of(x))


class MaxPoolS1Fn(torch.autograd.Function):

    @staticmethod
    def forward(ctx, x, ksize):
        L = lib()
        _require_gpu(x, 'maxpool input')
        B, C, H, W = x.shape
        x, ldx = as_nhwc(x)
        out = empty_nhwc(B, C, H, W, x.device)
        idx = torch.empty((B, H, W, C), dtype=torch.int8, device=x.device)
        check(L.y4_maxpool_s1_fwd_f32(_ptr(x), ldx, _ptr(out), nhwc_pitch(out), _ptr(idx), B, H, W, C, ksize,
                                      _stream()), 'maxpool')
        ctx.idx, ctx.ks, ctx.shape = idx, ksize, (B, C, H, W)
        return out

    @staticmethod
    def backward(ctx, g):
# ... 239 lines not shown
```

Before: 453.5.

## Fuse stem conv with BatchNorm and activation in forward and backward passes

Adds dedicated stem kernels that fuse the 3-channel 3x3 conv with BN statistics, normalization, activation and amax. In backward they recompute the conv output from x instead of storing y, and fuse BN backward, dgamma/dbeta and the weight gradient. The aim is to avoid materializing the large pre-BN stem activation (608x608x64 pixels, 32 channels) and the separate BN passes over it. The cost is recomputing the conv, which is cheap for K=27, plus added code complexity. The path is on by default and is gated on the stem shape conditions.

```diff
diff --git a/include/yolov4_amd.h b/include/yolov4_amd.h
--- a/include/yolov4_amd.h
+++ b/include/yolov4_amd.h
@@ -111,6 +111,17 @@
 int y4_conv2d_stem_wgrad_f32(const float* x, long long sxb, long long sxc, long long sxh, long long sxw,
                              const float* dy, int lddy, float* dw, int B, int H, int W, int Cout,
                              void* workspace, size_t workspace_bytes, void* stream);
+
+size_t y4_stem_bn_workspace(long long sxb, long long sxc, long long sxh, long long sxw, int B, int H, int W, int Cout);
+int y4_stem_bn_fwd_f32(const float* x, long long sxb, long long sxc, long long sxh, long long sxw, const float* w,
+                       const float* gamma, const float* beta, int act, float* z, int ldz, int B, int H, int W, int Cout,
+                       float* mean, float* invstd, int stats_given, float* running_mean, float* running_var,
+                       long long* num_batches_tracked, float momentum, float eps, unsigned* out_amax,
+                       void* workspace, size_t workspace_bytes, void* stream);
+int y4_stem_bn_bwd_f32(const float* x, long long sxb, long long sxc, long long sxh, long long sxw, const float* w,
+                       const float* dz, int lddz, int B, int H, int W, int Cout,
+                       const float* mean, const float* invstd, const float* gamma, const float* beta, int act,
+                       float* dgamma, float* dbeta, float* dw, void* workspace, size_t workspace_bytes, void* stream);
 
 size_t y4_bn_workspace(long long M, int C);
 size_t y4_bn_finalize_workspace(int C);
diff --git a/yolov4_amd/_lib.py b/yolov4_amd/_lib.py
--- a/yolov4_amd/_lib.py
+++ b/yolov4_amd/_lib.py
@@ -51,6 +51,9 @@
     'y4_conv2d_wgrad_f32': (I, [P, I, P, I, P, I, I, I, I, I, I, I, P, Z, P, P, P]),
     'y4_conv2d_stem_wgrad_workspace': (Z, [I, I, I, I]),
     'y4_conv2d_stem_wgrad_f32': (I, [P, L, L, L, L, P, I, P, I, I, I, I, P, Z, P]),
+    'y4_stem_bn_workspace': (Z, [L, L, L, L, I, I, I, I]),
+    'y4_stem_bn_fwd_f32': (I, [P, L, L, L, L, P, P, P, I, P, I, I, I, I, I, P, P, I, P, P, P, F, F, P, P, Z, P]),
+    'y4_stem_bn_bwd_f32': (I, [P, L, L, L, L, P, P, I, I, I, I, I, P, P, P, P, I, P, P, P, P, Z, P]),
     'y4_bn_workspace': (Z, [L, I]),
     'y4_bn_finalize_workspace': (Z, [I]),
     'y4_bn_finalize_partials_f32': (I, [P, L, L, I, P, P, P, P, P, F, F, P, Z, P]),
diff --git a/yolov4_amd/csrc/common.h b/yolov4_amd/csrc/common.h
--- a/yolov4_amd/csrc/common.h
+++ b/yolov4_amd/csrc/common.h
@@ -69,6 +69,14 @@
     else return 1.0f;
 }
 
+#define Y4_ACT_SWITCH(ACTV, CALL)                                              \
+    switch (ACTV) {                                                            \
+        case Y4_ACT_MISH: { constexpr int A_ = Y4_ACT_MISH; CALL; } break;     \
+        case Y4_ACT_LEAKY: { constexpr int A_ = Y4_ACT_LEAKY; CALL; } break;   \
+        case Y4_ACT_RELU: { constexpr int A_ = Y4_ACT_RELU; CALL; } break;     \
+        default: { constexpr int A_ = Y4_ACT_LINEAR; CALL; } break;            \
+    }
+
 __device__ __forceinline__ int y4_xcd_remap(int bid, int nwg) {
     const int q = nwg >> 3, r = nwg & 7, xcd = bid & 7;
     const int base = (xcd < r) ? xcd * (q + 1) : r * (q + 1) + (xcd - r) * q;
diff --git a/yolov4_amd/csrc/conv_geom.h b/yolov4_amd/csrc/conv_geom.h
--- a/yolov4_amd/csrc/conv_geom.h
+++ b/yolov4_amd/csrc/conv_geom.h
@@ -76,5 +76,8 @@
                  size_t workspace_bytes, int B, int H, int W, int Cin, int Cout, int k, hipStream_t st, bool bf = false,
                  int stride = 1);
 
+int bn_bwd_finalize_partials(const float* part, long long nparts, long long M, int C, const float* gamma, const float* invstd,
+                             float* dgamma, float* dbeta, void* workspace, hipStream_t st);
+
 void note_kernel(const char* fmt, ...);
 }
diff --git a/yolov4_amd/csrc/conv_igemm.hip b/yolov4_amd/csrc/conv_igemm.hip
--- a/yolov4_amd/csrc/conv_igemm.hip
+++ b/yolov4_amd/csrc/conv_igemm.hip
@@ -1399,114 +1399,268 @@
     }
 }
 
+struct StemFrag {
+    bf16x8 fb[2][3];
+    int koff[16];
+    int ktap[16];
+};
+__device__ __forceinline__ void stem_setup(StemFrag& s, const StemGeom& g, const int fr, const int fh) {
+#pragma unroll
+    for (int i = 0; i < 16; ++i) {
+        const int k = (i >> 3) * 16 + fh * 8 + (i & 7);
+        const int r = k / 9, c = (k - r * 9) / 3, q = k - r * 9 - c * 3;
+        const bool kv = k < 27;
+        s.koff[i] = kv ? (int)(c * g.sxc + (r - 1) * g.sxh + (q - 1) * g.sxw) * 4 : 0;
+        s.ktap[i] = kv ? r * 3 + q : 9;
+    }
+#pragma unroll
+    for (int ks = 0; ks < 2; ++ks) {
+        f32x4 w0, w1;
+#pragma unroll
+        for (int i = 0; i < 8; ++i) {
+            const int k = ks * 16 + fh * 8 + i;
+            const int r = k / 9, c = (k - r * 9) / 3, q = k - r * 9 - c * 3;
+            const float v = (k < 27 && fr < g.Cout) ? g.w[fr * 27 + (r * 3 + q) * 3 + c] : 0.f;
+            if (i < 4) w0[i] = v; else w1[i - 4] = v;
+        }
+        u32x2 a1, a2, a3, b1, b2, b3;
+        split3x4(w0, a1, a2, a3);
+        split3x4(w1, b1, b2, b3);
+        const u32x4 q1 = {a1[0], a1[1], b1[0], b1[1]}, q2 = {a2[0], a2[1], b2[0], b2[1]}, q3 = {a3[0], a3[1], b3[0], b3[1]};
+        s.fb[ks][0] = __builtin_bit_cast(bf16x8, q1); s.fb[ks][1] = __builtin_bit_cast(bf16x8, q2); s.fb[ks][2] = __builtin_bit_cast(bf16x8, q3);
+    }
+}
+__device__ __forceinline__ void stem_pixel(const StemGeom& g, const long long p, const float inv_hw, const float inv_w, int& b, int& h,
+                                           int& w) {
+    const int HW = g.H * g.W;
+    b = (int)((float)p * inv_hw);
+    int rem = (int)(p - (long long)b * HW);
+    if (rem < 0) { --b; rem += HW; } else if (rem >= HW) { ++b; rem -= HW; }
+    h = (int)((float)rem * inv_w);
+    w = rem - h * g.W;
+    if (w < 0) { --h; w += g.W; } else if (w >= g.W) { ++h; w -= g.W; }
+}
+__device__ __forceinline__ void stem_load(const StemFrag& s, const StemGeom& g, const __amdgpu_buffer_rsrc_t rsrc, float (&xv)[16],
+                                          const long long tile, const int fr, const float inv_hw, const float inv_w) {
+    const long long p = tile * 32 + fr;
+    unsigned base = 0xffffffffu;
+    unsigned m9 = 0;
+    if (p < g.M) {
+        int b, h, w;
+        stem_pixel(g, p, inv_hw, inv_w, b, h, w);
+        base = (unsigned)(b * g.sxb + h * g.sxh + w * g.sxw) * 4u;
+        const unsigned hm = (h > 0 ? 1u : 0u) | 2u | (h + 1 < g.H ? 4u : 0u);
+        const unsigned wm = (w > 0 ? 1u : 0u) | 2u | (w + 1 < g.W ? 4u : 0u);
+        m9 = ((hm & 1u) ? wm : 0u) | ((hm & 2u) ? wm << 3 : 0u) | ((hm & 4u) ? wm << 6 : 0u);
+    }
+#pragma unroll
+    for (int i = 0; i < 16; ++i) {
+        const bool ok = (m9 >> s.ktap[i]) & 1u;
+        xv[i] = __builtin_bit_cast(float, __builtin_amdgcn_raw_buffer_load_b32(rsrc, ok ? (int)(base + (unsigned)s.koff[i]) : -1, 0, 0));
+    }
+}
+__device__ __forceinline__ f32x16 stem_mma(const StemFrag& s, const float (&xv)[16]) {
+    f32x16 acc;
+#pragma unroll
+    for (int e = 0; e < 16; ++e) acc[e] = 0.f;
+#pragma unroll
+    for (int ks = 0; ks < 2; ++ks) {
+        const f32x4 v0 = {xv[ks * 8 + 0], xv[ks * 8 + 1], xv[ks * 8 + 2], xv[ks * 8 + 3]};
+        const f32x4 v1 = {xv[ks * 8 + 4], xv[ks * 8 + 5], xv[ks * 8 + 6], xv[ks * 8 + 7]};
+        u32x2 a1, a2, a3, b1, b2, b3;
+        split3x4(v0, a1, a2, a3);
+        split3x4(v1, b1, b2, b3);
+        const u32x4 q1 = {a1[0], a1[1], b1[0], b1[1]}, q2 = {a2[0], a2[1], b2[0], b2[1]}, q3 = {a3[0], a3[1], b3[0], b3[1]};
+        const bf16x8 f1 = __builtin_bit_cast(bf16x8, q1), f2 = __builtin_bit_cast(bf16x8, q2), f3 = __builtin_bit_cast(bf16x8, q3);
+        acc = __builtin_amdgcn_mfma_f32_32x32x16_bf16(f3, s.fb[ks][0], acc, 0, 0, 0);
+        acc = __builtin_amdgcn_mfma_f32_32x32x16_bf16(f2, s.fb[ks][1], acc, 0, 0, 0);
+        acc = __builtin_amdgcn_mfma_f32_32x32x16_bf16(f1, s.fb[ks][2], acc, 0, 0, 0);
+        acc = __builtin_amdgcn_mfma_f32_32x32x16_bf16(f2, s.fb[ks][0], acc, 0, 0, 0);
+        acc = __builtin_amdgcn_mfma_f32_32x32x16_bf16(f1, s.fb[ks][1], acc, 0, 0, 0);
+        acc = __builtin_amdgcn_mfma_f32_32x32x16_bf16(f1, s.fb[ks][0], acc, 0, 0, 0);
+    }
+    return acc;
+}
+__device__ __forceinline__ void stem_stat_add(float& cs, float& css, const float raw) {
+#pragma clang fp contract(off)
+    cs += raw;
+    css += raw * raw;
+}
+__device__ __forceinline__ void stem_group_row(float (&sred)[4][32][2], float cs, float css, float* __restrict__ rows, const int grp,
+                                               const int Cout) {
+    const int tid = threadIdx.x, lane = tid & 63, wave = tid >> 6, fr = lane & 31, fh = lane >> 5;
+    cs += __shfl_xor(cs, 32, 64);
+    css += __shfl_xor(css, 32, 64);
+    if (fh == 0) { sred[wave][fr][0] = cs; sred[wave][fr][1] = css; }
+    __syncthreads();
+    if (tid < 64) {
+        const int c = tid & 31, which = tid >> 5;
+        const float t = (sred[0][c][which] + sred[1][c][which]) + (sred[2][c][which] + sred[3][c][which]);
+        if (c < Cout) rows[((long long)grp * 2 + which) * Cout + c] = t;
+    }
+    __syncthreads();
+}
+
 __global__ __launch_bounds__(256) void conv_stem_fwd_bf16x3_kernel(const StemGeom g, const int ngroups, const float inv_hw,
                                                                    const float inv_w) {
     __shared__ float sred[4][32][2];
     const int tid = threadIdx.x, lane = tid & 63, wave = tid >> 6;
     const int fr = lane & 31, fh = lane >> 5;
-    const int HW = g.H * g.W;
-    bf16x8 fb[2][3];
-    int koff[16];
-    int ktap[16];
-#pragma unroll
-    for (int i = 0; i < 16; ++i) {
-        const int k = (i >> 3) * 16 + fh * 8 + (i & 7);
-        const int r = k / 9, c = (k - r * 9) / 3, q = k - r * 9 - c * 3;
-        const bool kv = k < 27;
-        koff[i] = kv ? (int)(c * g.sxc + (r - 1) * g.sxh + (q - 1) * g.sxw) * 4 : 0;
-        ktap[i] = kv ? r * 3 + q : 9;
-    }
-#pragma unroll
-    for (int ks = 0; ks < 2; ++ks) {
-        f32x4 w0, w1;
-#pragma unroll
-        for (int i = 0; i < 8; ++i) {
-            const int k = ks * 16 + fh * 8 + i;
-            const int r = k / 9, c = (k - r * 9) / 3, q = k - r * 9 - c * 3;
-            const float v = (k < 27 && fr < g.Cout) ? g.w[fr * 27 + (r * 3 + q) * 3 + c] : 0.f;
-            if (i < 4) w0[i] = v; else w1[i - 4] = v;
-        }
-        u32x2 a1, a2, a3, b1, b2, b3;
-        split3x4(w0, a1, a2, a3);
-        split3x4(w1, b1, b2, b3);
-        const u32x4 q1 = {a1[0], a1[1], b1[0], b1[1]}, q2 = {a2[0], a2[1], b2[0], b2[1]}, q3 = {a3[0], a3[1], b3[0], b3[1]};
-        fb[ks][0] = __builtin_bit_cast(bf16x8, q1); fb[ks][1] = __builtin_bit_cast(bf16x8, q2); fb[ks][2] = __builtin_bit_cast(bf16x8, q3);
-    }
+    StemFrag s;
+    stem_setup(s, g, fr, fh);
     const float sc = (g.scale && fr < g.Cout) ? g.scale[fr] : 1.f;
     const float sh = (g.shift && fr < g.Cout) ? g.shift[fr] : 0.f;
     const __amdgpu_buffer_rsrc_t rsrc = y4_make_rsrc(g.x, 0xfffffff0u);
     float xv0[16], xv1[16];
-    auto load = [&](float (&xv)[16], long long tile) {
-        const long long p = tile * 32 + fr;
-        unsigned base = 0xffffffffu;
-        unsigned m9 = 0;
-        if (p < g.M) {
-            int b = (int)((float)p * inv_hw);
-            int rem = (int)(p - (long long)b * HW);
-            if (rem < 0) { --b; rem += HW; } else if (rem >= HW) { ++b; rem -= HW; }
-            int h = (int)((float)rem * inv_w);
-            int w = rem - h * g.W;
-            if (w < 0) { --h; w += g.W; } else if (w >= g.W) { ++h; w -= g.W; }
-            base = (unsigned)(b * g.sxb + h * g.sxh + w * g.sxw) * 4u;
-            const unsigned hm = (h > 0 ? 1u : 0u) | 2u | (h + 1 < g.H ? 4u : 0u);
-            const unsigned wm = (w > 0 ? 1u : 0u) | 2u | (w + 1 < g.W ? 4u : 0u);
-            m9 = ((hm & 1u) ? wm : 0u) | ((hm & 2u) ? wm << 3 : 0u) | ((hm & 4u) ? wm << 6 : 0u);
-        }
-#pragma unroll
-        for (int i = 0; i < 16; ++i) {
-            const bool ok = (m9 >> ktap[i]) & 1u;
-            xv[i] = __builtin_bit_cast(float, __builtin_amdgcn_raw_buffer_load_b32(rsrc, ok ? (int)(base + (unsigned)koff[i]) : -1, 0, 0));
-        }
-    };
     float cs = 0.f, css = 0.f;
     auto compute = [&](float (&xv)[16], long long tile) {
-        f32x16 acc;
-#pragma unroll
-        for (int e = 0; e < 16; ++e) acc[e] = 0.f;
-#pragma unroll
-        for (int ks = 0; ks < 2; ++ks) {
-            const f32x4 v0 = {xv[ks * 8 + 0], xv[ks * 8 + 1], xv[ks * 8 + 2], xv[ks * 8 + 3]};
-            const f32x4 v1 = {xv[ks * 8 + 4], xv[ks * 8 + 5], xv[ks * 8 + 6], xv[ks * 8 + 7]};
-            u32x2 a1, a2, a3, b1, b2, b3;
-            split3x4(v0, a1, a2, a3);
-            split3x4(v1, b1, b2, b3);
-            const u32x4 q1 = {a1[0], a1[1], b1[0], b1[1]}, q2 = {a2[0], a2[1], b2[0], b2[1]}, q3 = {a3[0], a3[1], b3[0], b3[1]};
-            const bf16x8 f1 = __builtin_bit_cast(bf16x8, q1), f2 = __builtin_bit_cast(bf16x8, q2), f3 = __builtin_bit_cast(bf16x8, q3);
-            acc = __builtin_amdgcn_mfma_f32_32x32x16_bf16(f3, fb[ks][0], acc, 0, 0, 0);
-            acc = __builtin_amdgcn_mfma_f32_32x32x16_bf16(f2, fb[ks][1], acc, 0, 0, 0);
-            acc = __builtin_amdgcn_mfma_f32_32x32x16_bf16(f1, fb[ks][2], acc, 0, 0, 0);
-            acc = __builtin_amdgcn_mfma_f32_32x32x16_bf16(f2, fb[ks][0], acc, 0, 0, 0);
-            acc = __builtin_amdgcn_mfma_f32_32x32x16_bf16(f1, fb[ks][1], acc, 0, 0, 0);
-            acc = __builtin_amdgcn_mfma_f32_32x32x16_bf16(f1, fb[ks][0], acc, 0, 0, 0);
-        }
+        const f32x16 acc = stem_mma(s, xv);
         const long long mbase = tile * 32 + 4 * fh;
 #pragma unroll
         for (int e = 0; e < 16; ++e) {
             const float raw = acc[e];
-            cs += raw; css += raw * raw;
+            stem_stat_add(cs, css, raw);
             const long long m = mbase + (e & 3) + 8 * (e >> 2);
             if (fr < g.Cout && m < g.M) g.y[m * g.ldy + fr] = y4_act(raw * sc + sh, g.act);
         }
     };
     for (int grp = blockIdx.x; grp < ngroups; grp += gridDim.x) {
         const long long t0 = (long long)grp * 8 + wave * 2;
-        load(xv0, t0);
-        load(xv1, t0 + 1);
+        stem_load(s, g, rsrc, xv0, t0, fr, inv_hw, inv_w);
+        stem_load(s, g, rsrc, xv1, t0 + 1, fr, inv_hw, inv_w);
         cs = 0.f; css = 0.f;
         compute(xv0, t0);
         compute(xv1, t0 + 1);
-        if (g.stats) {
-            cs += __shfl_xor(cs, 32, 64);
-            css += __shfl_xor(css, 32, 64);
-            if (fh == 0) { sred[wave][fr][0] = cs; sred[wave][fr][1] = css; }
+        if (g.stats) stem_group_row(sred, cs, css, g.stats, grp, g.Cout);
+    }
+}
+
+enum { STEM_STATS = 1, STEM_FWD = 2, STEM_RED = 3, STEM_APPLY = 4 };
+struct StemBn {
+    const float* mean; const float* invstd; const float* gamma; const float* beta;
+    const float* dz; long long lddz;
+    unsigned* out_amax;
+    float* rows;
+    const double* acc;
+    float* slabs;
+    double invM;
+};
+
+template <int MODE, int ACT>
+__global__ __launch_bounds__(256) void stem_bn_kernel(const StemGeom g, const StemBn q, const int ngroups, const float inv_hw,
+                                                      const float inv_w) {
+    constexpr bool ROWS = MODE == STEM_STATS || MODE == STEM_RED;
+    constexpr bool BWD = MODE == STEM_RED || MODE == STEM_APPLY;
+    __shared__ float sred[4][32][2];
+    const int tid = threadIdx.x, lane = tid & 63, wave = tid >> 6;
+    const int fr = lane & 31, fh = lane >> 5;
+    const bool cok = fr < g.Cout;
+    StemFrag s;
+    stem_setup(s, g, fr, fh);
+    float mu = 0.f, is = 0.f, ga = 0.f, be = 0.f, k1 = 0.f, k2 = 0.f;
+    if (MODE != STEM_STATS && cok) { mu = q.mean[fr]; is = q.invstd[fr]; ga = q.gamma[fr]; be = q.beta[fr]; }
+    if (MODE == STEM_APPLY && cok) { k1 = (float)(q.acc[fr] * q.invM); k2 = (float)(q.acc[g.Cout + fr] * q.invM); }
+    const float a = is * ga, b = be - mu * a;
+    const __amdgpu_buffer_rsrc_t rsrc = y4_make_rsrc(g.x, 0xfffffff0u);
+    auto load_dz = [&](float (&d)[16], const long long tile) {
+        long long rows = g.M - tile * 32;
+        rows = rows < 0 ? 0 : (rows > 32 ? 32 : rows);
+        const __amdgpu_buffer_rsrc_t drs = y4_make_rsrc(q.dz + tile * 32 * q.lddz, (unsigned)(rows * q.lddz * 4));
+        const unsigned o0 = ((unsigned)(4 * fh) * (unsigned)q.lddz + (unsigned)fr) * 4u;
+#pragma unroll
+        for (int e = 0; e < 16; ++e) {
+            const unsigned o = o0 + (unsigned)((e & 3) + 8 * (e >> 2)) * (unsigned)q.lddz * 4u;
+            d[e] = __builtin_bit_cast(float, __builtin_amdgcn_raw_buffer_load_b32(drs, cok ? (int)o : -1, 0, 0));
+        }
+    };
+    __shared__ __attribute__((aligned(16))) float xs[MODE == STEM_APPLY ? 4 * 2 * 32 * 36 : 4];
+    const int jtap = fr / 3, jc = fr - jtap * 3;
+    const int jk = fr < 27 ? (jtap / 3) * 9 + jc * 3 + (jtap - (jtap / 3) * 3) : fr;
+    auto put_x = [&](const float (&xv)[16], const int t) {
+        float* row = xs + ((wave * 2 + t) * 32 + fr) * 36 + fh * 8;
+#pragma unroll
+        for (int h = 0; h < 2; ++h) {
+            const f32x4 v0 = {xv[h * 8 + 0], xv[h * 8 + 1], xv[h * 8 + 2], xv[h * 8 + 3]};
+            const f32x4 v1 = {xv[h * 8 + 4], xv[h * 8 + 5], xv[h * 8 + 6], xv[h * 8 + 7]};
+            *reinterpret_cast<f32x4*>(row + h * 16) = v0;
+            *reinterpret_cast<f32x4*>(row + h * 16 + 4) = v1;
+        }
+    };
+    const float* const xcol = xs + (wave * 2 * 32 + 4 * fh) * 36 + jk;
+    float cs = 0.f, css = 0.f;
+    unsigned amax = 0u;
+    f32x16 wacc;
+#pragma unroll
+    for (int e = 0; e < 16; ++e) wacc[e] = 0.f;
+    float xv0[16], xv1[16], d0[BWD ? 16 : 1], d1[BWD ? 16 : 1];
+    auto compute = [&](float (&xv)[16], float (&d)[BWD ? 16 : 1], const int t, const long long tile) {
+        const f32x16 acc = stem_mma(s, xv);
+        const long long mbase = tile * 32 + 4 * fh;
+        const long long mleft = g.M - mbase;
+        const int left = cok ? (int)(mleft < 0 ? 0 : (mleft > 32 ? 32 : mleft)) : 0;
+        float* const zcol = MODE == STEM_FWD ? g.y + mbase * g.ldy + fr : nullptr;
+#pragma unroll
+        for (int e = 0; e < 16; ++e) {
+            const float raw = acc[e];
+            const int re = (e & 3) + 8 * (e >> 2);
+            if constexpr (MODE == STEM_STATS) {
+                stem_stat_add(cs, css, raw);
+            } else if constexpr (MODE == STEM_FWD) {
+                const float o = y4_act_t<ACT>(raw * a + b);
+                if (re < left) {
+                    zcol[(long long)re * g.ldy] = o;
+                    const unsigned ob = __float_as_uint(o) & 0x7fffffffu;
+                    if (ob < 0x7f800000u && ob > amax) amax = ob;
+                }
+            } else {
+                const float xh = (raw - mu) * is;
+                const float gg = d[e] * y4_act_grad_t<ACT>(ga * xh + be);
+                if constexpr (MODE == STEM_RED) {
+                    cs += gg; css += gg * xh;
+                } else {
+                    const float dy = re < left ? (ga * is) * (gg - k1 - xh * k2) : 0.f;
+                    wacc = __builtin_amdgcn_mfma_f32_32x32x2f32(dy, xcol[(t * 32 + re) * 36], wacc, 0, 0, 0);
+                }
+            }
+        }
+    };
+    for (int grp = blockIdx.x; grp < ngroups; grp += gridDim.x) {
+        const long long t0 = (long long)grp * 8 + wave * 2;
+        stem_load(s, g, rsrc, xv0, t0, fr, inv_hw, inv_w);
+        stem_load(s, g, rsrc, xv1, t0 + 1, fr, inv_hw, inv_w);
+        if constexpr (BWD) { load_dz(d0, t0); load_dz(d1, t0 + 1); }
+        if constexpr (MODE == STEM_APPLY) {
+            put_x(xv0, 0); put_x(xv1, 1);
             __syncthreads();
-            if (tid < 64) {
-                const int c = tid & 31, which = tid >> 5;
-                const float t = (sred[0][c][which] + sred[1][c][which]) + (sred[2][c][which] + sred[3][c][which]);
-                if (c < g.Cout) g.stats[((long long)grp * 2 + which) * g.Cout + c] = t;
-            }
+        }
+        cs = 0.f; css = 0.f;
+        compute(xv0, d0, 0, t0);
+        compute(xv1, d1, 1, t0 + 1);
+        if constexpr (ROWS) stem_group_row(sred, cs, css, q.rows, grp, g.Cout);
+        if constexpr (MODE == STEM_APPLY) __syncthreads();
+    }
+    if constexpr (MODE == STEM_FWD) {
+        if (q.out_amax) {
+            unsigned* wmax = reinterpret_cast<unsigned*>(&sred[0][0][0]);
+#pragma unroll
+            for (int off = 32; off > 0; off >>= 1) {
+                const unsigned o = (unsigned)__shfl_xor((int)amax, off, 64);
+                amax = o > amax ? o : amax;
+            }
+            if (lane == 0) wmax[wave] = amax;
             __syncthreads();
-        }
+            if (tid == 0) {
+                unsigned v = wmax[0];
+#pragma unroll
+                for (int w = 1; w < 4; ++w) v = wmax[w] > v ? wmax[w] : v;
+                if (v > __hip_atomic_load(q.out_amax, __ATOMIC_RELAXED, __HIP_MEMORY_SCOPE_AGENT)) atomicMax(q.out_amax, v);
+            }
+        }
+    }
+    if constexpr (MODE == STEM_APPLY) {
+        float* out = q.slabs + ((long long)blockIdx.x * 4 + wave) * 1024;
+#pragma unroll
+        for (int e = 0; e < 16; ++e) out[((e & 3) + 8 * (e >> 2) + 4 * fh) * 32 + fr] = wacc[e];
     }
 }
 
@@ -1589,12 +1743,41 @@
     for (int i = threadIdx.x; i < Cout * 27; i += 256) {
         const int n = i / 27, j = i - n * 27;
         double s = 0.0;
-        for (int k = 0; k < nparts; ++k) s += part[(long long)k * 1024 + n * 32 + j];
+        int k = 0;
+        for (; k + 16 <= nparts; k += 16) {
+            double v[16];
+#pragma unroll
+            for (int u = 0; u < 16; ++u) v[u] = part[(long long)(k + u) * 1024 + n * 32 + j];
+#pragma unroll
+            for (int u = 0; u < 16; ++u) s += v[u];
+        }
+        for (; k < nparts; ++k) s += part[(long long)k * 1024 + n * 32 + j];
         dw[i] = (float)s;
     }
 }
 
 constexpr int STEM_WAVES = 4096;
+
+int stem_bn_grid(long long M, int max_grid) {
+    const long long groups = (M + 255) / 256;
+    return (int)(groups < max_grid ? groups : max_grid);
+}
+template <int MODE, int ACT>
+void launch_stem_bn_act(const StemGeom& g, const StemBn& q, int grid, hipStream_t st) {
+    y4::note_kernel("stem_bn_kernel<%d, %d>", MODE, ACT);
+    hipLaunchKernelGGL((stem_bn_kernel<MODE, ACT>), dim3(grid), dim3(256), 0, st, g, q, (int)((g.M + 255) / 256),
+                       1.0f / (float)((long long)g.H * g.W), 1.0f / (float)g.W);
+}
+template <int MODE>
+int launch_stem_bn(const StemGeom& g, const StemBn& q, int act, int grid, hipStream_t st) {
+    if constexpr (MODE == STEM_STATS) {
+        launch_stem_bn_act<MODE, Y4_ACT_LINEAR>(g, q, grid, st);
+    } else {
+        Y4_ACT_SWITCH(act, (launch_stem_bn_act<MODE, A_>(g, q, grid, st)));
+    }
+    Y4_CHECK_LAUNCH();
+    return Y4_OK;
+}
 
 }
 
@@ -1950,11 +2133,13 @@
                          (long long)H * W < (1 << 24);
     if (mfma_ok) {
         const int grid = (int)(blocks < 2048 ? blocks : 2048);
+        y4::note_kernel("conv_stem_fwd_bf16x3_kernel");
         hipLaunchKernelGGL(conv_stem_fwd_bf16x3_kernel, dim3(grid), dim3(256), 0, y4_stream(stream), g, (int)blocks,
                            1.0f / (float)((long long)H * W), 1.0f / (float)W);
         Y4_CHECK_LAUNCH();
         return Y4_OK;
     }
+    y4::note_kernel("conv_stem_fwd_kernel");
     hipLaunchKernelGGL(conv_stem_fwd_kernel, dim3((unsigned)blocks), dim3(256), 0, y4_stream(stream), g);
     Y4_CHECK_LAUNCH();
     return Y4_OK;
@@ -1982,6 +2167,7 @@
         return Y4_ERR_SHAPE;
     g.pix_per_wave = ppw;
     hipStream_t st = y4_stream(stream);
+    y4::note_kernel("conv_stem_wgrad_kernel");
     hipLaunchKernelGGL(conv_stem_wgrad_kernel, dim3(STEM_WAVES / 4), dim3(256), 0, st, g);
     Y4_CHECK_LAUNCH();
     double* part = reinterpret_cast<double*>(static_cast<char*>(workspace) + (size_t)STEM_WAVES * 1024 * sizeof(float));
@@ -1993,4 +2179,81 @@
     return Y4_OK;
 }
 
-}
+static size_t stem_bn_fin_bytes(int Cout) { return (y4_bn_finalize_workspace(Cout) + 15) & ~(size_t)15; }
+static bool stem_bn_fit(long long sxb, long long sxc, long long sxh, long long sxw, int B, int H, int W, int Cout) {
+    if (B <= 0 || H <= 0 || W <= 0 || Cout <= 0 || Cout > 32) return false;
+    return (g_conv_mode >= 1 && g_conv_mode <= 3) && sxb >= 0 && sxc >= 0 && sxh >= 0 && sxw >= 0 &&
+           ((long long)(B - 1) * sxb + 2 * sxc + (long long)(H - 1) * sxh + (long long)(W - 1) * sxw + 1) * 4 < 0xfffffff0ll &&
+           (long long)H * W < (1 << 24) && ((long long)B * H * W + 255) / 256 < (1ll << 31);
+}
+size_t y4_stem_bn_workspace(long long sxb, long long sxc, long long sxh, long long sxw, int B, int H, int W, int Cout) {
+    if (!stem_bn_fit(sxb, sxc, sxh, sxw, B, H, W, Cout)) return 0;
+    const long long groups = ((long long)B * H * W + 255) / 256;
+    return stem_bn_fin_bytes(Cout) + y4_conv2d_stem_wgrad_workspace(B, H, W, Cout) + (size_t)groups * 2 * Cout * sizeof(float);
+}
+
+int y4_stem_bn_fwd_f32(const float* x, long long sxb, long long sxc, long long sxh, long long sxw, const float* w,
+                       const float* gamma, const float* beta, int act, float* z, int ldz, int B, int H, int W, int Cout,
+                       float* mean, float* invstd, int stats_given, float* running_mean, float* running_var,
+                       long long* num_batches_tracked, float momentum, float eps, unsigned* out_amax,
+                       void* workspace, size_t workspace_bytes, void* stream) {
+    if (!x || !w || !gamma || !beta || !z || !mean || !invstd || !workspace) return Y4_ERR_NULL;
+    if (!stem_bn_fit(sxb, sxc, sxh, sxw, B, H, W, Cout) || ldz < Cout) return Y4_ERR_SHAPE;
+    if (workspace_bytes < y4_stem_bn_workspace(sxb, sxc, sxh, sxw, B, H, W, Cout)) return Y4_ERR_WORKSPACE;
+    hipStream_t st = y4_stream(stream);
+    StemGeom g{};
+    g.x = x; g.w = w; g.y = z; g.sxb = sxb; g.sxc = sxc; g.sxh = sxh; g.sxw = sxw; g.ldy = ldz;
+    g.B = B; g.H = H; g.W = W; g.Cout = Cout; g.act = act;
+    g.M = (long long)B * H * W;
+    StemBn q{};
+    q.mean = mean; q.invstd = invstd; q.gamma = gamma; q.beta = beta; q.out_amax = out_amax;
+    q.rows = reinterpret_cast<float*>(static_cast<char*>(workspace) + stem_bn_fin_bytes(Cout) +
+                                      y4_conv2d_stem_wgrad_workspace(B, H, W, Cout));
+    if (!stats_given) {
+        const int rc = launch_stem_bn<STEM_STATS>(g, q, act, stem_bn_grid(g.M, 2048), st);
+        if (rc != Y4_OK) return rc;
+        const int rc2 = y4_bn_finalize_partials_f32(q.rows, (g.M + 255) / 256, g.M, Cout, mean, invstd, running_mean, running_var,
+                                                    num_batches_tracked, momentum, eps, workspace, y4_bn_finalize_workspace(Cout),
+                                                    stream);
+        if (rc2 != Y4_OK) return rc2;
+    }
+    return launch_stem_bn<STEM_FWD>(g, q, act, stem_bn_grid(g.M, 2048), st);
+}
+
+int y4_stem_bn_bwd_f32(const float* x, long long sxb, long long sxc, long long sxh, long long sxw, const float* w,
+                       const float* dz, int lddz, int B, int H, int W, int Cout,
+                       const float* mean, const float* invstd, const float* gamma, const float* beta, int act,
+                       float* dgamma, float* dbeta, float* dw, void* workspace, size_t workspace_bytes, void* stream) {
+    if (!x || !w || !dz || !mean || !invstd || !gamma || !beta || !dgamma || !dbeta || !workspace) return Y4_ERR_NULL;
+    if (!stem_bn_fit(sxb, sxc, sxh, sxw, B, H, W, Cout) || lddz < Cout || lddz >= (1 << 24)) return Y4_ERR_SHAPE;
+    if (workspace_bytes < y4_stem_bn_workspace(sxb, sxc, sxh, sxw, B, H, W, Cout)) return Y4_ERR_WORKSPACE;
+    hipStream_t st = y4_stream(stream);
+    StemGeom g{};
+    g.x = x; g.w = w; g.sxb = sxb; g.sxc = sxc; g.sxh = sxh; g.sxw = sxw;
+    g.B = B; g.H = H; g.W = W; g.Cout = Cout; g.act = act;
+    g.M = (long long)B * H * W;
+    char* const ws = static_cast<char*>(workspace);
+    float* const slabs = reinterpret_cast<float*>(ws + stem_bn_fin_bytes(Cout));
+    StemBn q{};
+    q.mean = mean; q.invstd = invstd; q.gamma = gamma; q.beta = beta; q.dz = dz; q.lddz = lddz;
+    q.rows = reinterpret_cast<float*>(ws + stem_bn_fin_bytes(Cout) + y4_conv2d_stem_wgrad_workspace(B, H, W, Cout));
+    q.acc = reinterpret_cast<const double*>(ws);
+    q.slabs = slabs;
+    q.invM = 1.0 / (double)g.M;
+    int rc = launch_stem_bn<STEM_RED>(g, q, act, stem_bn_grid(g.M, 2048), st);
+    if (rc != Y4_OK) return rc;
+    rc = y4::bn_bwd_finalize_partials(q.rows, (g.M + 255) / 256, g.M, Cout, gamma, invstd, dgamma, dbeta, workspace, st);
+    if (rc != Y4_OK) return rc;
+    if (!dw) return Y4_OK;
+    const int grid = stem_bn_grid(g.M, STEM_WAVES / 4);
+    rc = launch_stem_bn<STEM_APPLY>(g, q, act, grid, st);
+    if (rc != Y4_OK) return rc;
+    double* part = reinterpret_cast<double*>(slabs + (size_t)STEM_WAVES * 1024);
+    hipLaunchKernelGGL(stem_wgrad_reduce1_kernel, dim3(64), dim3(256), 0, st, slabs, part, grid * 4);
+    Y4_CHECK_LAUNCH();
+    hipLaunchKernelGGL(stem_wgrad_reduce2_kernel, dim3(1), dim3(256), 0, st, part, dw, 64, Cout);
+    Y4_CHECK_LAUNCH();
+    return Y4_OK;
+}
+
+}
diff --git a/yolov4_amd/csrc/pointwise.hip b/yolov4_amd/csrc/pointwise.hip
--- a/yolov4_amd/csrc/pointwise.hip
+++ b/yolov4_amd/csrc/pointwise.hip
@@ -1,16 +1,10 @@
 #include "common.h"
+#include "conv_geom.h"
 
 namespace {
 
 constexpr int PW_THREADS = 256;
 constexpr int PW_UNROLL = 4;
-#define Y4_ACT_SWITCH(ACTV, CALL)                                              \
-    switch (ACTV) {                                                            \
-        case Y4_ACT_MISH: { constexpr int A_ = Y4_ACT_MISH; CALL; } break;     \
-        case Y4_ACT_LEAKY: { constexpr int A_ = Y4_ACT_LEAKY; CALL; } break;   \
-        case Y4_ACT_RELU: { constexpr int A_ = Y4_ACT_RELU; CALL; } break;     \
-        default: { constexpr int A_ = Y4_ACT_LINEAR; CALL; } break;            \
-    }
 
 struct RowMap {
     int tpr;
@@ -1167,3 +1161,17 @@
 }
 
 }
+
+namespace y4 {
+int bn_bwd_finalize_partials(const float* part, long long nparts, long long M, int C, const float* gamma, const float* invstd,
+                             float* dgamma, float* dbeta, void* workspace, hipStream_t st) {
+    double* acc = static_cast<double*>(workspace);
+    double* bacc = acc + 2 * C;
+    int nb = 0;
+    { const int rc = fold_partials(part, nparts, C, bacc, &nb, st); if (rc != Y4_OK) return rc; }
+    hipLaunchKernelGGL(bn_bwd_finalize_kernel, dim3((C + 31) / 32), dim3(256), 0, st, bacc, nb, C, acc, dgamma, dbeta, gamma,
+                       invstd, 1.0 / (double)M, static_cast<unsigned*>(nullptr));
+    Y4_CHECK_LAUNCH();
+    return Y4_OK;
+}
+}
diff --git a/yolov4_amd/ops.py b/yolov4_amd/ops.py
--- a/yolov4_amd/ops.py
+++ b/yolov4_amd/ops.py
@@ -632,6 +632,70 @@
     return dy, dgamma, dbeta
 
 
+_STEM_FUSED = {'on': os.environ.get('Y4_STEM_FUSED', '1') != '0'}
+
+
+def set_stem_fused(on):
+    _STEM_FUSED['on'] = bool(on)
+
+
+def stem_bn_workspace(x, Cout):
+    B, Cin, H, W = x.shape
+    if Cin != 3 or Cout > 32:
+        return 0
+    return lib().y4_stem_bn_workspace(*x.stride(), B, H, W, Cout)
+
+
+def stem_bn_fwd_raw(x, w, gamma, beta, act, running_mean=None, running_var=None, nbt=None, momentum=0.1, eps=1e-5, out=None,
+                    out_amax=None, stats=None):
+    L = lib()
+    B, _, H, W = x.shape
+    Cout = w.shape[0]
+    nbytes = stem_bn_workspace(x, Cout)
+    if not nbytes:
+        raise Y4Error('the fused stem kernels cannot serve this input (conv mode 0, or strides / extents beyond their windows)')
+    z = out if _slot_ok(out, (B, Cout, H, W)) else empty_nhwc(B, Cout, H, W, x.device)
+    ws = _ws(nbytes, x.device)
+    if stats is not None:
+        mean, invstd = stats
+    else:
+        mean = torch.empty(Cout, device=x.device, dtype=torch.float32)
+        invstd = torch.empty(Cout, device=x.device, dtype=torch.float32)
+    check(L.y4_stem_bn_fwd_f32(_ptr(x), *x.stride(), _ptr(krsc(w)), _ptr(gamma), _ptr(beta), ACT_IDS[act], _ptr(z), nhwc_pitch(z),
+                               B, H, W, Cout, _ptr(mean), _ptr(invstd), 0 if stats is None else 1, _ptr(running_mean),
+                               _ptr(running_var), _ptr(nbt), float(momentum), float(eps), _ptr(out_amax), _ptr(ws), nbytes,
+                               _stream()), 'stem_bn_fwd')
+    return z, mean, invstd
+
+
+def stem_bn_bwd_raw(dz, x, w, mean, invstd, gamma, beta, act, dgamma_out=None, dbeta_out=None, dw_out=None, want_dw=True):
+    L = lib()
+    B, _, H, W = x.shape
+    Cout = w.shape[0]
+    nbytes = stem_bn_workspace(x, Cout)
+    if not nbytes:
+        raise Y4Error('the fused stem kernels cannot serve this input (conv mode 0, or strides / extents beyond their windows)')
+    dz, lddz = as_nhwc(dz, need_vec4=False)
+
+    def slot(t):
+        ok = t is not None and t.dtype == torch.float32 and tuple(t.shape) == (Cout,) and t.is_contiguous() and t.is_cuda
+        return t if ok else torch.empty(Cout, device=x.device, dtype=torch.float32)
+    dgamma, dbeta = slot(dgamma_out), slot(dbeta_out)
+    dw = None
+    if want_dw:
+        if dw_out is not None and tuple(dw_out.shape) == tuple(w.shape) and _is_krsc_dense(dw_out):
+            dw = dw_out
+            WGRAD_STATS['in_place'] += 1
+        else:
+            WGRAD_STATS['temporary'] += 1
+            dw = krsc(torch.empty(tuple(w.shape), device=x.device, dtype=torch.float32).contiguous(memory_format=CL))
+    ws = _ws(nbytes, x.device)
+    check(L.y4_stem_bn_bwd_f32(_ptr(x), *x.stride(), _ptr(krsc(w)), _ptr(dz), lddz, B, H, W, Cout, _ptr(mean), _ptr(invstd),
+                               _ptr(gamma), _ptr(beta), ACT_IDS[act], _ptr(dgamma), _ptr(dbeta), _ptr(dw), _ptr(ws), nbytes,
+                               _stream()), 'stem_bn_bwd')
+    return dgamma, dbeta, dw
+
+
 def bias_grad_raw(dy):
     L = lib()
     B, C, H, W = dy.shape
@@ -744,6 +808,42 @@
     buf = torch.empty((B, H, W, cop * 4), dtype=torch.uint8, device=t.device)
     check(lib().y4_planes_split_into_f32(_ptr(t), ld, B * H * W, cop, _ptr(amax), _ptr(buf), cop, C, _stream()), 'planes_split(padded)')
     return Planes(buf, (B, cop, H, W), amax)
+
+
+def _stem_train_ok(ctx, x, weight, residual, cfg, dest, bfm):
+    Cout = weight.shape[0]
+    if not (_STEM_FUSED['on'] and x.shape[1] == 3 and cfg['k'] == 3 and cfg['s'] == 1 and Cout <= 32 and Cout % 4 == 0
+            and residual is None and not ctx.needs_input_grad[0]):
+        return False
+    cb, want = cfg.get('out_cat'), cfg.get('out_planes')
+    if (cb is not None and cb.planes) or (want and bfm and Cout % 32 == 0 and (want == 'both' or dest is None)):
+        return False
+    return stem_bn_workspace(x, Cout) > 0
+
+
+def _stem_train_backward(ctx, dz):
+    cfg = ctx.cfg
+    x, weight, mean, invstd, gamma, beta = ctx.saved_tensors
+    gp, bp, wp = cfg.get('gamma_param'), cfg.get('beta_param'), cfg.get('weight_param')
+    sink = (gp is not None and bp is not None and getattr(gp, '_y4_grad_fresh', False)
+            and getattr(bp, '_y4_grad_fresh', False) and gp.grad is not None and bp.grad is not None
+            and ctx.needs_input_grad[3] and ctx.needs_input_grad[4])
+    wsink = ctx.needs_input_grad[1] and wp is not None and getattr(wp, '_y4_grad_fresh', False) and wp.grad is not None
+    dgamma, dbeta, dw = stem_bn_bwd_raw(dz, x, weight, mean, invstd, gamma, beta, cfg['act'],
+                                        gp.grad if sink else None, bp.grad if sink else None,
+                                        dw_out=wp.grad if wsink else None, want_dw=ctx.needs_input_grad[1])
+    if sink and dgamma is gp.grad and dbeta is bp.grad:
+        gp._y4_grad_fresh = bp._y4_grad_fresh = False
+        gp._y4_grad_ready()
+        bp._y4_grad_ready()
+        dgamma = dbeta = None
+    if wsink:
+        wp._y4_grad_fresh = False
+        if dw is not wp.grad:
+            wp.grad.add_(dw)
+        wp._y4_grad_ready()
+        dw = None
+    return None, dw, None, dgamma, dbeta, None, None
 
 
 class ConvBNActFn(torch.autograd.Function):
@@ -776,7 +876,18 @@
         elif f16 and x_amax is None and (ctx.needs_input_grad[0] or ctx.needs_input_grad[1]):
             x_amax = amax_raw(x)
         ctx.x_amax = x_amax
-        if bn and training:
+        if bn and training and _stem_train_ok(ctx, x, weight, residual, cfg, dest, bfm):
+            if x.shape[0] * x.shape[2] * x.shape[3] <= 1:
+                raise ValueError('Expected more than 1 value per channel when training')
+            if f16x2_mode():
+                z_amax = live(cfg.get('out_amax')) if (dest is not None and _slot_ok(dest, (x.shape[0], weight.shape[0]) + tuple(x.shape[2:]))) else None
+                if z_amax is None:
+                    z_amax = new_amax(x.device)
+            z, mean, invstd = stem_bn_fwd_raw(x, weight, gamma, beta, act, cfg['running_mean'], cfg['running_var'], cfg['nbt'],
+                                              cfg['momentum'], cfg['eps'], out=dest, out_amax=z_amax)
+            ctx.save_for_backward(x, weight, mean, invstd, gamma, beta)
+            ctx.mode = 'stem_train'
+        elif bn and training:
             if x.shape[0] * conv_out_hw(x.shape[2], x.shape[3], k, s)[0] * conv_out_hw(x.shape[2], x.shape[3], k, s)[1] <= 1:
                 raise ValueError('Expected more than 1 value per channel when training')
             ctx.dgrad_filter = None
@@ -879,6 +990,8 @@
         dy_amax = dy_pl = dyP = wq = None
         x_amax = live(ctx.x_amax)
         x_planes = getattr(ctx, 'x_planes', False)
+        if ctx.mode == 'stem_train':
+            return _stem_train_backward(ctx, dz)
         if ctx.mode in ('bn_train', 'bn_eval_grad'):
             x, weight, y, mean, invstd, gamma, beta = ctx.saved_tensors
             gp, bp = cfg.get('gamma_param'), cfg.get('beta_param')
```

New measurement: 458.0 (median of 6 runs). About the same (+1.0%).
